# ZKTLabs/zkt-plonk

Hardware: AMD Instinct MI355X
Metric: proofs/sec (withdraw, n=2^20) (higher is better)
Workload: dtype u32 limbs (256-bit Montgomery); 1 GPU; full prove, WithdrawCircuit INPUTS=8 HEIGHT=64 Poseidon x5 (1019498 gates, 538 Poseidon gadgets), bn254, n=2^20, TABLE_SIZE=1024, 12 public inputs; parallelism=proofs sharded across 1 GPU(s), chained=True, distinct_witnesses=2, witness_on_device=True, table_cached=True, proof_bytes=802

## Files before the change

### include/zkt_plonk.h

```cpp
#ifndef ZKT_PLONK_H
#define ZKT_PLONK_H

#include <stddef.h>
#include <stdint.h>

#ifdef __cplusplus
extern "C" {
#endif

typedef struct zkt_ctx zkt_ctx;

enum {
    ZKT_CURVE_BN254 = 0,
    ZKT_CURVE_BLS12_381 = 1
};

enum {
    ZKT_OK = 0,
    ZKT_ERR_INVALID_ARGUMENT = 1,
    ZKT_ERR_INVALID_DOMAIN_SIZE = 2,
    ZKT_ERR_HIP = 3,
    ZKT_ERR_NO_DEVICE = 4,
    ZKT_ERR_TOO_MANY_COEFFICIENTS = 5,
    ZKT_ERR_ZERO_DENOMINATOR = 6,
    ZKT_ERR_EQUAL_CHALLENGES = 7,
    ZKT_ERR_NOT_IN_TABLE = 8,
    ZKT_ERR_QUOTIENT_TOO_SHORT = 9,
    ZKT_ERR_NOT_LOADED = 10,
    ZKT_ERR_COMM = 11
};

int zkt_ctx_create(int curve_id, int device_id, zkt_ctx** out);
void zkt_ctx_destroy(zkt_ctx* ctx);
int zkt_ctx_fork(zkt_ctx* ctx, zkt_ctx** out);
const char* zkt_last_error(const zkt_ctx* ctx);
int zkt_ctx_set_stream(zkt_ctx* ctx, void* hip_stream);
int zkt_ctx_synchronize(zkt_ctx* ctx);
int zkt_profile_enable(zkt_ctx* ctx, int on);
int zkt_profile_get(zkt_ctx* ctx, const char* name, uint64_t* calls, double* total_ms);
const char* zkt_version(void);

typedef struct {
    void* user;
    int rank;
    int world;
    int device_buffers;
    int (*all_gather)(void* user, const void* send, void* recv, size_t bytes, int on_device, void* hip_stream);
    int (*all_gather_async)(void* user, const void* d_send, void* d_recv, size_t bytes, void* hip_stream);
} zkt_comm_vtable;
#define ZKT_QUOTIENT_CHUNKS 4
int zkt_ctx_set_comm(zkt_ctx* ctx, const zkt_comm_vtable* comm);
int zkt_shard_range(size_t total, int rank, int world, size_t* lo, size_t* hi);
int zkt_comm_stats(zkt_ctx* ctx, uint64_t* calls, uint64_t* bytes_sent);
int zkt_comm_selftest(const zkt_comm_vtable* comm, const void* send, void* recv, size_t bytes);

int zkt_dev_alloc(zkt_ctx* ctx, size_t bytes, void** dptr);
int zkt_dev_free(zkt_ctx* ctx, void* dptr);
int zkt_dev_upload(zkt_ctx* ctx, void* dptr, const void* host, size_t bytes);
int zkt_dev_download(zkt_ctx* ctx, void* host, const void* dptr, size_t bytes);

int zkt_ntt(zkt_ctx* ctx, int log_n, int inverse, int coset, const uint64_t* in, size_t in_len, uint64_t* out);
int zkt_ntt_dev(zkt_ctx* ctx, int log_n, int inverse, int coset, const void* d_in, size_t in_len, void* d_out);
int zkt_ntt_class(zkt_ctx* ctx, int log_n, int log_big, int cls, const uint64_t* in, size_t in_len, uint64_t* out);
int zkt_domain_group_gen(zkt_ctx* ctx, int log_n, uint64_t* out4);

int zkt_srs_load(zkt_ctx* ctx, const uint64_t* g1_xy_mont, size_t count);
int zkt_srs_load_dev(zkt_ctx* ctx, const void* d_g1_xy_mont, size_t count);
int zkt_srs_generate(zkt_ctx* ctx, const uint64_t* tau_canonical4, size_t count);
int zkt_srs_download(zkt_ctx* ctx, size_t offset, size_t count, uint64_t* out_xy_mont);
int zkt_srs_generate_g2(int curve_id, const uint64_t* tau_canonical4, uint64_t* out_h, uint64_t* out_beta_h);
int zkt_srs_load_slice(zkt_ctx* ctx, const uint64_t* g1_xy_mont_slice, size_t offset, size_t count, size_t total);
int zkt_srs_generate_slice(zkt_ctx* ctx, const uint64_t* tau_canonical4, size_t offset, size_t count, size_t total);
int zkt_msm_g1(zkt_ctx* ctx, const uint64_t* scalars, size_t len, size_t base_offset, int scalars_montgomery,
               uint64_t* out_xy_mont, int* out_is_infinity);
int zkt_msm_g1_dev(zkt_ctx* ctx, const void* d_scalars, size_t len, size_t base_offset, int scalars_montgomery,
                   void* out_xy_mont_host);
int zkt_msm_enqueue_dev(zkt_ctx* ctx, const void* d_scalars, size_t len, size_t base_offset, int scalars_montgomery);
int zkt_msm_info(zkt_ctx* ctx, int* window_bits, int* windows, size_t* srs_count);

#define ZKT_MSM_BASES_MAX ((size_t)1 << 22)
int zkt_msm_g1_bases(zkt_ctx* ctx, const uint64_t* bases_xy_mont, const uint64_t* scalars, size_t n,
                     int scalars_montgomery, uint64_t* out_xy_mont, int* out_is_infinity);
int zkt_msm_g1_bases_dev(zkt_ctx* ctx, const void* d_bases_xy_mont, const void* d_scalars, size_t n,
                         int scalars_montgomery, uint64_t* out_xy_mont_host, int* out_is_infinity);
int zkt_msm_bases_info(zkt_ctx* ctx, size_t n, int scalars_montgomery, int* window_bits, int* windows);

#define ZKT_KZG_BATCH_MAX 32
int zkt_kzg_commit_batch(zkt_ctx* ctx, const uint64_t* const* coeffs, const size_t* lens, int k,
                         int scalars_montgomery, uint64_t* out_xy_mont, int* out_is_infinity);
int zkt_kzg_commit_batch_dev(zkt_ctx* ctx, const void* const* d_coeffs, const size_t* lens, int k,
                             int scalars_montgomery, uint64_t* out_xy_mont, int* out_is_infinity);
int zkt_kzg_open(zkt_ctx* ctx, const uint64_t* const* coeffs, const size_t* lens, int k,
                 const uint64_t* challenges_mont, const uint64_t* point_mont,
                 uint64_t* out_w_xy_mont, int* out_w_is_infinity, uint64_t* out_evals_mont);
int zkt_kzg_open_dev(zkt_ctx* ctx, const void* const* d_coeffs, const size_t* lens, int k,
                     const uint64_t* challenges_mont, const uint64_t* point_mont,
                     uint64_t* out_w_xy_mont, int* out_w_is_infinity, uint64_t* out_evals_mont);

int zkt_ctx_set_lagrange(zkt_ctx* ctx, int on);
int zkt_ctx_set_wire_elimination(zkt_ctx* ctx, int mode);
int zkt_ctx_set_quotient_route(zkt_ctx* ctx, int mode);
int zkt_ctx_set_fused_passes(zkt_ctx* ctx, int mode);
int zkt_lagrange_info(zkt_ctx* ctx, int* log_n, size_t* bases);
int zkt_commit_evals_dev(zkt_ctx* ctx, const void* d_evals, const uint64_t* blinders, int k, int path, uint64_t* out_xy_mont,
                         int* out_is_infinity);

enum {
    ZKT_TRANSCRIPT_MERLIN = 0,
    ZKT_TRANSCRIPT_ETHEREUM = 1
};
typedef struct zkt_transcript zkt_transcript;
zkt_transcript* zkt_transcript_new(int kind, const char* label);
void zkt_transcript_free(zkt_transcript* t);
void zkt_transcript_append_u64(zkt_transcript* t, const char* label, uint64_t v);
void zkt_transcript_append_scalars(zkt_transcript* t, const char* label, const uint8_t* le32, size_t count, int single);
void zkt_transcript_append_commitment(zkt_transcript* t, const char* label, const uint8_t* x_le, const uint8_t* y_le,
                                      size_t fq_bytes, int is_infinity);
void zkt_transcript_challenge_scalar(zkt_transcript* t, const char* label, int fr_bits, uint8_t out_le32[32]);
void zkt_transcript_seed(zkt_transcript* t, uint64_t circuit_size, const uint8_t* xy_le, const uint8_t* is_infinity,
                         size_t fq_bytes);
int zkt_transcript_append_message(zkt_transcript* t, const char* label, const uint8_t* msg, size_t len);
int zkt_transcript_challenge_bytes(zkt_transcript* t, const char* label, uint8_t* out, size_t len);

typedef struct {
    void* user;
    void (*append_u64)(void* user, const char* label, uint64_t v);
    void (*append_scalars)(void* user, const char* label, const uint64_t* fr_mont, size_t count, int single);
    void (*append_commitment)(void* user, const char* label, const uint64_t* g1_xy_mont, int is_infinity);
    void (*challenge_scalar)(void* user, const char* label, uint64_t* fr_mont_out4);
} zkt_transcript_vtable;

int zkt_circuit_load(zkt_ctx* ctx, int log_n, const uint64_t* const* pk_polys, const size_t* pk_lens);

int zkt_circuit_setup(zkt_ctx* ctx, int log_n, const uint64_t* const* evals, const size_t* eval_lens, int evals_on_device,
                      uint64_t* out_commitments, int* out_is_infinity);

int zkt_circuit_sigma_dev(zkt_ctx* ctx, int log_n, const uint32_t* d_w_l, const uint32_t* d_w_r, const uint32_t* d_w_o,
                          size_t n_rows, size_t n_vars, void* const* d_sigma);
int zkt_circuit_setup_wiring(zkt_ctx* ctx, int log_n, const uint64_t* const* evals, const size_t* eval_lens,
                             int evals_on_device, const uint32_t* w_l, const uint32_t* w_r, const uint32_t* w_o,
                             size_t n_rows, size_t n_vars, int wiring_on_device,
                             uint64_t* out_commitments, int* out_is_infinity);

typedef struct {
    const uint64_t* a_evals;
    const uint64_t* b_evals;
    const uint64_t* c_evals;
    size_t n_rows;
    const uint64_t* table;
    size_t table_len;
    const size_t* pi_pos;
    const uint64_t* pi_vals;
    size_t n_pi;
    const uint64_t* blinders;
    int wires_on_device;
    const uint64_t* variables;
    size_t n_vars;
    const uint32_t* w_l;
    const uint32_t* w_r;
    const uint32_t* w_o;
} zkt_prove_inputs;
#define ZKT_VARIABLE_ZERO 0xFFFFFFFFu

int zkt_prove(zkt_ctx* ctx, const zkt_prove_inputs* in, zkt_transcript* transcript, uint8_t* proof_out,
              size_t proof_cap, size_t* proof_len);
int zkt_prove_set_next(zkt_ctx* ctx, const zkt_prove_inputs* next);
int zkt_prove_with(zkt_ctx* ctx, const zkt_prove_inputs* in, const zkt_transcript_vtable* transcript,
                   uint8_t* proof_out, size_t proof_cap, size_t* proof_len);

enum {
    ZKT_CHECK_WIRING = 1
};
#define ZKT_CHECK_NONE ((uint64_t)-1)
typedef struct {
    int satisfied;
    int checked;
    uint64_t n_arithmetic;
    uint64_t first_arithmetic;
    uint64_t residual[4];
    uint64_t n_lookup;
    uint64_t first_lookup;
    uint64_t n_wiring;
    uint64_t first_wiring_row;
    int first_wiring_column;
} zkt_witness_report;
int zkt_circuit_check_witness(zkt_ctx* ctx, const zkt_prove_inputs* in, int flags, zkt_witness_report* out);

typedef struct {
// ... 207 lines not shown
```

### shim/src/ffi.rs

```rust
use std::os::raw::{c_char, c_int, c_void};

#[repr(C)]
pub struct ZktCtx {
    _private: [u8; 0],
}

#[repr(C)]
pub struct ZktTranscriptVtable {
    pub user: *mut c_void,
    pub append_u64: extern "C" fn(*mut c_void, *const c_char, u64),
    pub append_scalars: extern "C" fn(*mut c_void, *const c_char, *const u64, usize, c_int),
    pub append_commitment: extern "C" fn(*mut c_void, *const c_char, *const u64, c_int),
    pub challenge_scalar: extern "C" fn(*mut c_void, *const c_char, *mut u64),
}

#[repr(C)]
pub struct ZktCommVtable {
    pub user: *mut c_void,
    pub rank: c_int,
    pub world: c_int,
    pub device_buffers: c_int,
    pub all_gather: extern "C" fn(*mut c_void, *const c_void, *mut c_void, usize, c_int, *mut c_void) -> c_int,
    pub all_gather_async: Option<extern "C" fn(*mut c_void, *const c_void, *mut c_void, usize, *mut c_void) -> c_int>,
}
// ... 4 lines not shown
    pub b_evals: *const u64,
    pub c_evals: *const u64,
    pub n_rows: usize,
    pub table: *const u64,
    pub table_len: usize,
    pub pi_pos: *const usize,
    pub pi_vals: *const u64,
    pub n_pi: usize,
    pub blinders: *const u64,
    pub wires_on_device: c_int,
    pub variables: *const u64,
    pub n_vars: usize,
    pub w_l: *const u32,
    pub w_r: *const u32,
    pub w_o: *const u32,
}

#[repr(C)]
pub struct ZktWitnessReport {
    pub satisfied: c_int,
    pub checked: c_int,
    pub n_arithmetic: u64,
    pub first_arithmetic: u64,
    pub residual: [u64; 4],
    pub n_lookup: u64,
    pub first_lookup: u64,
    pub n_wiring: u64,
    pub first_wiring_row: u64,
    pub first_wiring_column: c_int,
}

#[repr(C)]
pub struct ZktSrsReport {
    pub count: u64,
    pub n_bad: u64,
    pub first_bad: u64,
    pub by_status: [u64; 6],
    pub first_bad_status: c_int,
    pub points_ok: c_int,
    pub structure_checked: c_int,
    pub structure_ok: c_int,
    pub ok: c_int,
    pub sum_xy_mont: [u64; 12],
    pub sum_is_infinity: c_int,
}

pub const ZKT_CHECK_WIRING: c_int = 1;
pub const ZKT_CHECK_NONE: u64 = u64::MAX;
pub const ZKT_VARIABLE_ZERO: u32 = 0xFFFF_FFFF;
pub const ZKT_CURVE_BN254: c_int = 0;
pub const ZKT_CURVE_BLS12_381: c_int = 1;
pub const ZKT_KZG_BATCH_MAX: usize = 32;

extern "C" {
    pub fn zkt_ctx_create(curve_id: c_int, device_id: c_int, out: *mut *mut ZktCtx) -> c_int;
    pub fn zkt_ctx_destroy(ctx: *mut ZktCtx);
    pub fn zkt_last_error(ctx: *const ZktCtx) -> *const c_char;
    pub fn zkt_ctx_set_comm(ctx: *mut ZktCtx, comm: *const ZktCommVtable) -> c_int;
    pub fn zkt_shard_range(total: usize, rank: c_int, world: c_int, lo: *mut usize, hi: *mut usize) -> c_int;
    pub fn zkt_ntt(ctx: *mut ZktCtx, log_n: c_int, inverse: c_int, coset: c_int, input: *const u64, in_len: usize,
                   out: *mut u64) -> c_int;
    pub fn zkt_srs_load(ctx: *mut ZktCtx, g1_xy_mont: *const u64, count: usize) -> c_int;
    pub fn zkt_srs_load_slice(ctx: *mut ZktCtx, g1_xy_mont: *const u64, offset: usize, count: usize, total: usize) -> c_int;
    pub fn zkt_srs_load_file(ctx: *mut ZktCtx, ck_path: *const c_char, max_powers: usize) -> c_int;
    pub fn zkt_msm_g1(ctx: *mut ZktCtx, scalars: *const u64, len: usize, base_offset: usize, scalars_montgomery: c_int,
                      out_xy_mont: *mut u64, out_is_infinity: *mut c_int) -> c_int;
    pub fn zkt_ctx_fork(ctx: *mut ZktCtx, out: *mut *mut ZktCtx) -> c_int;
    pub fn zkt_kzg_commit_batch(ctx: *mut ZktCtx, coeffs: *const *const u64, lens: *const usize, k: c_int,
                                scalars_montgomery: c_int, out_xy_mont: *mut u64, out_is_infinity: *mut c_int) -> c_int;
    pub fn zkt_kzg_commit_batch_dev(ctx: *mut ZktCtx, d_coeffs: *const *const c_void, lens: *const usize, k: c_int,
                                    scalars_montgomery: c_int, out_xy_mont: *mut u64, out_is_infinity: *mut c_int) -> c_int;
    pub fn zkt_kzg_open(ctx: *mut ZktCtx, coeffs: *const *const u64, lens: *const usize, k: c_int, challenges_mont: *const u64,
                        point_mont: *const u64, out_w_xy_mont: *mut u64, out_w_is_infinity: *mut c_int,
                        out_evals_mont: *mut u64) -> c_int;
    pub fn zkt_kzg_open_dev(ctx: *mut ZktCtx, d_coeffs: *const *const c_void, lens: *const usize, k: c_int,
                            challenges_mont: *const u64, point_mont: *const u64, out_w_xy_mont: *mut u64,
                            out_w_is_infinity: *mut c_int, out_evals_mont: *mut u64) -> c_int;
    pub fn zkt_commit_evals_dev(ctx: *mut ZktCtx, d_evals: *const c_void, blinders: *const u64, k: c_int, path: c_int,
                                out_xy_mont: *mut u64, out_is_infinity: *mut c_int) -> c_int;
    pub fn zkt_ctx_set_lagrange(ctx: *mut ZktCtx, on: c_int) -> c_int;
    pub fn zkt_ctx_set_wire_elimination(ctx: *mut ZktCtx, mode: c_int) -> c_int;
    pub fn zkt_ctx_set_quotient_route(ctx: *mut ZktCtx, mode: c_int) -> c_int;
    pub fn zkt_ctx_set_fused_passes(ctx: *mut ZktCtx, mode: c_int) -> c_int;
    pub fn zkt_lagrange_info(ctx: *mut ZktCtx, log_n: *mut c_int, bases: *mut usize) -> c_int;
    pub fn zkt_circuit_load(ctx: *mut ZktCtx, log_n: c_int, pk_polys: *const *const u64, pk_lens: *const usize) -> c_int;
    pub fn zkt_circuit_load_file(ctx: *mut ZktCtx, pk_path: *const c_char, log_n: c_int) -> c_int;
    pub fn zkt_keyfile_extended_prover_key(path: *const c_char, curve_id: c_int, which: c_int, out_mont: *mut u64, cap: usize,
                                           lens17: *mut usize) -> c_int;
    pub fn zkt_circuit_check_epk_file(ctx: *mut ZktCtx, epk_path: *const c_char, first_mismatch_vector: *mut c_int,
                                      mismatch_at: *mut usize) -> c_int;
    pub fn zkt_circuit_setup(ctx: *mut ZktCtx, log_n: c_int, evals: *const *const u64, eval_lens: *const usize,
                             evals_on_device: c_int, out_commitments: *mut u64, out_is_infinity: *mut c_int) -> c_int;
    pub fn zkt_circuit_sigma_dev(ctx: *mut ZktCtx, log_n: c_int, d_w_l: *const u32, d_w_r: *const u32, d_w_o: *const u32,
                                 n_rows: usize, n_vars: usize, d_sigma: *const *mut c_void) -> c_int;
    pub fn zkt_circuit_setup_wiring(ctx: *mut ZktCtx, log_n: c_int, evals: *const *const u64, eval_lens: *const usize,
                                    evals_on_device: c_int, w_l: *const u32, w_r: *const u32, w_o: *const u32, n_rows: usize,
                                    n_vars: usize, wiring_on_device: c_int, out_commitments: *mut u64,
                                    out_is_infinity: *mut c_int) -> c_int;
    pub fn zkt_prove_with(ctx: *mut ZktCtx, inputs: *const ZktProveInputs, transcript: *const ZktTranscriptVtable,
                          proof_out: *mut u8, proof_cap: usize, proof_len: *mut usize) -> c_int;
    pub fn zkt_prove_set_next(ctx: *mut ZktCtx, next: *const ZktProveInputs) -> c_int;
    pub fn zkt_circuit_check_witness(ctx: *mut ZktCtx, inputs: *const ZktProveInputs, flags: c_int,
                                     out: *mut ZktWitnessReport) -> c_int;
    pub fn zkt_g1_msm_host(curve_id: c_int, points_xy_mont: *const u64, scalars: *const u64, n: usize, scalars_montgomery: c_int,
                           out_xy_mont: *mut u64, out_is_infinity: *mut c_int) -> c_int;
    pub fn zkt_msm_g1_bases(ctx: *mut ZktCtx, bases_xy_mont: *const u64, scalars: *const u64, n: usize,
                            scalars_montgomery: c_int, out_xy_mont: *mut u64, out_is_infinity: *mut c_int) -> c_int;
    pub fn zkt_msm_g1_bases_dev(ctx: *mut ZktCtx, d_bases_xy_mont: *const c_void, d_scalars: *const c_void, n: usize,
                                scalars_montgomery: c_int, out_xy_mont_host: *mut u64, out_is_infinity: *mut c_int) -> c_int;
    pub fn zkt_verify(curve_id: c_int, inputs: *const ZktVerifyInputs, transcript: *mut c_void, h_g2_mont: *const u64,
                      beta_h_g2_mont: *const u64, accepted: *mut c_int) -> c_int;
    pub fn zkt_verify_batch(curve_id: c_int, inputs: *const ZktVerifyInputs, transcripts: *const *mut c_void, count: usize,
                            h_g2_mont: *const u64, beta_h_g2_mont: *const u64, accepted: *mut c_int) -> c_int;
    pub fn zkt_verify_batch_prepare_dev(ctx: *mut ZktCtx, inputs: *const ZktVerifyInputs, transcripts: *const *mut c_void, count: usize,
                                        h_g2_mont: *const u64, beta_h_g2_mont: *const u64, out_ab: *mut u64,
                                        out_ab_is_infinity: *mut c_int, out_rho: *mut u64) -> c_int;
    pub fn zkt_verify_batch_dev(ctx: *mut ZktCtx, inputs: *const ZktVerifyInputs, transcripts: *const *mut c_void, count: usize,
                                h_g2_mont: *const u64, beta_h_g2_mont: *const u64, accepted: *mut c_int) -> c_int;
    pub fn zkt_verify_batch_locate(ctx: *mut ZktCtx, inputs: *const ZktVerifyInputs, transcripts: *const *mut c_void, count: usize,
                                   h_g2_mont: *const u64, beta_h_g2_mont: *const u64, accepted: *mut c_int, out_bad: *mut u8,
                                   n_bad: *mut usize, n_checks: *mut usize) -> c_int;
    pub fn zkt_g1_decompress(ctx: *mut ZktCtx, compressed: *const u8, n: usize, out_xy_mont: *mut u64, out_status: *mut u8) -> c_int;
    pub fn zkt_g1_decompress_dev(ctx: *mut ZktCtx, d_compressed: *const c_void, n: usize, d_out_xy_mont: *mut c_void,
                                 d_out_status: *mut c_void) -> c_int;
    pub fn zkt_g1_check(ctx: *mut ZktCtx, points_xy_mont: *const c_void, n: usize, points_on_device: c_int, out_status: *mut u8) -> c_int;
    pub fn zkt_srs_check(ctx: *mut ZktCtx, g1_xy_mont: *const c_void, count: usize, points_on_device: c_int, h_g2_mont: *const u64,
                         beta_h_g2_mont: *const u64, seed32: *const u8, out_status: *mut u8, report: *mut ZktSrsReport) -> c_int;
    pub fn zkt_poseidon_load(ctx: *mut ZktCtx, params: *const ZktPoseidonParams, out: *mut *mut c_void) -> c_int;
    pub fn zkt_poseidon_free(ctx: *mut ZktCtx, params: *mut c_void);
    pub fn zkt_poseidon_hash_batch_dev(ctx: *mut ZktCtx, params: *const c_void, d_inputs: *const c_void, batch: usize,
                                       arity: c_int, d_out_hashes: *mut c_void, d_out_states: *mut c_void) -> c_int;
    pub fn zkt_poseidon_gadget_vars_per_hash(params: *const c_void) -> usize;
    pub fn zkt_poseidon_gadget_witness_dev(ctx: *mut ZktCtx, params: *const c_void, args: *const ZktPoseidonGadgetArgs) -> c_int;
    pub fn zkt_poseidon_gadget_check(ctx: *mut ZktCtx, params: *const c_void) -> c_int;
    pub fn zkt_merkle_path_vars_per_level(params: *const c_void) -> usize;
    pub fn zkt_poseidon_merkle_path_witness_dev(ctx: *mut ZktCtx, params: *const c_void, args: *const ZktMerklePathArgs) -> c_int;
    pub fn zkt_poseidon_merkle_path_validate(ctx: *mut ZktCtx, params: *const c_void, args: *const ZktMerklePathArgs) -> c_int;
    pub fn zkt_merkle_tree_create(ctx: *mut ZktCtx, params: *const c_void, height: c_int, capacity: usize, out: *mut *mut c_void) -> c_int;
    pub fn zkt_merkle_tree_free(ctx: *mut ZktCtx, tree: *mut c_void);
    pub fn zkt_merkle_tree_append_dev(ctx: *mut ZktCtx, tree: *mut c_void, d_leaves: *const c_void, m: usize, first_index: *mut u64) -> c_int;
    pub fn zkt_merkle_tree_append(ctx: *mut ZktCtx, tree: *mut c_void, leaves: *const u64, m: usize, first_index: *mut u64) -> c_int;
    pub fn zkt_merkle_tree_root(ctx: *mut ZktCtx, tree: *mut c_void, out4: *mut u64) -> c_int;
    pub fn zkt_merkle_tree_info(tree: *const c_void, height: *mut c_int, count: *mut u64, capacity: *mut u64) -> c_int;
    pub fn zkt_merkle_tree_layer(ctx: *mut ZktCtx, tree: *mut c_void, layer: c_int, first: u64, n: usize, out: *mut u64) -> c_int;
    pub fn zkt_merkle_tree_paths(ctx: *mut ZktCtx, tree: *mut c_void, indices: *const u64, k: usize, out_siblings: *mut u64) -> c_int;
    pub fn zkt_merkle_tree_paths_to_variables_dev(ctx: *mut ZktCtx, tree: *mut c_void, indices: *const u64, k: usize,
                                                  d_variables: *mut c_void, n_vars: usize, bit_var0: *const u32,
                                                  sibling_var0: *const u32) -> c_int;
    pub fn zkt_debug_merkle_tree_split(tree: *mut c_void, wide_min_parents: c_int) -> c_int;
    pub fn zkt_debug_live_allocations(count: *mut u64, bytes: *mut u64) -> c_int;
    pub fn zkt_dev_alloc(ctx: *mut ZktCtx, bytes: usize, dptr: *mut *mut c_void) -> c_int;
    pub fn zkt_dev_free(ctx: *mut ZktCtx, dptr: *mut c_void) -> c_int;
    pub fn zkt_dev_upload(ctx: *mut ZktCtx, dptr: *mut c_void, host: *const c_void, bytes: usize) -> c_int;
}

#[cfg(feature = "rccl")]
#[link(name = "zkt_comm_rccl")]
extern "C" {
    pub fn zkt_comm_rccl_unique_id(out: *mut u8) -> c_int;
    pub fn zkt_comm_rccl_create(id: *const u8, rank: c_int, world: c_int, device: c_int, out: *mut *mut c_void) -> c_int;
    pub fn zkt_comm_rccl_vtable(comm: *mut c_void, out: *mut ZktCommVtable) -> c_int;
    pub fn zkt_comm_rccl_destroy(comm: *mut c_void);
    pub fn zkt_comm_rccl_last_error(comm: *const c_void) -> *const c_char;
}

#[repr(C)]
// ... 50 lines not shown
```

### zkt-plonk_amd/_lib.py

```python
from __future__ import annotations

import ctypes
import os
import re
from typing import Optional

import numpy as np

_HERE = os.path.dirname(os.path.abspath(__file__))
_LIB = os.environ.get("ZKT_LIB_PATH") or os.path.join(_HERE, "libzkt_plonk_hip.so")
_HEADER = os.path.join(_HERE, "..", "include", "zkt_plonk.h")

MSM_BASES_MAX = 1 << 22
G1_DECOMPRESS_MAX = 1 << 22
VERIFY_BATCH_DEV_MAX = MSM_BASES_MAX // 24
KZG_BATCH_MAX = 32
CURVE_BN254 = 0
CURVE_BLS12_381 = 1
_CURVES = {"bn254": 0, "bls12_381": 1, "bls12-381": 1, 0: 0, 1: 1}

_lib = None


class ZktError(RuntimeError):
# ... 1433 lines not shown
    def debug_combine_split(self, table, f, fresh: bool = True):
        t = np.ascontiguousarray(table, dtype=np.uint64).reshape(-1, 4)
        ff = np.ascontiguousarray(f, dtype=np.uint64).reshape(-1, 4)
        if self.circuit_log_n is None or ff.shape[0] != 1 << self.circuit_log_n:
            raise ValueError("f must hold the n elements of a circuit loaded through this Context")
        n = ff.shape[0]
        h1, h2 = np.empty((n, 4), dtype=np.uint64), np.empty((n, 4), dtype=np.uint64)
        P64 = ctypes.POINTER(ctypes.c_uint64)
        self._L.zkt_debug_combine_split.argtypes = [ctypes.c_void_p, P64, ctypes.c_size_t, P64, ctypes.c_int, P64, P64]
        self.check(self._L.zkt_debug_combine_split(self._h, u64p(t) if t.shape[0] else None, t.shape[0], u64p(ff),
                                                   1 if fresh else 0, u64p(h1), u64p(h2)))
        return h1, h2

    def debug_commit_wires_dev(self, d_variables: int, n_vars: int, d_w_l: int, d_w_r: int, d_w_o: int, n_rows: int, blinders,
                               route: int = 1, pi_pos=None):
        bl = np.ascontiguousarray(blinders, dtype=np.uint64).reshape(6, 4)
        out = np.zeros((3, 2 * self.fq_limbs), dtype=np.uint64)
        inf = (ctypes.c_int * 3)()
        took = (ctypes.c_int * 3)()
        if route == 2 or pi_pos is not None:
            pos = [int(x) for x in (pi_pos or ())]
            pi = (ctypes.c_size_t * max(len(pos), 1))(*pos)
            self._L.zkt_debug_commit_wires_pi_dev.argtypes = [ctypes.c_void_p, ctypes.c_void_p, ctypes.c_size_t, ctypes.c_void_p,
                                                              ctypes.c_void_p, ctypes.c_void_p, ctypes.c_size_t,
                                                              ctypes.POINTER(ctypes.c_uint64), ctypes.c_int,
                                                              ctypes.POINTER(ctypes.c_size_t), ctypes.c_size_t,
                                                              ctypes.POINTER(ctypes.c_uint64), ctypes.POINTER(ctypes.c_int),
                                                              ctypes.POINTER(ctypes.c_int)]
            self.check(self._L.zkt_debug_commit_wires_pi_dev(self._h, ctypes.c_void_p(d_variables), n_vars, ctypes.c_void_p(d_w_l),
                                                             ctypes.c_void_p(d_w_r), ctypes.c_void_p(d_w_o), n_rows, u64p(bl),
                                                             int(route), pi, len(pos), u64p(out), inf, took))
            return out, [bool(x) for x in inf], [int(x) for x in took]
        self._L.zkt_debug_commit_wires_dev.argtypes = [ctypes.c_void_p, ctypes.c_void_p, ctypes.c_size_t, ctypes.c_void_p,
                                                       ctypes.c_void_p, ctypes.c_void_p, ctypes.c_size_t,
                                                       ctypes.POINTER(ctypes.c_uint64), ctypes.c_int,
                                                       ctypes.POINTER(ctypes.c_uint64), ctypes.POINTER(ctypes.c_int),
                                                       ctypes.POINTER(ctypes.c_int)]
        self.check(self._L.zkt_debug_commit_wires_dev(self._h, ctypes.c_void_p(d_variables), n_vars, ctypes.c_void_p(d_w_l),
                                                      ctypes.c_void_p(d_w_r), ctypes.c_void_p(d_w_o), n_rows, u64p(bl), int(route),
                                                      u64p(out), inf, took))
        return out, [bool(x) for x in inf], [int(x) for x in took]

    def check_epk_file(self, path: str):
        self._L.zkt_circuit_check_epk_file.argtypes = [ctypes.c_void_p, ctypes.c_char_p, ctypes.POINTER(ctypes.c_int),
                                                       ctypes.POINTER(ctypes.c_size_t)]
        vec, at = ctypes.c_int(0), ctypes.c_size_t(0)
        self.check(self._L.zkt_circuit_check_epk_file(self._h, path.encode(), ctypes.byref(vec), ctypes.byref(at)))
        if vec.value < 0:
            return None
        return vec.value, (-1 if at.value == ctypes.c_size_t(-1).value else at.value)

    def debug_eval_lincomb(self, polys, points, scalars, out_len: int):
        keep = [np.ascontiguousarray(p_, dtype=np.uint64).reshape(-1, 4) for p_ in polys]
        k = len(keep)
        P64 = ctypes.POINTER(ctypes.c_uint64)
        ptrs = (P64 * k)(*[u64p(a) for a in keep])
        lens = (ctypes.c_size_t * k)(*[a.shape[0] for a in keep])
        pts = np.ascontiguousarray(points, dtype=np.uint64).reshape(k, 4)
        scs = np.ascontiguousarray(scalars, dtype=np.uint64).reshape(k, 4)
        ev = np.empty((k, 4), dtype=np.uint64)
        lc = np.empty((out_len, 4), dtype=np.uint64)
        self._L.zkt_debug_eval_lincomb.argtypes = [ctypes.c_void_p, ctypes.POINTER(P64), ctypes.POINTER(ctypes.c_size_t), ctypes.c_int,
                                                   P64, P64, P64, P64, ctypes.c_size_t]
        self.check(self._L.zkt_debug_eval_lincomb(self._h, ptrs, lens, k, u64p(pts), u64p(scs), u64p(ev), u64p(lc), out_len))
        return ev, lc

    def debug_open_witness(self, coeffs, z) -> np.ndarray:
        p_ = np.ascontiguousarray(coeffs, dtype=np.uint64).reshape(-1, 4)
        zz = np.ascontiguousarray(z, dtype=np.uint64).reshape(4)
        out = np.empty((p_.shape[0] - 1, 4), dtype=np.uint64)
        self._L.zkt_debug_open_witness.argtypes = [ctypes.c_void_p, ctypes.POINTER(ctypes.c_uint64), ctypes.c_size_t,
                                                   ctypes.POINTER(ctypes.c_uint64), ctypes.POINTER(ctypes.c_uint64)]
        self.check(self._L.zkt_debug_open_witness(self._h, u64p(p_), p_.shape[0], u64p(zz), u64p(out)))
        return out

    def set_quotient_route(self, mode: int = 0):
        self._L.zkt_ctx_set_quotient_route.argtypes = [ctypes.c_void_p, ctypes.c_int]
        self.check(self._L.zkt_ctx_set_quotient_route(self._h, int(mode)))

    def set_fused_passes(self, mode: int = 0):
        self._L.zkt_ctx_set_fused_passes.argtypes = [ctypes.c_void_p, ctypes.c_int]
        self.check(self._L.zkt_ctx_set_fused_passes(self._h, int(mode)))

    def debug_quotient_top(self):
        u = np.zeros((6, 4), dtype=np.uint64)
        on = ctypes.c_int(0)
        self._L.zkt_debug_quotient_top.argtypes = [ctypes.c_void_p, ctypes.POINTER(ctypes.c_uint64), ctypes.POINTER(ctypes.c_int)]
        self.check(self._L.zkt_debug_quotient_top(self._h, u64p(u), ctypes.byref(on)))
        return u, bool(on.value)

    def debug_quotient_coeffs(self, count: int) -> np.ndarray:
        out = np.zeros((count, 4), dtype=np.uint64)
        self._L.zkt_debug_quotient_coeffs.argtypes = [ctypes.c_void_p, ctypes.POINTER(ctypes.c_uint64), ctypes.c_size_t]
        self.check(self._L.zkt_debug_quotient_coeffs(self._h, u64p(out), int(count)))
        return out

    def debug_quotient(self, n: int, challenges, wit, pi_pos=(), pi_vals=None) -> np.ndarray:
        ch = np.ascontiguousarray(challenges, dtype=np.uint64).reshape(5, 4)
        keep = [None if w is None else np.ascontiguousarray(w, dtype=np.uint64).reshape(4 * n, 4) for w in wit]
        assert len(keep) == 9
        ptrs = (ctypes.c_void_p * 9)(*[None if w is None else w.ctypes.data for w in keep])
        pos = np.ascontiguousarray(list(pi_pos), dtype=np.uint64)
        vals = np.ascontiguousarray(pi_vals if len(pos) else np.zeros((0, 4)), dtype=np.uint64).reshape(-1, 4)
        out = np.empty((4 * n, 4), dtype=np.uint64)
        self.check(self._L.zkt_debug_quotient(self._h, u64p(ch), ptrs, u64p(pos) if len(pos) else None,
                                              u64p(vals) if len(pos) else None, len(pos), u64p(out)))
        return out
```

### zkt-plonk_amd/csrc/capi.hip

```cpp
#include "ctx.hpp"

#include <cstdlib>
#include "hostinv.hpp"
#include "ec.hpp"
#include "hostec.hpp"
#include "fx_test.hpp"
#include "msm.hpp"

#include <atomic>
#include <cstring>

namespace zkt {

const char* exp_env(const char* name) {
#ifdef ZKT_EXPERIMENTS
    return getenv(name);
#else
    (void)name;
    return nullptr;
#endif
}

int set_err(zkt_ctx* c, int code, const std::string& msg) {
    if (c) c->err = msg;
// ... 128 lines not shown
    (void)hipEventCreate(&e);
    return e;
}
ProfScope::ProfScope(zkt_ctx* ctx, const char* name, hipStream_t on_stream, uint64_t units) : c(ctx), count(units) {
    if (!c->prof_on) return;
    if (c->prof_on == 2 && strcmp(name, "msm_accumulate") != 0 && strcmp(name, "host_wait") != 0) return;
    stream = on_stream ? on_stream : c->stream;
    slot = &c->prof[name];
    e0 = prof_event(c);
    e1 = prof_event(c);
    (void)hipEventRecord(e0, stream);
}
ProfScope::~ProfScope() {
    if (!slot) return;
    (void)hipEventRecord(e1, stream);
    slot->pending.emplace_back(e0, e1);
    slot->calls += count;
    ++slot->launches;
}
static void prof_resolve(zkt_ctx* c) {
    (void)hipStreamSynchronize(c->stream);
    (void)hipDeviceSynchronize();
    for (auto& kv : c->prof) {
        for (auto& pr : kv.second.pending) {
            float ms = 0.f;
            if (hipEventElapsedTime(&ms, pr.first, pr.second) == hipSuccess) kv.second.total_ms += ms;
            c->event_pool.push_back(pr.first);
            c->event_pool.push_back(pr.second);
        }
        kv.second.pending.clear();
    }
}

template <class P>
__global__ void k_fr_mul(const Fe<P>* a, const Fe<P>* b, Fe<P>* o, size_t n) {
    size_t i = (size_t)blockIdx.x * blockDim.x + threadIdx.x;
    if (i < n) fe_store<P>(o + i, fe_mul<P>(fe_load<P>(a + i), fe_load<P>(b + i)));
}

template <class P>
__global__ void k_fx_test(int op, const uint32_t* in, size_t n, uint32_t* out) {
    constexpr int W = 4 * FxP<P>::L;
    size_t i = (size_t)blockIdx.x * blockDim.x + threadIdx.x;
    if (i < n) fx_test_op<P>(op, in + i * W, out + i * W);
}
template <class Q>
__global__ void k_xyzz_test(int op, const uint32_t* in, size_t n, uint32_t* out) {
    constexpr int W = 4 * FxP<Q>::L + 1;
    size_t i = (size_t)blockIdx.x * blockDim.x + threadIdx.x;
    if (i < n) xyzz_test_op<Q>(op, in + i * 2 * W, out + i * W);
}

template <class P>
static int dump_params(uint32_t* out, size_t words) {
    const int N = P::N;
    if (words < (size_t)(3 * N + 1)) return -1;
    for (int i = 0; i < N; ++i) out[i] = P::mod(i);
    out[N] = P::INV;
    for (int i = 0; i < N; ++i) out[N + 1 + i] = P::one(i);
    for (int i = 0; i < N; ++i) out[2 * N + 1 + i] = P::r2(i);
    return N;
}

}

using namespace zkt;

extern "C" {

const char* zkt_version(void) { return "zkt-plonk_amd 0.1 (gfx950)"; }

int zkt_ctx_create(int curve_id, int device_id, zkt_ctx** out) {
    if (!out) return ZKT_ERR_INVALID_ARGUMENT;
    *out = nullptr;
    if (curve_id != ZKT_CURVE_BN254 && curve_id != ZKT_CURVE_BLS12_381) return ZKT_ERR_INVALID_ARGUMENT;
    int count = 0;
    if (hipGetDeviceCount(&count) != hipSuccess || count <= 0 || device_id < 0 || device_id >= count)
        return ZKT_ERR_NO_DEVICE;
    if (hipSetDevice(device_id) != hipSuccess) return ZKT_ERR_NO_DEVICE;
    zkt_ctx* c = new zkt_ctx();
    c->batch_off = exp_env("ZKT_MSM_NO_BATCH") != nullptr;
    c->aux_off = exp_env("ZKT_NO_AUX") != nullptr;
    if (const char* parts = exp_env("ZKT_FUSED_PARTS")) c->fused_parts = atoi(parts) & 63;
    c->curve = curve_id;
    c->device = device_id;
    if (hipStreamCreateWithFlags(&c->stream, hipStreamNonBlocking) != hipSuccess) {
        delete c;
        return ZKT_ERR_HIP;
    }
    c->own_stream = true;
    *out = c;
    return ZKT_OK;
}

int zkt_ctx_fork(zkt_ctx* parent, zkt_ctx** out) {
    if (!parent || !out) return ZKT_ERR_INVALID_ARGUMENT;
    *out = nullptr;
    if (parent->sharded()) return set_err(parent, ZKT_ERR_INVALID_ARGUMENT, "zkt_ctx_fork: not for a context with a communicator");
    zkt_ctx* c = nullptr;
    int rc = zkt_ctx_create(parent->curve, parent->device, &c);
    if (rc) return rc;
    (void)hipStreamSynchronize(parent->stream);
    c->is_fork = true;
    c->lagrange_off = parent->lagrange_off;
    c->wire_elim_mode = parent->wire_elim_mode;
    c->quotient_route = parent->quotient_route;
    c->fused_passes = parent->fused_passes;
    c->fused_parts = parent->fused_parts;
    c->batch_off = parent->batch_off;
    c->aux_off = parent->aux_off;
    c->ntt_plans = parent->ntt_plans;
    if ((rc = msm_fork(c, parent)) || (rc = circuit_fork(c, parent))) {
        parent->err = c->err;
        zkt_ctx_destroy(c);
        return rc;
    }
    *out = c;
    return ZKT_OK;
}

void zkt_ctx_destroy(zkt_ctx* c) {
    if (!c) return;
    (void)hipSetDevice(c->device);
    (void)hipStreamSynchronize(c->stream);
    circuit_release(c);
    msm_release(c);
    prof_resolve(c);
    for (hipEvent_t e : c->event_pool) (void)hipEventDestroy(e);
    c->event_pool.clear();
    c->ntt_plans.clear();
    c->msmb.reset();
    c->kzg.reset();
    if (c->comm.pinned) (void)hipHostFree(c->comm.pinned);
    for (const auto& a : c->owned) counted_free(a);
    c->owned.clear();
    if (c->own_stream && c->stream) (void)hipStreamDestroy(c->stream);
    delete c;
}

int zkt_ctx_set_comm(zkt_ctx* c, const zkt_comm_vtable* comm) {
    if (!c) return ZKT_ERR_INVALID_ARGUMENT;
    if (int rf = refuse_if_forked(c, "zkt_ctx_set_comm")) return rf;
    if (c->is_fork && comm && comm->world > 1) return set_err(c, ZKT_ERR_INVALID_ARGUMENT, "a forked context cannot take a communicator");
    if (comm && comm->world > 1) {
        const int w = comm->world;
        if ((w != 2 && w != 4 && w != 8) || comm->rank < 0 || comm->rank >= w || !comm->all_gather)
            return set_err(c, ZKT_ERR_INVALID_ARGUMENT, "communicator: world must be 1, 2, 4 or 8 with a valid rank and callback");
    }
    (void)hipSetDevice(c->device);
    (void)hipStreamSynchronize(c->stream);
    circuit_release(c);
    msm_release(c);
    c->comm.vt = zkt_comm_vtable{};
    c->comm.vt.world = 1;
    if (comm && comm->world > 1) c->comm.vt = *comm;
    c->comm.calls = 0;
    c->comm.bytes = 0;
    return ZKT_OK;
}
int zkt_shard_range(size_t total, int rank, int world, size_t* lo, size_t* hi) {
    if (world < 1 || rank < 0 || rank >= world || !lo || !hi) return ZKT_ERR_INVALID_ARGUMENT;
    const size_t base = total / (size_t)world, rem = total % (size_t)world;
    *lo = (size_t)rank * base + ((size_t)rank < rem ? (size_t)rank : rem);
    *hi = *lo + base + ((size_t)rank < rem ? 1 : 0);
    return ZKT_OK;
}
int zkt_comm_stats(zkt_ctx* c, uint64_t* calls, uint64_t* bytes_sent) {
    if (!c || !calls || !bytes_sent) return ZKT_ERR_INVALID_ARGUMENT;
    *calls = c->comm.calls;
    *bytes_sent = c->comm.bytes;
    return ZKT_OK;
}
int zkt_comm_selftest(const zkt_comm_vtable* comm, const void* send, void* recv, size_t bytes) {
    if (!comm || !comm->all_gather || !send || !recv) return ZKT_ERR_INVALID_ARGUMENT;
    return comm->all_gather(comm->user, send, recv, bytes, 0, nullptr) ? ZKT_ERR_COMM : ZKT_OK;
}

const char* zkt_last_error(const zkt_ctx* c) { return c ? c->err.c_str() : "null context"; }

int zkt_ctx_set_stream(zkt_ctx* c, void* hip_stream) {
    if (!c) return ZKT_ERR_INVALID_ARGUMENT;
    ZKT_HIP(c, hipStreamSynchronize(c->stream));
    if (c->own_stream && c->stream) (void)hipStreamDestroy(c->stream);
    c->stream = (hipStream_t)hip_stream;
    c->own_stream = false;
    return ZKT_OK;
}

int zkt_profile_enable(zkt_ctx* c, int on) {
    if (!c) return ZKT_ERR_INVALID_ARGUMENT;
    prof_resolve(c);
// ... 336 lines not shown
```

### zkt-plonk_amd/csrc/ctx.hpp

```cpp
#pragma once
#include <hip/hip_runtime.h>
#include <stdint.h>
#include <stddef.h>
#include <map>
#include <string>
#include <tuple>
#include <vector>
#include <memory>

#include "../../include/zkt_plonk.h"
#include "fp.hpp"
#include "fx.hpp"
#include "ntt.hpp"

namespace zkt {

struct MsmState;
struct MsmBasesState;
struct KzgState;
struct CircuitState;

}

struct zkt_ctx {
    int curve = 0;
    int device = 0;
    hipStream_t stream = nullptr;
    bool own_stream = false;
    std::string err;

    std::map<std::tuple<int, int, int, int>, std::shared_ptr<void>> ntt_plans;
    int ntt_split_npass = 0;
    int ntt_split_log_r[3] = {0, 0, 0};
    void* ntt_scratch = nullptr;
    size_t ntt_scratch_bytes = 0;
    void* io_a = nullptr;
    size_t io_a_bytes = 0;
    void* io_b = nullptr;
    size_t io_b_bytes = 0;
    void* check_scratch = nullptr;
    size_t check_scratch_bytes = 0;
    void* verify_scratch = nullptr;
    size_t verify_scratch_bytes = 0;

    int prof_on = 0;
    struct ProfSlot {
        std::vector<std::pair<hipEvent_t, hipEvent_t>> pending;
        double total_ms = 0.0;
        uint64_t calls = 0;
        uint64_t launches = 0;
    };
    std::map<std::string, ProfSlot> prof;
    std::vector<hipEvent_t> event_pool;

    struct Comm {
        zkt_comm_vtable vt{};
        void* pinned = nullptr;
        size_t pinned_bytes = 0;
        uint64_t calls = 0, bytes = 0;
    } comm;
    bool sharded() const { return comm.vt.world > 1; }

    std::shared_ptr<zkt::MsmState> msm;
    std::shared_ptr<zkt::MsmBasesState> msmb;
    std::shared_ptr<zkt::KzgState> kzg;
    size_t srs_check_chunk = 0;
    uint64_t msm_epoch = 0;
    uint64_t srs_generation = 0;
    bool is_fork = false;
    bool aux_off = false;
    bool batch_off = false;
    bool lagrange_off = false;
    int wire_elim_mode = 1;
    int quotient_route = 0;
    int fused_passes = 0;
    int fused_parts = 63;
    bool fused(int part) const { return fused_passes != 2 && (fused_parts & part); }
    std::shared_ptr<zkt::CircuitState> circuit;
    std::vector<std::pair<void*, size_t>> owned;
};

namespace zkt {

const char* exp_env(const char* name);

int set_err(zkt_ctx* c, int code, const std::string& msg);
int refuse_if_forked(zkt_ctx* c, const char* what);
int hip_fail(zkt_ctx* c, hipError_t e, const char* what);

#define ZKT_HIP(c, call)                                        \
    do {                                                        \
        hipError_t _e = (call);                                 \
        if (_e != hipSuccess) return zkt::hip_fail((c), _e, #call); \
    } while (0)

struct ProfScope {
    zkt_ctx* c;
    zkt_ctx::ProfSlot* slot = nullptr;
    hipEvent_t e0 = nullptr, e1 = nullptr;
    hipStream_t stream = nullptr;
    uint64_t count = 1;
    ProfScope(zkt_ctx* ctx, const char* name, hipStream_t on_stream = nullptr, uint64_t units = 1);
    ~ProfScope();
};

int comm_all_gather_host(zkt_ctx* c, const void* send, void* recv, size_t bytes);
int comm_all_gather_dev(zkt_ctx* c, const void* d_send, void* d_recv, size_t bytes);
bool comm_async_available(const zkt_ctx* c);
int comm_all_gather_async(zkt_ctx* c, const void* d_send, void* d_recv, size_t bytes, hipStream_t st);

int ensure_buffer(zkt_ctx* c, void** p, size_t* cur, size_t bytes);
struct DevBuf {
    void* p = nullptr;
    size_t bytes = 0;
};
inline int grow(zkt_ctx* c, DevBuf& b, size_t bytes) { return ensure_buffer(c, &b.p, &b.bytes, bytes); }
int dev_alloc(zkt_ctx* c, void** p, size_t bytes);
void dev_free(zkt_ctx* c, void* p);

struct DevShared {
    const int device;
    std::vector<std::pair<void*, size_t>> mem;
    std::shared_ptr<DevShared> from;
    explicit DevShared(int dev) : device(dev) {}
    DevShared(const DevShared&) = delete;
    DevShared& operator=(const DevShared&) = delete;
    ~DevShared();
    int alloc(zkt_ctx* c, void** p, size_t bytes);
    void release(void* p);
};
inline std::shared_ptr<DevShared> dev_shared_reader(const std::shared_ptr<DevShared>& of) {
    if (!of) return nullptr;
    auto r = std::make_shared<DevShared>(of->device);
    r->from = of;
    return r;
}
inline bool dev_shared_has_readers(const std::shared_ptr<DevShared>& m) { return m && m.use_count() > 1; }

template <class P>
Fe<P> root_of_unity(int log_n);
int ntt_run(zkt_ctx* c, int log_n, int inverse, int coset, const void* d_in, size_t in_len, void* d_out);
int ntt_run_batch(zkt_ctx* c, int log_n, int inverse, int coset, int nb, const void* const* d_in, const size_t* in_len,
                  void* const* d_out, const void* d_head = nullptr);
int ntt_fold_heads(zkt_ctx* c, int nb, const void* const* d_in, size_t n, const uint32_t* gammas, void* d_out);
int ntt_run_classes(zkt_ctx* c, int log_n, int inverse, const int codes[3], int nb, const void* const* d_in, const size_t* in_len,
                    void* const* d_out, size_t in_stride, size_t out_stride, const void* d_head = nullptr);
int ntt_class_code(int log_big, int cls);
int ntt_force_split(zkt_ctx* c, int npass, const int* log_r);
int ntt_run_class(zkt_ctx* c, int log_n, int log_big, int cls, const void* d_in, size_t in_len, void* d_out, void* d_fold);

void circuit_release(zkt_ctx* c);
int circuit_fork(zkt_ctx* child, const zkt_ctx* parent);
bool circuit_tables_have_readers(const zkt_ctx* c);

}
```

### zkt-plonk_amd/csrc/msm.hip

```cpp
#include "ctx.hpp"
#include "ec.hpp"
#include "ecx.hpp"
#include "hostec.hpp"
#include "msm.hpp"

#include <algorithm>
#include <functional>
#include <type_traits>
#include <cstdlib>
#include <cstring>

namespace zkt {

template <class C>
__global__ void k_srs_generate(Affine<typename C::Fq>* out, size_t count, Fe<typename C::Fr> tau_mont,
                               Affine<typename C::Fq> g, size_t first) {
    using Q = typename C::Fq;
    using R = typename C::Fr;
    size_t i = (size_t)blockIdx.x * blockDim.x + threadIdx.x;
    if (i >= count) return;
    Fe<R> s = fe_from_mont<R>(fe_from_mont<R>(fe_pow_u64<R>(tau_mont, (uint64_t)(first + i))));
    Xyzz<Q> acc = xyzz_identity<Q>();
    bool started = false;
#pragma unroll 1
// ... 487 lines not shown
        const uint32_t key = (b << lb) + col;
        if (owns) offsets[key] = first[k];
        if (owns && key >= 1 && key <= B && run[k]) {
            const uint32_t tb = (first[k] + chunk - 1) / chunk;
            const uint32_t te = (uint32_t)(((uint64_t)first[k] + run[k] + chunk - 1) / chunk);
            uint32_t at = 256;
            if (te - tb > 8) at = atomicAdd(&nbig, 1u);
            if (at < 256) {
                big[at][0] = key; big[at][1] = tb; big[at][2] = te;
            } else {
                for (uint32_t t = tb; t < te; ++t) chunk_bucket[t] = key;
            }
        }
    }
    __syncthreads();
    const uint32_t nb = nbig < 256u ? nbig : 256u;
    for (uint32_t e = 0; e < nb; ++e)
        for (uint32_t t = big[e][1] + threadIdx.x; t < big[e][2]; t += 256) chunk_bucket[t] = big[e][0];
    for (uint32_t t = t0; t < t1; ++t) {
#pragma unroll
        for (uint32_t k = 0; k < K; ++k) pos2[(size_t)t * COLS + threadIdx.x * K + k] += first[k];
    }
}

constexpr int MSM_L2S_THREADS = 1024;
constexpr int MSM_L2S_PER = MSM_L2_TILE / MSM_L2S_THREADS;
template <class PF, int LC>
__global__ __launch_bounds__(MSM_L2S_THREADS) void k_msm_l2_scatter(const typename PF::type* pairs, uint32_t nb1, uint32_t lb,
                                                                    const uint32_t* tile_start, const uint2* tile_desc,
                                                                    const uint32_t* cnt2, const uint32_t* pos2,
                                                                    uint32_t* vals, MsmBatch bt) {
    constexpr uint32_t COLS = 1u << LC;
    {
        const uint32_t y = blockIdx.y;
        pairs = reinterpret_cast<const typename PF::type*>(reinterpret_cast<const char*>(pairs) + y * bt.s_pairs_bytes);
        tile_start += y * bt.s_bin;
        tile_desc += y * bt.s_tile_desc;
        cnt2 += y * bt.s_cnt;
        pos2 += y * bt.s_cnt;
        vals += y * bt.s_vals;
    }
    typedef typename std::conditional<(LC <= 8), uint8_t, uint16_t>::type key_t;
    __shared__ uint32_t cursor[COLS], delta[COLS], wsum[16];
    __shared__ uint32_t sval[MSM_L2_TILE];
    __shared__ key_t skey[MSM_L2_TILE];
    const L2Item it = msm_l2_item(blockIdx.x, nb1, tile_start, tile_desc);
    if (!it.valid) return;
    const uint32_t cnt = it.e - it.s;
    typename PF::type v[MSM_L2S_PER];
#pragma unroll
    for (int k = 0; k < MSM_L2S_PER; ++k) {
        const uint32_t j = (uint32_t)MSM_L2S_THREADS * k + threadIdx.x;
        if (j < cnt) v[k] = pairs[it.s + j];
    }
    uint32_t mine = 0, p2 = 0;
    if (threadIdx.x < COLS) {
        mine = cnt2[(size_t)blockIdx.x * COLS + threadIdx.x];
        p2 = pos2[(size_t)blockIdx.x * COLS + threadIdx.x];
    }
    uint32_t ex;
    if constexpr (LC <= 8) ex = block_excl_scan_256(mine, wsum);
    else ex = block_excl_scan_1024(mine, wsum, nullptr);
    if (threadIdx.x < COLS) {
        cursor[threadIdx.x] = ex;
        delta[threadIdx.x] = p2 - ex;
    }
    __syncthreads();
    uint32_t a[MSM_L2S_PER];
#pragma unroll
    for (int k = 0; k < MSM_L2S_PER; ++k) {
        const uint32_t j = (uint32_t)MSM_L2S_THREADS * k + threadIdx.x;
        if (j < cnt) a[k] = atomicAdd(&cursor[PF::low(v[k], lb)], 1u);
    }
#pragma unroll
    for (int k = 0; k < MSM_L2S_PER; ++k) {
        const uint32_t j = (uint32_t)MSM_L2S_THREADS * k + threadIdx.x;
        if (j < cnt) {
            sval[a[k]] = PF::val(v[k], lb);
            skey[a[k]] = (key_t)PF::low(v[k], lb);
        }
    }
    __syncthreads();
    for (uint32_t j = threadIdx.x; j < cnt; j += MSM_L2S_THREADS) vals[delta[skey[j]] + j] = sval[j];
}

template <class C>
__global__ __launch_bounds__(256) void k_msm_accumulate(const uint32_t* vals, uint32_t B, const uint32_t* chunk_bucket,
                                                        MsmBatch bt) {
    using Q = typename C::Fq;
    const uint32_t y = blockIdx.y;
    const Affine<Q>* table = (const Affine<Q>*)bt.table[y];
    vals += y * bt.s_vals;
    chunk_bucket += y * bt.s_chunk;
    const uint32_t* offsets = bt.offsets[y];
    XyzzRaw<Q>* pieces = (XyzzRaw<Q>*)bt.pieces[y];
    const uint32_t chunk = bt.params[y][0];
    const uint32_t base = offsets[1], m = offsets[B + 1];
    const uint32_t t = blockIdx.x * blockDim.x + threadIdx.x;
    const uint64_t p0 = (uint64_t)base + (uint64_t)t * chunk;
    if (p0 >= m) return;
    const uint32_t p1 = (uint32_t)((p0 + chunk < m) ? p0 + chunk : m);
    uint32_t cur = chunk_bucket[t];
    uint32_t end = offsets[cur + 1];
    uint32_t end2 = offsets[(cur + 2 <= B + 1) ? cur + 2 : B + 1];
    XyzzX<Q> acc = xx_identity<Q>();
    uint32_t v = vals[p0];
    uint32_t v1 = (p0 + 1 < p1) ? vals[p0 + 1] : 0u;
    Fe<Q> nx = fe_load<Q>(&table[v & 0x7fffffffu].x), ny = fe_load<Q>(&table[v & 0x7fffffffu].y);
    for (uint32_t p = (uint32_t)p0; p < p1; ++p) {
        const uint32_t vcur = v;
        const Fe<Q> cx = nx, cy = ny;
        v = v1;
        if (p + 1 < p1) {
            nx = fe_load<Q>(&table[v & 0x7fffffffu].x);
            ny = fe_load<Q>(&table[v & 0x7fffffffu].y);
        }
        if (p + 2 < p1) v1 = vals[p + 2];
        if (p == end) {
            xx_store_raw<Q>(pieces + (size_t)t + cur, acc);
            acc = xx_identity<Q>();
            do {
                ++cur;
                end = end2;
                end2 = offsets[(cur + 2 <= B + 1) ? cur + 2 : B + 1];
            } while (end <= p);
        }
        if (!(fe_is_zero<Q>(cx) && fe_is_zero<Q>(cy))) {
            AffineX<Q> q;
            q.x = fx_unpack<Q>(cx);
            q.y = fx_unpack<Q>(cy);
            if (vcur >> 31) q.y = fx_sub<Q, 1>(fx_zero<Q>(), q.y);
            acc = xx_add_mixed<Q, true>(acc, q);
        }
    }
    xx_store_raw<Q>(pieces + (size_t)t + cur, acc);
}


template <class C, bool MSM_TAIL_INL>
__global__ __launch_bounds__(256) void k_msm_bucket_sum(uint32_t B, MsmTailBatch tb) {
    using Q = typename C::Fq;
    const uint32_t* offsets = tb.offsets[blockIdx.y];
    const XyzzRaw<Q>* pieces = (const XyzzRaw<Q>*)tb.pieces[blockIdx.y];
    Xyzz<Q>* buckets = (Xyzz<Q>*)tb.buckets[blockIdx.y];
    uint32_t* heavy = tb.heavy[blockIdx.y];
    const uint32_t chunk = tb.params[blockIdx.y][0];
    const uint32_t b = blockIdx.x * blockDim.x + threadIdx.x;
    if (b > B) return;
    XyzzX<Q> acc = xx_identity<Q>();
    if (b >= 1) {
        const uint32_t base = offsets[1];
        const uint32_t s = offsets[b], e = offsets[b + 1];
        if (e > s) {
            const uint32_t t0 = (s - base) / chunk, t1 = (e - 1 - base) / chunk;
            if (t1 - t0 >= MSM_HEAVY) {
                heavy[1 + atomicAdd(heavy, 1u)] = b;
                return;
            }
            acc = xx_load_raw<Q>(pieces + (size_t)t0 + b);
            for (uint32_t t = t0 + 1; t <= t1; ++t) acc = xx_add<Q, MSM_TAIL_INL>(acc, xx_load_raw<Q>(pieces + (size_t)t + b));
        }
    }
    xx_store<Q>(buckets + b, acc);
}

template <class Q>
// ... 331 lines not shown
    st->strides.s_tile_desc = up(P.l2_items);
    st->strides.s_cnt = up((size_t)P.l2_items << P.lcols);
    if ((rc = dev_alloc(c, (void**)&st->bin_offs, NB * st->strides.s_bin_offs * 4))) return rc;
    if ((rc = dev_alloc(c, (void**)&st->bin_aux, NB * st->strides.s_bin_aux * 4))) return rc;
    if ((rc = dev_alloc(c, (void**)&st->bin_start, NB * st->strides.s_bin * 4))) return rc;
    if ((rc = dev_alloc(c, (void**)&st->tile_start, NB * st->strides.s_bin * 4))) return rc;
    if ((rc = dev_alloc(c, &st->tile_desc, NB * st->strides.s_tile_desc * 8))) return rc;
    if ((rc = dev_alloc(c, (void**)&st->cnt2, NB * st->strides.s_cnt * 4))) return rc;
    if ((rc = dev_alloc(c, (void**)&st->pos2, NB * st->strides.s_cnt * 4))) return rc;
    if ((rc = msm_scatter_lds_cap<C, false>(c, P.packed, P.dig))) return rc;
    static_assert(MsmState::SLOTS == 11, "per-slot arrays are sized for 11 slots");
    for (int i = 0; i < MsmState::SLOTS; ++i) {
        if ((rc = dev_alloc(c, (void**)&st->offsets[i], (((size_t)P.nb1 << P.lb) + 2) * 4))) return rc;
        if ((rc = dev_alloc(c, (void**)&st->heavy[i], ((size_t)P.keys + 2) * 4))) return rc;
        if ((rc = dev_alloc(c, (void**)&st->params[i], 16))) return rc;
    }
    if ((rc = msm_acc_setup<C>(c, &st->acc_threads, &st->acc_lds))) return rc;
    size_t max_chunks = std::min(m, st->acc_threads) + 1;
    for (int i = 0; i < MsmState::SLOTS; ++i)
        if ((rc = dev_alloc(c, &st->pieces[i], (max_chunks + P.keys + 2) * sizeof(XyzzRaw<Q>)))) return rc;
    st->strides.s_chunk = up(max_chunks + 2);
    if ((rc = dev_alloc(c, (void**)&st->chunk_bucket, NB * st->strides.s_chunk * 4))) return rc;
    ZKT_HIP(c, hipStreamCreateWithFlags(&st->side, hipStreamNonBlocking));
    for (int i = 0; i < MsmState::SLOTS; ++i) {
        if ((rc = dev_alloc(c, &st->buckets[i], ((size_t)P.keys + 1) * sizeof(Xyzz<Q>)))) return rc;
        {
            const int q = P.c - 1, q2 = q / 2, q1 = q - q2;
            if ((rc = dev_alloc(c, &st->rowcol[i], (((size_t)1 << q1) + ((size_t)1 << q2)) * sizeof(Xyzz<Q>)))) return rc;
        }
        ZKT_HIP(c, hipHostMalloc(&st->host_result[i], (size_t)(MSM_MAX_Y + 1) * MSM_R2_BLOCKS * sizeof(Xyzz<Q>), hipHostMallocMapped));
        ZKT_HIP(c, hipHostGetDevicePointer(&st->host_result_dev[i], st->host_result[i], 0));
        ZKT_HIP(c, hipEventCreateWithFlags(&st->ev_main[i], hipEventDisableTiming));
        ZKT_HIP(c, hipEventCreateWithFlags(&st->ev_done[i], hipEventDisableTiming));
    }
    st->defer_tails = count <= MSM_DEFER_MAX;
    if (const char* e = exp_env("ZKT_MSM_DEFER")) st->defer_tails = atoi(e) != 0;
    c->msm = st;
    ++c->msm_epoch;
    ++c->srs_generation;
    return ZKT_OK;
}

template <class C>
static int table_finish(zkt_ctx* c, void* table, size_t count) {
    using Q = typename C::Fq;
    MsmState& st = *c->msm;
    unsigned blocks = (unsigned)((count + 127) / 128);
    hipLaunchKernelGGL(k_srs_windows<C>, dim3(blocks), dim3(128), 0, c->stream, (Affine<Q>*)table, count, st.plan.win);
    ZKT_HIP(c, hipGetLastError());
    const size_t total = (size_t)st.plan.W * count;
    hipLaunchKernelGGL(k_srs_to_fx<C>, dim3((unsigned)((total + 255) / 256)), dim3(256), 0, c->stream,
                       (Affine<Q>*)table, total);
    ZKT_HIP(c, hipGetLastError());
    ZKT_HIP(c, hipStreamSynchronize(c->stream));
    return ZKT_OK;
}
template <class C>
static int srs_finish(zkt_ctx* c) {
    return table_finish<C>(c, c->msm->table, c->msm->count);
}
int msm_fork(zkt_ctx* child, const zkt_ctx* parent) {
    msm_release(child);
    if (!parent->msm) return ZKT_OK;
    int rc = parent->curve == ZKT_CURVE_BN254 ? msm_setup<Bn254Curve>(child, parent->msm->count, parent->msm.get())
                                               : msm_setup<Bls381Curve>(child, parent->msm->count, parent->msm.get());
    if (rc) return rc;
    child->srs_generation = parent->srs_generation;
    return ZKT_OK;
}
int msm_table_finish(zkt_ctx* c, void* table, size_t count) {
    if (c->curve == ZKT_CURVE_BN254) return table_finish<Bn254Curve>(c, table, count);
    return table_finish<Bls381Curve>(c, table, count);
}

void msm_release(zkt_ctx* c) {
    if (!c->msm) return;
    MsmState& st = *c->msm;
    (void)hipStreamSynchronize(c->stream);
    if (st.side) (void)hipStreamSynchronize(st.side);
    wire_bases_drop(c);
    for (DevBuf& b : st.wb_scalars) dev_free(c, b.p);
    dev_free(c, st.wb_dig);
    void* ptrs[] = {st.vals2, st.pairs, st.bin_offs, st.bin_aux, st.bin_start, st.tile_start, st.cnt2, st.pos2, st.chunk_bucket,
                    st.tile_desc};
    for (void* p : ptrs) dev_free(c, p);
    for (int i = 0; i < MsmState::SLOTS; ++i) {
        dev_free(c, st.heavy[i]); dev_free(c, st.offsets[i]); dev_free(c, st.pieces[i]); dev_free(c, st.params[i]);
        dev_free(c, st.buckets[i]); dev_free(c, st.rowcol[i]);
    }
    c->msm.reset();
}
bool msm_tables_have_readers(const zkt_ctx* c) {
    return c->msm && (dev_shared_has_readers(c->msm->table_mem) || dev_shared_has_readers(c->msm->lag_mem) ||
                      dev_shared_has_readers(c->msm->wb.mem));
}

template <class C>
static int srs_load_t(zkt_ctx* c, const void* src, size_t count, bool src_on_device, size_t slice_off = 0, size_t total = 0) {
    using Q = typename C::Fq;
    if (count == 0) return set_err(c, ZKT_ERR_INVALID_ARGUMENT, "empty SRS");
    if (int rf = refuse_if_forked(c, "loading a key")) return rf;
    msm_release(c);
    int rc = msm_setup<C>(c, count);
    if (rc) return rc;
    c->msm->slice_off = slice_off;
    c->msm->total = total ? total : count;
    ZKT_HIP(c, hipMemcpyAsync(c->msm->table, src, count * sizeof(Affine<Q>),
                              src_on_device ? hipMemcpyDeviceToDevice : hipMemcpyHostToDevice, c->stream));
    {
        using R = typename C::Fr;
        Fe<R> raw_one = fe_zero<R>();
        raw_one.v[0] = 1u;
        const Fe<R> rinv = fe_from_mont<R>(raw_one);
        hipLaunchKernelGGL((k_srs_scale<C, false>), dim3((unsigned)((count + 127) / 128)), dim3(128), 0, c->stream,
                           (const Affine<Q>*)c->msm->table, (Affine<Q>*)c->msm->table, count, rinv);
        ZKT_HIP(c, hipGetLastError());
    }
    return srs_finish<C>(c);
}

template <class C>
static Affine<typename C::Fq> generator_mont();
template <>
Affine<Bn254Fq> generator_mont<Bn254Curve>() {
    Affine<Bn254Fq> g;
    g.x = fe_from_u32<Bn254Fq>(1);
    g.y = fe_from_u32<Bn254Fq>(2);
    return g;
}
template <>
Affine<Bls381Fq> generator_mont<Bls381Curve>() {
    static const uint32_t gx[12] = {0xdb22c6bbu, 0xfb3af00au, 0xf97a1aefu, 0x6c55e83fu, 0x171bac58u, 0xa14e3a3fu,
                                    0x9774b905u, 0xc3688c4fu, 0x4fa9ac0fu, 0x2695638cu, 0x3197d794u, 0x17f1d3a7u};
    static const uint32_t gy[12] = {0x46c5e7e1u, 0x0caa2329u, 0xa2888ae4u, 0xd03cc744u, 0x2c04b3edu, 0x00db18cbu,
                                    0xd5d00af6u, 0xfcf5e095u, 0x741d8ae4u, 0xa09e30edu, 0xe3aaa0f1u, 0x08b3f481u};
    Affine<Bls381Fq> g;
    for (int i = 0; i < 12; ++i) {
        g.x.v[i] = gx[i];
        g.y.v[i] = gy[i];
    }
    g.x = fe_to_mont<Bls381Fq>(g.x);
    g.y = fe_to_mont<Bls381Fq>(g.y);
    return g;
}

template <class C>
static int srs_generate_t(zkt_ctx* c, const uint64_t* tau4, size_t count, size_t slice_off = 0, size_t total = 0) {
    using Q = typename C::Fq;
    using R = typename C::Fr;
    if (count == 0) return set_err(c, ZKT_ERR_INVALID_ARGUMENT, "empty SRS");
    if (int rf = refuse_if_forked(c, "loading a key")) return rf;
    msm_release(c);
    int rc = msm_setup<C>(c, count);
    if (rc) return rc;
    c->msm->slice_off = slice_off;
    c->msm->total = total ? total : count;
    Fe<R> tau;
    memcpy(tau.v, tau4, 32);
    tau = fe_to_mont<R>(tau);
    unsigned blocks = (unsigned)((count + 127) / 128);
    hipLaunchKernelGGL(k_srs_generate<C>, dim3(blocks), dim3(128), 0, c->stream, (Affine<Q>*)c->msm->table, count, tau,
                       generator_mont<C>(), slice_off);
    ZKT_HIP(c, hipGetLastError());
    return srs_finish<C>(c);
}

template <class C, bool TI>
// ... 37 lines not shown
    ZKT_HIP(c, hipGetLastError());
    }
    for (int j = 0; j < k; ++j) ZKT_HIP(c, hipEventRecord(st.ev_done[st.tail_wait[j]], st.side));
    return ZKT_OK;
}

template <class C>
static int msm_launch_tails(zkt_ctx* c) {
    bool inl = c->msm->defer_tails || c->msm->count <= MSM_TAIL_INL_MAX;
    if (const char* e = exp_env("ZKT_MSM_TAIL_INL")) inl = atoi(e) != 0;
    return inl ? msm_launch_tails_t<C, true>(c) : msm_launch_tails_t<C, false>(c);
}

struct MsmWork {
    uint32_t *bin_offs, *bin_aux, *bin_start, *tile_start;
    void* tile_desc;
    uint32_t *cnt2, *pos2;
    void* pairs;
    uint32_t *vals, *chunk_bucket;
};

template <class C, bool VB>
static int msm_launch_grouping(zkt_ctx* c, const MsmPlan& P, const MsmWork& wk, const MsmBatch& bt, int mont, size_t n, unsigned ky,
                               size_t acc_threads, bool defer_tails) {
    const uint32_t S = P.l1_scalars;
    const unsigned nblk = (unsigned)((n + S - 1) / S);
    const uint32_t total = P.nb1 * nblk, ntiles = (total + MSM_SCAN_TILE - 1) / MSM_SCAN_TILE;
    const uint2* tile_desc = (const uint2*)wk.tile_desc;
    {
        auto kc = msm_pick_bin_count<C, VB>(P.dig);
        hipLaunchKernelGGL(kc, dim3(nblk, ky), dim3(1024), (size_t)P.nb1 * 4, c->stream, bt, mont, P.win, S, P.nb1, P.lb, wk.bin_offs);
    }
    hipLaunchKernelGGL(k_msm_scan_tiles, dim3(ntiles, ky), dim3(1024), 0, c->stream, wk.bin_offs, total, wk.bin_aux, bt);
    hipLaunchKernelGGL(k_msm_scan_aux, dim3(1, ky), dim3(1024), 0, c->stream, wk.bin_offs, wk.bin_aux, ntiles, nblk, P.nb1,
                       wk.bin_start, wk.tile_start, (uint2*)wk.tile_desc, (uint32_t)acc_threads, P.keys, defer_tails ? 1u : 0u, bt);
    ZKT_HIP(c, hipGetLastError());
    const size_t lds_scatter = (size_t)((3 * P.nb1 + 3) & ~3u) * 4 + (size_t)MSM_L1_CAP * (P.packed ? 4 : 8);
    const uint32_t items = (uint32_t)((size_t)P.W * n / MSM_L2_TILE + P.nb1);
    if (P.packed) {
        auto ks = msm_pick_bin_scatter<C, PairPacked, VB>(P.dig);
        hipLaunchKernelGGL(ks, dim3(nblk, ky), dim3(1024), lds_scatter, c->stream, bt, mont, P.win, S, P.nb1, P.lb, wk.bin_offs,
                           wk.bin_aux, (uint32_t*)wk.pairs);
        ZKT_HIP(c, hipGetLastError());
        hipLaunchKernelGGL((k_msm_l2_count<PairPacked, 8>), dim3(items, ky), dim3(256), 0, c->stream, (const uint32_t*)wk.pairs,
                           P.nb1, P.lb, wk.tile_start, tile_desc, wk.cnt2, bt);
    } else {
        auto ks = msm_pick_bin_scatter<C, PairWide, VB>(P.dig);
        hipLaunchKernelGGL(ks, dim3(nblk, ky), dim3(1024), lds_scatter, c->stream, bt, mont, P.win, S, P.nb1, P.lb, wk.bin_offs,
                           wk.bin_aux, (uint2*)wk.pairs);
        ZKT_HIP(c, hipGetLastError());
        auto kc2 = P.lcols == 8 ? k_msm_l2_count<PairWide, 8> : k_msm_l2_count<PairWide, 10>;
        hipLaunchKernelGGL(kc2, dim3(items, ky), dim3(256), 0, c->stream, (const uint2*)wk.pairs, P.nb1, P.lb, wk.tile_start,
                           tile_desc, wk.cnt2, bt);
    }
    {
        auto ksc = P.lcols == 8 ? k_msm_l2_scan<8> : k_msm_l2_scan<10>;
        hipLaunchKernelGGL(ksc, dim3(P.nb1, ky), dim3(256), 0, c->stream, wk.cnt2, wk.pos2, wk.bin_start, wk.tile_start, P.keys,
                           P.lb, wk.chunk_bucket, bt);
    }
    if (P.packed) {
        hipLaunchKernelGGL((k_msm_l2_scatter<PairPacked, 8>), dim3(items, ky), dim3(MSM_L2S_THREADS), 0, c->stream,
                           (const uint32_t*)wk.pairs, P.nb1, P.lb, wk.tile_start, tile_desc, wk.cnt2, wk.pos2, wk.vals, bt);
    } else {
        auto kss = P.lcols == 8 ? k_msm_l2_scatter<PairWide, 8> : k_msm_l2_scatter<PairWide, 10>;
        hipLaunchKernelGGL(kss, dim3(items, ky), dim3(MSM_L2S_THREADS), 0, c->stream, (const uint2*)wk.pairs, P.nb1, P.lb,
                           wk.tile_start, tile_desc, wk.cnt2, wk.pos2, wk.vals, bt);
    }
    ZKT_HIP(c, hipGetLastError());
    return ZKT_OK;
}

template <class C>
static int msm_launch_accumulate(zkt_ctx* c, const MsmPlan& P, const uint32_t* vals, const uint32_t* chunk_bucket, const MsmBatch& bt,
                                 size_t n, size_t acc_threads, size_t acc_lds) {
    const uint32_t max_chunks = (uint32_t)std::min((size_t)P.W * n, acc_threads);
    hipLaunchKernelGGL(k_msm_accumulate<C>, dim3((max_chunks + 255) / 256, 1), dim3(256), acc_lds, c->stream, vals, P.keys,
                       chunk_bucket, bt);
    ZKT_HIP(c, hipGetLastError());
    return ZKT_OK;
}

template <class C>
static int msm_enqueue_batch(zkt_ctx* c, int k, const void* const* d_scalars, const size_t* ns, const size_t* base_offs, int mont,
                             const int* slots, const int* tbls) {
    MsmState& st = *c->msm;
    if (k < 1 || k > MSM_BATCH) return set_err(c, ZKT_ERR_INVALID_ARGUMENT, "msm batch size");
    ++c->msm_epoch;
    for (int j = 0; j < k; ++j)
        for (int w = 0; w < st.n_tail_wait; ++w)
            if (st.tail_wait[w] == slots[j])
                if (int rc0 = msm_launch_tails<C>(c)) return rc0;
    if (st.n_tail_wait + k > MSM_TAIL_BATCH)
        if (int rc0 = msm_launch_tails<C>(c)) return rc0;
    MsmBatch bt = st.strides;
    bool all_lag = true;
    for (int j = 0; j < k; ++j) all_lag = all_lag && tbls[j] != 0;
    size_t n_max = 0;
    for (int j = 0; j < MSM_BATCH; ++j) {
        const int jj = j < k ? j : 0;
        const int slot = slots[jj];
        if (j < k && st.pending[slot]) ZKT_HIP(c, hipStreamWaitEvent(c->stream, st.ev_done[slot], 0));
        bt.scalars[j] = d_scalars[jj];
        bt.n[j] = ns[jj];
        bt.base_off[j] = base_offs[jj];
        bt.table[j] = st.tbl_table(tbls[jj]);
        bt.tcount[j] = st.tbl_count(tbls[jj]);
        bt.heavy[j] = st.heavy[slot];
        bt.params[j] = st.params[slot];
        bt.offsets[j] = st.offsets[slot];
        bt.pieces[j] = st.pieces[slot];
        if (j < k) n_max = std::max(n_max, ns[jj]);
    }
    {
    ProfScope prof_all(c, all_lag ? "msm_lag_main" : "msm_main", nullptr, (uint64_t)k);
    const MsmWork wk{st.bin_offs, st.bin_aux, st.bin_start, st.tile_start, st.tile_desc, st.cnt2, st.pos2, st.pairs, st.vals2,
                     st.chunk_bucket};
    if (int rc = msm_launch_grouping<C, false>(c, st.plan, wk, bt, mont, n_max, (unsigned)k, st.acc_threads, st.defer_tails))
        return rc;
    for (int j = 0; j < k; ++j) {
        MsmBatch one = bt;
        one.offsets[0] = bt.offsets[j];
        one.pieces[0] = bt.pieces[j];
        one.params[0] = bt.params[j];
        one.table[0] = bt.table[j];
        {
            ProfScope prof_acc(c, tbls[j] ? "msm_lag_accumulate" : "msm_accumulate");
            if (int rc = msm_launch_accumulate<C>(c, st.plan, st.vals2 + (size_t)j * st.strides.s_vals,
                                                  st.chunk_bucket + (size_t)j * st.strides.s_chunk, one, ns[j], st.acc_threads, st.acc_lds))
                return rc;
        }
        ZKT_HIP(c, hipEventRecord(st.ev_main[slots[j]], c->stream));
        st.tail_wait[st.n_tail_wait++] = slots[j];
        st.pending[slots[j]] = true;
        if (st.defer_tails && st.n_tail_wait < MSM_TAIL_BATCH) continue;
        if (int rc = msm_launch_tails<C>(c)) return rc;
    }
    }
    return ZKT_OK;
}

template <class C>
static int msm_enqueue(zkt_ctx* c, const void* d_scalars, size_t n, size_t base_off, int mont, int slot = 0, int tbl = 0) {
    return msm_enqueue_batch<C>(c, 1, &d_scalars, &n, &base_off, mont, &slot, &tbl);
}

template <class Q>
static Xyzz<Q> msm_host_finish(const MsmState& st, int slot) {
    const int ny = msm_rows(st.plan.c);
    int exps[MSM_MAX_Y + 1];
    for (int y = 0; y <= ny; ++y) exps[y] = y;
    return hostec::weighted_row_sum<Q>((const Xyzz<Q>*)st.host_result[slot], ny + 1, MSM_R2_BLOCKS, exps);
}

template <class C>
static int msm_collect(zkt_ctx* c, int slot, Affine<typename C::Fq>* out) {
    using Q = typename C::Fq;
    MsmState& st = *c->msm;
    if (int rc0 = msm_launch_tails<C>(c)) return rc0;
    ZKT_HIP(c, hipEventSynchronize(st.ev_done[slot]));
    st.pending[slot] = false;
    *out = xyzz_to_affine_host<Q>(msm_host_finish<Q>(st, slot));
    return ZKT_OK;
}

template <class C>
static int msm_collect_sharded(zkt_ctx* c, const int* slots, const bool* have, int k, Affine<typename C::Fq>* out) {
    using Q = typename C::Fq;
    MsmState& st = *c->msm;
    const int world = c->comm.vt.world;
    std::vector<Xyzz<Q>> send(k), recv((size_t)k * world);
    if (int rc0 = msm_launch_tails<C>(c)) return rc0;
    for (int j = 0; j < k; ++j) {
        if (have[j]) {
            ZKT_HIP(c, hipEventSynchronize(st.ev_done[slots[j]]));
            st.pending[slots[j]] = false;
            send[j] = msm_host_finish<Q>(st, slots[j]);
        } else {
            send[j] = xyzz_identity<Q>();
        }
    }
    int rc = comm_all_gather_host(c, send.data(), recv.data(), (size_t)k * sizeof(Xyzz<Q>));
    if (rc) return rc;
    for (int j = 0; j < k; ++j) {
        Xyzz<Q> acc = xyzz_identity<Q>();
        for (int r = 0; r < world; ++r) acc = xyzz_add<Q>(acc, recv[(size_t)r * k + j]);
        out[j] = xyzz_to_affine_host<Q>(acc);
    }
    return ZKT_OK;
}

template <class C>
static int msm_run_t(zkt_ctx* c, const void* d_scalars, size_t n, size_t base_off, int mont, uint64_t* out_xy,
                     int* out_inf) {
    using Q = typename C::Fq;
    if (!c->msm) return set_err(c, ZKT_ERR_NOT_LOADED, "no SRS loaded (zkt_srs_load)");
    MsmState& st = *c->msm;
    if (base_off > st.count || n > st.count - base_off)
        return set_err(c, ZKT_ERR_TOO_MANY_COEFFICIENTS, "TooManyCoefficients: polynomial longer than the committer key");
    Affine<Q> res;
    if (n == 0) {
        res.x = fe_zero<Q>();
        res.y = fe_zero<Q>();
    } else {
        int rc = msm_enqueue<C>(c, d_scalars, n, base_off, mont, 0);
        if (rc) return rc;
        if ((rc = msm_collect<C>(c, 0, &res))) return rc;
    }
    memcpy(out_xy, res.x.v, Q::N * 4);
    memcpy(out_xy + Q::N / 2, res.y.v, Q::N * 4);
    if (out_inf) *out_inf = aff_is_inf<Q>(res) ? 1 : 0;
    return ZKT_OK;
}

int msm_begin(zkt_ctx* c, const void* d_scalars, size_t n, size_t base_off, int mont, int slot, int tbl) {
    if (!c->msm) return set_err(c, ZKT_ERR_NOT_LOADED, "no SRS loaded (zkt_srs_load)");
    if (slot < 0 || slot >= MsmState::SLOTS) return set_err(c, ZKT_ERR_INVALID_ARGUMENT, "bad MSM slot");
    if (tbl < 0 || tbl > MSM_TBL_WIRE + 2) return set_err(c, ZKT_ERR_INVALID_ARGUMENT, "bad MSM base table");
    if (tbl && !c->msm->tbl_table(tbl)) return set_err(c, ZKT_ERR_NOT_LOADED, "no Lagrange-basis table built");
    const size_t cnt = c->msm->tbl_count(tbl);
    if (n == 0 || base_off > cnt || n > cnt - base_off)
        return set_err(c, ZKT_ERR_TOO_MANY_COEFFICIENTS, "TooManyCoefficients: polynomial longer than the committer key");
    if (c->curve == ZKT_CURVE_BN254) return msm_enqueue<Bn254Curve>(c, d_scalars, n, base_off, mont, slot, tbl);
    return msm_enqueue<Bls381Curve>(c, d_scalars, n, base_off, mont, slot, tbl);
}
int msm_begin_batch(zkt_ctx* c, int k, const void* const* d_scalars, const size_t* ns, int mont, const int* slots, const int* tbls) {
    if (!c->msm) return set_err(c, ZKT_ERR_NOT_LOADED, "no SRS loaded (zkt_srs_load)");
    if (k < 1 || k > MSM_BATCH) return set_err(c, ZKT_ERR_INVALID_ARGUMENT, "msm batch size");
    size_t offs[MSM_BATCH] = {};
    for (int j = 0; j < k; ++j) {
        if (slots[j] < 0 || slots[j] >= MsmState::SLOTS) return set_err(c, ZKT_ERR_INVALID_ARGUMENT, "bad MSM slot");
        for (int i = 0; i < j; ++i)
            if (slots[i] == slots[j]) return set_err(c, ZKT_ERR_INVALID_ARGUMENT, "msm batch: slots must differ");
        if (tbls[j] < 0 || tbls[j] > MSM_TBL_WIRE + 2) return set_err(c, ZKT_ERR_INVALID_ARGUMENT, "bad MSM base table");
        if (tbls[j] && !c->msm->tbl_table(tbls[j])) return set_err(c, ZKT_ERR_NOT_LOADED, "no Lagrange-basis table built");
        if (ns[j] == 0 || ns[j] > c->msm->tbl_count(tbls[j]))
            return set_err(c, ZKT_ERR_TOO_MANY_COEFFICIENTS, "TooManyCoefficients: polynomial longer than the committer key");
    }
    if (c->curve == ZKT_CURVE_BN254) return msm_enqueue_batch<Bn254Curve>(c, k, d_scalars, ns, offs, mont, slots, tbls);
    return msm_enqueue_batch<Bls381Curve>(c, k, d_scalars, ns, offs, mont, slots, tbls);
}
bool msm_defers_tails(const zkt_ctx* c) { return c->msm && c->msm->defer_tails; }
bool msm_batches_grouping(const zkt_ctx* c) {
    if (!c->msm) return false;
    const size_t n = c->msm->count;
    if (const char* e = exp_env("ZKT_MSM_BATCH_MAX_LOG")) return n <= ((size_t)1 << atoi(e)) + 64;
    return n <= MSM_DEFER_MAX || (n > ((size_t)1 << 17) + 64 && n <= ((size_t)1 << 18) + 64);
}
int msm_flush_tails(zkt_ctx* c) {
    if (!c->msm) return ZKT_OK;
    if (c->curve == ZKT_CURVE_BN254) return msm_launch_tails<Bn254Curve>(c);
    return msm_launch_tails<Bls381Curve>(c);
}
int msm_begin_many(zkt_ctx* c, int k, const void* const* d_scalars, const size_t* ns, int mont, const int* slots, const int* tbls,
                   bool grouped, const std::function<int(int)>& ready) {
    for (int at = 0; at < k;) {
        const int kk = grouped ? std::min(MSM_BATCH, k - at) : 1;
        for (int j = at; j < at + kk && ready; ++j)
            if (int rc = ready(j)) return rc;
        const int rc = grouped ? msm_begin_batch(c, kk, d_scalars + at, ns + at, mont, slots + at, tbls + at)
                               : msm_begin(c, d_scalars[at], ns[at], 0, mont, slots[at], tbls[at]);
        if (rc) return rc;
        at += kk;
    }
    return msm_flush_tails(c);
}
int msm_end(zkt_ctx* c, int slot, uint64_t* out_xy) {
    if (c->curve == ZKT_CURVE_BN254) {
        Affine<Bn254Fq> a;
        int rc = msm_collect<Bn254Curve>(c, slot, &a);
        if (rc) return rc;
        memcpy(out_xy, a.x.v, 32);
        memcpy(out_xy + 4, a.y.v, 32);
        return ZKT_OK;
    }
    Affine<Bls381Fq> a;
    int rc = msm_collect<Bls381Curve>(c, slot, &a);
    if (rc) return rc;
    memcpy(out_xy, a.x.v, 48);
    memcpy(out_xy + 6, a.y.v, 48);
    return ZKT_OK;
}

int msm_end_sharded(zkt_ctx* c, const int* slots, const bool* have, int k, uint64_t* out_xy ) {
    if (c->curve == ZKT_CURVE_BN254) {
        std::vector<Affine<Bn254Fq>> a(k);
        int rc = msm_collect_sharded<Bn254Curve>(c, slots, have, k, a.data());
        if (rc) return rc;
        for (int j = 0; j < k; ++j) {
            memcpy(out_xy + 12 * j, a[j].x.v, 32);
            memcpy(out_xy + 12 * j + 4, a[j].y.v, 32);
        }
        return ZKT_OK;
    }
    std::vector<Affine<Bls381Fq>> a(k);
    int rc = msm_collect_sharded<Bls381Curve>(c, slots, have, k, a.data());
    if (rc) return rc;
    for (int j = 0; j < k; ++j) {
        memcpy(out_xy + 12 * j, a[j].x.v, 48);
        memcpy(out_xy + 12 * j + 6, a[j].y.v, 48);
    }
    return ZKT_OK;
}
void msm_slice(zkt_ctx* c, size_t* off, size_t* count, size_t* total) {
    *off = c->msm ? c->msm->slice_off : 0;
    *count = c->msm ? c->msm->count : 0;
    *total = c->msm ? c->msm->total : 0;
}
// ... 304 lines not shown
```

### zkt-plonk_amd/csrc/msm.hpp

```cpp
#pragma once
#include "ctx.hpp"

#include <functional>

namespace zkt {

constexpr int MSM_CHUNK_MIN = 16;
constexpr int MSM_R2_BLOCKS = 1;
constexpr int MSM_MAX_Y = 24;

struct MsmWindows {
    int W;
    uint8_t width[40];
    uint16_t start[40];
};

struct MsmPlan {
    MsmWindows win{};
    int W = 0, c = 0;
    int dig = 0;
    uint32_t Bw = 0;
    uint32_t keys = 0;
    uint32_t lb = 8;
    int lcols = 8;
// ... 20 lines not shown

constexpr int MSM_TAIL_BATCH = 6;
struct MsmTailBatch {
    const uint32_t* offsets[MSM_TAIL_BATCH];
    const uint32_t* params[MSM_TAIL_BATCH];
    const void* pieces[MSM_TAIL_BATCH];
    void* buckets[MSM_TAIL_BATCH];
    uint32_t* heavy[MSM_TAIL_BATCH];
    void* rowcol[MSM_TAIL_BATCH];
    void* partials[MSM_TAIL_BATCH];
};

constexpr int MSM_HEAVY = 32;
constexpr int MSM_HEAVY_BLOCKS = 64;

struct WireBases {
    std::shared_ptr<DevShared> mem;
    void* table[3] = {};
    uint32_t* u[3] = {};
    size_t cnt[3] = {};
    bool use[3] = {};
    bool elim[3] = {};
    bool has_c[3] = {};
    bool elim_wanted = false;
    std::vector<size_t> pi_pos;
    bool built = false;
    bool stale = false;
    const void* w[3] = {};
    size_t n_rows = 0, n_vars = 0;
    int log_n = -1;
    uint64_t srs_generation = 0;
    uint64_t digest[2] = {};
};
constexpr int MSM_TBL_WIRE = 2;

struct LagrangeTable {
    std::shared_ptr<DevShared> lag_mem;
    void* table2 = nullptr;
    size_t count2 = 0;
    int lag_log_n = -1;
    bool lag_failed = false;
};

struct MsmState : LagrangeTable {
    size_t count = 0;
    size_t slice_off = 0, total = 0;
    MsmPlan plan;
    uint32_t* heavy[11] = {};
    std::shared_ptr<DevShared> table_mem;
    void* table = nullptr;
    WireBases wb;
    DevBuf wb_scalars[3];
    uint64_t* wb_dig = nullptr;
    uint64_t* wb_pin = nullptr;
    const void* tbl_table(int tbl) const { return tbl >= MSM_TBL_WIRE ? wb.table[tbl - MSM_TBL_WIRE] : tbl ? table2 : table; }
    size_t tbl_count(int tbl) const {
        return tbl >= MSM_TBL_WIRE ? wb.cnt[tbl - MSM_TBL_WIRE] + (wb.has_c[tbl - MSM_TBL_WIRE] ? 1 : 0) + 2 : tbl ? count2 : count;
    }
    uint32_t* params[11] = {};
    uint32_t* vals2 = nullptr;
    void* pairs = nullptr;
    uint32_t* bin_offs = nullptr;
    uint32_t* bin_aux = nullptr;
    uint32_t *bin_start = nullptr, *tile_start = nullptr;
    void* tile_desc = nullptr;
    uint32_t *cnt2 = nullptr, *pos2 = nullptr;
    uint32_t* chunk_bucket = nullptr;
    MsmBatch strides{};
    uint32_t* offsets[11] = {};
    void* pieces[11] = {};
    static constexpr int SLOTS = 11;
    void* buckets[SLOTS] = {};
    void* rowcol[SLOTS] = {};
    void* host_result[SLOTS] = {};
    void* host_result_dev[SLOTS] = {};
    size_t acc_lds = 0;
    size_t acc_threads = 196608;
    hipStream_t side = nullptr;
    hipEvent_t ev_main[SLOTS] = {}, ev_done[SLOTS] = {};
    bool pending[SLOTS] = {};
    bool defer_tails = false;
    int tail_wait[SLOTS] = {};
    int n_tail_wait = 0;
    ~MsmState() {
        for (int i = 0; i < SLOTS; ++i) {
            if (host_result[i]) (void)hipHostFree(host_result[i]);
            if (ev_main[i]) (void)hipEventDestroy(ev_main[i]);
            if (ev_done[i]) (void)hipEventDestroy(ev_done[i]);
        }
        if (side) (void)hipStreamDestroy(side);
        if (wb_pin) (void)hipHostFree(wb_pin);
    }
};

struct MsmBasesState {
    DevBuf bases;
    DevBuf scalars;
    DevBuf vals, pairs, bin_offs, bin_aux, bin_start, tile_start, tile_desc, cnt2, pos2, chunk_bucket;
    DevBuf offsets, heavy, params, pieces, buckets, rowcol;
    DevBuf check_points, check_status;
    void* partials = nullptr;
    void* partials_dev = nullptr;
    size_t acc_lds = 0, acc_threads = 0;
    ~MsmBasesState() {
        if (partials) (void)hipHostFree(partials);
    }
};

constexpr size_t MSM_DEFER_MAX = ((size_t)1 << 16) + 64;
constexpr size_t MSM_TAIL_INL_MAX = ((size_t)1 << 18) + 64;

int srs_load(zkt_ctx* c, const void* src, size_t count, bool on_device, size_t slice_off = 0, size_t total = 0);
int srs_generate(zkt_ctx* c, const uint64_t* tau4, size_t count, size_t slice_off = 0, size_t total = 0);
void msm_release(zkt_ctx* c);
bool msm_tables_have_readers(const zkt_ctx* c);
int msm_table_finish(zkt_ctx* c, void* table, size_t count);
int msm_fork(zkt_ctx* child, const zkt_ctx* parent);
void msm_slice(zkt_ctx* c, size_t* off, size_t* count, size_t* total);
int msm_g1_dev(zkt_ctx* c, const void* d_scalars, size_t n, size_t base_off, int mont, uint64_t* out_xy, int* out_inf);
int msm_bases(zkt_ctx* c, const void* bases, bool bases_on_device, const void* scalars, bool scalars_on_device, size_t n, int mont,
              uint64_t* out_xy, int* out_inf);
int msm_bases_scratch(zkt_ctx* c, MsmBasesState** out);
int msm_begin(zkt_ctx* c, const void* d_scalars, size_t n, size_t base_off, int mont, int slot, int tbl = 0);
int msm_begin_batch(zkt_ctx* c, int k, const void* const* d_scalars, const size_t* ns, int mont, const int* slots, const int* tbls);
int msm_begin_many(zkt_ctx* c, int k, const void* const* d_scalars, const size_t* ns, int mont, const int* slots, const int* tbls,
                   bool grouped, const std::function<int(int)>& ready = {});
int msm_end(zkt_ctx* c, int slot, uint64_t* out_xy);
int msm_end_sharded(zkt_ctx* c, const int* slots, const bool* have, int k, uint64_t* out_xy );
int msm_flush_tails(zkt_ctx* c);
bool msm_defers_tails(const zkt_ctx* c);
bool msm_batches_grouping(const zkt_ctx* c);

int lagrange_ensure(zkt_ctx* c, int log_n);
bool lagrange_ready(const zkt_ctx* c, int log_n);
size_t lagrange_bases(const zkt_ctx* c);
struct WireElimKeys {
    const void* pk[5];
    const size_t* pi_pos;
    size_t n_pi;
};
int wire_bases_prepare(zkt_ctx* c, int log_n, const uint32_t* const* d_idx, size_t n_rows, size_t n_vars, const WireElimKeys* elim = nullptr);
bool wire_bases_use(const zkt_ctx* c, int k);
int wire_bases_route(const zkt_ctx* c, int k);
int wire_bases_digest(zkt_ctx* c, const uint32_t* const* d_idx, size_t n_rows);
int wire_bases_lens(zkt_ctx* c, const uint32_t* d_lens);
int wire_bases_scalars(zkt_ctx* c, int k, const void* d_vars, const void* d_blinders, size_t n, const void** out, size_t* len);
bool wire_bases_check(zkt_ctx* c, int k, size_t n);
void wire_bases_drop(zkt_ctx* c);

}
```

### zkt-plonk_amd/csrc/poly.hip

```cpp
#include "poly.hpp"
#include "hostinv.hpp"

namespace zkt {

template <class P>
ZKT_D Fe<P> arg_fe(const uint32_t* w) {
    Fe<P> r;
#pragma unroll
    for (int i = 0; i < 8; ++i) r.v[i] = w[i];
    return r;
}

template <class P>
__global__ void k_mul_vec(const Fe<P>* a, const Fe<P>* b, Fe<P>* o, size_t n) {
    size_t i = (size_t)blockIdx.x * blockDim.x + threadIdx.x;
    if (i < n) fe_store<P>(o + i, fe_mul<P>(fe_load<P>(a + i), fe_load<P>(b + i)));
}

template <class P>
__global__ void k_trim_len(const Fe<P>* p, size_t lo, size_t n, uint32_t* len, int skip_if_set, Fe<P>* zero_at,
                           int zero_count) {
    if (zero_at && blockIdx.x == 0 && (int)threadIdx.x < zero_count) fe_store<P>(zero_at + threadIdx.x, fe_zero<P>());
    if (skip_if_set && *len != 0) return;
    size_t i = lo + (size_t)blockIdx.x * blockDim.x + threadIdx.x;
// ... 345 lines not shown
}

constexpr int TB_THREADS = 1024;
template <class P>
ZKT_D uint32_t wg_trim_len(const Fe<P>* p, size_t n, uint32_t* best) {
    const int t = threadIdx.x;
    __syncthreads();
    if (t == 0) *best = 0;
    __syncthreads();
    for (size_t hi = n; hi > 0;) {
        const size_t lo = hi > (size_t)TB_THREADS ? hi - TB_THREADS : 0;
        const size_t i = lo + t;
        uint32_t v = 0;
        if (i < hi && !fe_is_zero<P>(fe_load<P>(p + i))) v = (uint32_t)(i + 1);
#pragma unroll
        for (int d = 32; d >= 1; d >>= 1) {
            uint32_t o = __shfl_down(v, d);
            v = o > v ? o : v;
        }
        if ((t & 63) == 0 && v) atomicMax(best, v);
        __syncthreads();
        const uint32_t found = *best;
        __syncthreads();
        if (found) return found;
        hi = lo;
    }
    return 0;
}
struct TrimBlindJob {
    void* poly;
    const void* bl;
    uint32_t* len;
    int k;
};
struct TrimBlindArgs {
    TrimBlindJob job[NTT_MAX_BATCH];
};
template <class P>
__global__ __launch_bounds__(TB_THREADS) void k_trim_blind(TrimBlindArgs a, size_t n, int zero_count) {
    __shared__ uint32_t best;
    const TrimBlindJob j = a.job[blockIdx.x];
    Fe<P>* p = (Fe<P>*)j.poly;
    const int t = threadIdx.x;
    if (t < zero_count) fe_store<P>(p + n + t, fe_zero<P>());
    if (j.k < 0) return;
    const uint32_t L = wg_trim_len<P>(p, n, &best);
    if (t == 0) *j.len = L;
    Fe<P> b = fe_zero<P>();
    if (t < j.k) {
        b = fe_load<P>((const Fe<P>*)j.bl + t);
        fe_store<P>(p + L + t, b);
    }
    __syncthreads();
    if (t < j.k) fe_store<P>(p + t, fe_sub<P>(fe_load<P>(p + t), b));
}

template <class P>
__global__ void k_lagrange_scalars(const Fe<P>* ev, size_t n, const uint32_t* len, const Fe<P>* bl, int k, const Fe<P>* roots,
                                   Fe<P> ninv, Fe<P>* D) {
    const size_t i = (size_t)blockIdx.x * blockDim.x + threadIdx.x;
    if (i >= n + (size_t)k) return;
    const size_t L = k ? (size_t)*len : n;
    if (i >= n) {
        const size_t t = i - n;
        Fe<P> acc = fe_zero<P>();
        for (int j = 0; j < k; ++j)
            if (L + j == n + t) acc = fe_add<P>(acc, fe_load<P>(bl + j));
        fe_store<P>(D + i, acc);
        return;
    }
    Fe<P> e0 = fe_load<P>(ev + i), e1 = (i + 1 < n) ? fe_load<P>(ev + i + 1) : fe_zero<P>();
    if (L != n) {
        for (int j = 0; j < k; ++j) {
            const size_t q = (L + j) & (n - 1);
            if (q == (size_t)j) continue;
            const Fe<P> b = fe_load<P>(bl + j);
            e0 = fe_add<P>(e0, fe_mul<P>(b, fe_sub<P>(fe_load<P>(roots + ((i * q) & (n - 1))), fe_load<P>(roots + ((i * j) & (n - 1))))));
            if (i + 1 < n)
                e1 = fe_add<P>(e1, fe_mul<P>(b, fe_sub<P>(fe_load<P>(roots + (((i + 1) * q) & (n - 1))),
                                                           fe_load<P>(roots + (((i + 1) * j) & (n - 1))))));
        }
    }
    fe_store<P>(D + i, fe_mul<P>(fe_sub<P>(e0, e1), ninv));
}

struct FxArg {
    uint32_t l[9];
};
struct QuotientDev {
    const void *a, *b, *c, *pi, *z1, *z2, *t, *h1, *h2;
    const void *q_m, *q_l, *q_r, *q_o, *q_c, *q_lookup, *q_table, *sigma1, *sigma2, *sigma3, *x, *l1;
    void* out;
    FxArg beta, delta, alpha_k3, alpha2, alpha3_opd_k2, alpha3_k2, alpha4, alpha5;
    FxArg gamma, epsilon, eopd;
    FxArg zh_inv[4];
    uint64_t n4;
    uint64_t first, count;
    const uint32_t* pi_tab;
    uint32_t n_pi_direct;
    uint32_t G, cls, next_off;
    const void *z1_next, *z2_next, *t_next, *h1_next;
    uint64_t cls_stride;
};
template <class P>
ZKT_D Fx<P> arg_fx(const FxArg& w) {
    Fx<P> r;
#pragma unroll
    for (int i = 0; i < FxP<P>::L; ++i) r.l[i] = w.l[i];
    return r;
}

template <class P>
__global__ __launch_bounds__(256) void k_quotient(QuotientDev q) {
    static_assert(FxP<P>::L == 9, "scalar field limbs");
    typedef Fx<P> X;
    const uint64_t i = q.first + (uint64_t)blockIdx.x * blockDim.x + threadIdx.x;
    if (i >= q.first + q.count) return;
    const uint64_t j = (i + q.next_off < q.n4) ? i + q.next_off : i + q.next_off - q.n4;
    const uint64_t coff = (uint64_t)blockIdx.y * q.cls_stride;
    const uint32_t cls = q.cls + blockIdx.y;
#define LD(ptr, idx) fx_unpack<P>(fe_load<P>((const Fe<P>*)(ptr) + coff + (idx)))
    const X beta = arg_fx<P>(q.beta), delta = arg_fx<P>(q.delta), gamma = arg_fx<P>(q.gamma);
    const X a = LD(q.a, i), b = LD(q.b, i), c = LD(q.c, i);
    X acc = fx_mul2_inl<P>(fx_mul<P>(a, b), LD(q.q_m, i), c, LD(q.q_o, i));
    acc = fx_add<P>(acc, fx_mul2_inl<P>(a, LD(q.q_l, i), b, LD(q.q_r, i)));
    const X l1 = LD(q.l1, i);
    if (q.pi_tab) {
        X pi = fx_zero<P>();
#pragma unroll 1
        for (uint32_t e = 0; e < q.n_pi_direct; e += 2) {
            X v[2], l[2];
#pragma unroll
            for (int h = 0; h < 2; ++h) {
                const uint32_t* ent = q.pi_tab + (size_t)(e + h) * 10;
                const bool live = e + h < q.n_pi_direct;
                const uint64_t rot = live ? ent[0] : 0;
                const uint64_t at = (i >= rot) ? i - rot : i + q.n4 - rot;
                l[h] = LD(q.l1, at);
#pragma unroll
                for (int w = 0; w < 9; ++w) v[h].l[w] = live ? ent[1 + w] : 0u;
            }
            pi = fx_add<P>(pi, fx_mul2_inl<P>(v[0], l[0], v[1], l[1]));
        }
        acc = fx_add<P>(acc, fx_add<P>(LD(q.q_c, i), pi));
    } else {
        acc = fx_add<P>(acc, fx_add<P>(LD(q.q_c, i), LD(q.pi, i)));
    }
    const X z1 = LD(q.z1, i), z1n = LD(q.z1_next, j);
    const X ag = fx_add<P>(a, gamma), bg = fx_add<P>(b, gamma), cg = fx_add<P>(c, gamma);
    const X one = fx_const_to_ark<P>();
    {
        const X bx = fx_mul<P>(LD(q.x, i), beta);
        const X d2 = fx_dbl<P>(bx), d4 = fx_dbl<P>(d2), d8 = fx_dbl<P>(d4);
        const X ak3 = arg_fx<P>(q.alpha_k3);
        X p1 = fx_mul<P>(z1, ak3);
        p1 = fx_mul<P>(p1, fx_add<P>(bx, ag));
        p1 = fx_mul<P>(p1, fx_add<P>(fx_sub<P, 2>(d8, bx), bg));
        X p2 = fx_mul<P>(z1n, ak3);
        p2 = fx_mul<P>(p2, fx_add<P>(fx_mul<P>(LD(q.sigma1, i), beta), ag));
        p2 = fx_mul<P>(p2, fx_add<P>(fx_mul<P>(LD(q.sigma2, i), beta), bg));
        const X p12 = fx_mul2_inl<P>(p1, fx_add<P>(fx_add<P>(fx_add<P>(d8, d4), bx), cg), fx_sub_lazy<P, 3>(fx_zero<P>(), p2),
                                     fx_add<P>(fx_mul<P>(LD(q.sigma3, i), beta), cg));
        acc = fx_add<P>(acc, p12);
    }
    {
        const X eps = arg_fx<P>(q.epsilon), eopd = arg_fx<P>(q.eopd);
// ... 462 lines not shown
int scan_add(zkt_ctx* c, const void* in, void* out, size_t n, bool reverse, void* d_tmp) { ZKT_DISPATCH(c, scan_add_t, in, out, n, reverse, d_tmp); }

template <class P> static int z_combine_t(zkt_ctx* c, const void* pn, const void* sd, const uint32_t* inv, void* out, size_t n) {
    hipLaunchKernelGGL(k_z_combine<P>, dim3(nblocks(n)), dim3(256), 0, c->stream, (const Fe<P>*)pn, (const Fe<P>*)sd, host_fe<P>(inv), (Fe<P>*)out, n);
    ZKT_HIP(c, hipGetLastError());
    return ZKT_OK;
}
int z_combine(zkt_ctx* c, const void* pn, const void* sd, const uint32_t inv_total[8], void* out, size_t n) { ZKT_DISPATCH(c, z_combine_t, pn, sd, inv_total, out, n); }

static size_t scan_tmp_elems(size_t n) {
    size_t nb = (n + SC_BLK - 1) / SC_BLK, need = 1;
    while (nb > 1) {
        need += 2 * nb;
        nb = (nb + SC_BLK - 1) / SC_BLK;
    }
    return need;
}
size_t grand_product_tmp_elems(size_t n) { return 2 * scan_tmp_elems(n); }
template <class P> static int grand_product_scan_t(zkt_ctx* c, const ZTermsArgs& a, int which, void* pn, void* sd, void* tmp,
                                                   const void** d_total_den, bool totals_later) {
    const size_t n = a.n;
    if (n == 0 || (n & (n - 1))) return set_err(c, ZKT_ERR_INVALID_ARGUMENT, "grand product: n must be a power of two");
    const size_t nb = (n + SC_BLK - 1) / SC_BLK;
    Fe<P>* tn = (Fe<P>*)tmp;
    Fe<P>* td = tn + scan_tmp_elems(n);
    if (which == 1)
        hipLaunchKernelGGL((k_z_terms_scan<P, 1>), dim3((unsigned)nb, 2), dim3(256), 0, c->stream, a, (Fe<P>*)pn, (Fe<P>*)sd, tn, td);
    else
        hipLaunchKernelGGL((k_z_terms_scan<P, 2>), dim3((unsigned)nb, 2), dim3(256), 0, c->stream, a, (Fe<P>*)pn, (Fe<P>*)sd, tn, td);
    ZKT_HIP(c, hipGetLastError());
    if (nb > 1 && !totals_later) {
        int rc;
        if ((rc = scan_t<P, OpMul>(c, tn, tn + nb, nb, false, tn + 2 * nb))) return rc;
        if ((rc = scan_t<P, OpMul>(c, td, td + nb, nb, false, td + 2 * nb))) return rc;
    }
    *d_total_den = nb > 1 ? td + nb + (nb - 1) : td;
    return ZKT_OK;
}
int grand_product_scan(zkt_ctx* c, const ZTermsArgs& a, int which, void* pn_local, void* sd_local, void* d_tmp, const void** d_total_den,
                       bool totals_later) {
    ZKT_DISPATCH(c, grand_product_scan_t, a, which, pn_local, sd_local, d_tmp, d_total_den, totals_later);
}
bool grand_product_totals_fit(size_t n) { return (n + SC_BLK - 1) / SC_BLK <= (size_t)SC_BLK; }
template <class P> static int grand_product_totals2_t(zkt_ctx* c, size_t n, void* tmp1, void* tmp2) {
    const size_t nb = (n + SC_BLK - 1) / SC_BLK;
    if (nb <= 1) return ZKT_OK;
    if (nb > (size_t)SC_BLK) return set_err(c, ZKT_ERR_INVALID_ARGUMENT, "grand product: the block totals need more than one block");
    Fe<P>*tn1 = (Fe<P>*)tmp1, *tn2 = (Fe<P>*)tmp2;
    hipLaunchKernelGGL((k_scan_rows4<P, OpMul>), dim3(1, 4), dim3(256), 0, c->stream, tn1, tn1 + scan_tmp_elems(n), tn2,
                       tn2 + scan_tmp_elems(n), nb);
    ZKT_HIP(c, hipGetLastError());
    return ZKT_OK;
}
int grand_product_totals2(zkt_ctx* c, size_t n, void* d_tmp1, void* d_tmp2) { ZKT_DISPATCH(c, grand_product_totals2_t, n, d_tmp1, d_tmp2); }
template <class P> static int grand_product_combine_t(zkt_ctx* c, const void* pn, const void* sd, const void* tmp, const uint32_t* inv,
                                                      void* out, size_t n) {
    const size_t nb = (n + SC_BLK - 1) / SC_BLK;
    const Fe<P>* tn = (const Fe<P>*)tmp;
    const Fe<P>* td = tn + scan_tmp_elems(n);
    hipLaunchKernelGGL(k_z_apply_combine<P>, dim3((unsigned)nb), dim3(256), 0, c->stream, (const Fe<P>*)pn, (const Fe<P>*)sd, tn + nb, td + nb,
                       host_fe<P>(inv), (Fe<P>*)out, n);
    ZKT_HIP(c, hipGetLastError());
    return ZKT_OK;
}
int grand_product_combine(zkt_ctx* c, const void* pn_local, const void* sd_local, const void* d_tmp, const uint32_t inv_total[8], void* out,
                          size_t n) {
    ZKT_DISPATCH(c, grand_product_combine_t, pn_local, sd_local, d_tmp, inv_total, out, n);
}

template <class P> static int lagrange_scalars_t(zkt_ctx* c, const void* ev, size_t n, const uint32_t* d_len, const void* d_bl, int k,
                                                 const void* roots, void* out) {
    Fe<P> nn = fe_zero<P>();
    nn.v[0] = (uint32_t)(n & 0xffffffffu);
    nn.v[1] = (uint32_t)((uint64_t)n >> 32);
    const Fe<P> ninv = fe_inv_host<P>(fe_to_mont<P>(nn));
    hipLaunchKernelGGL(k_lagrange_scalars<P>, dim3(nblocks(n + (size_t)k)), dim3(256), 0, c->stream, (const Fe<P>*)ev, n, d_len,
                       (const Fe<P>*)d_bl, k, (const Fe<P>*)roots, ninv, (Fe<P>*)out);
    ZKT_HIP(c, hipGetLastError());
    return ZKT_OK;
}
int lagrange_scalars(zkt_ctx* c, const void* ev, size_t n, const uint32_t* d_len, const void* d_blinders, int k, const void* d_roots,
                     void* out) {
    ZKT_DISPATCH(c, lagrange_scalars_t, ev, n, d_len, d_blinders, k, d_roots, out);
}

template <class P> static FxArg hat_arg(const Fe<P>& s) {
    const Fx<P> h = fx_cond_sub_p<P>(fx_from_ark<P>(s));
    FxArg r;
    for (int i = 0; i < 9; ++i) r.l[i] = h.l[i];
    return r;
}
template <class P> static FxArg ark_arg(const Fe<P>& s) {
    const Fx<P> h = fx_unpack<P>(s);
    FxArg r;
    for (int i = 0; i < 9; ++i) r.l[i] = h.l[i];
    return r;
}
template <class P> static int quotient_t(zkt_ctx* c, const QuotientArgs& a) {
    ProfScope prof(c, "quotient");
    auto get = [](const uint32_t* w) { Fe<P> r; for (int i = 0; i < 8; ++i) r.v[i] = w[i]; return r; };
    const Fe<P> alpha = get(a.alpha), beta = get(a.beta), gamma = get(a.gamma), delta = get(a.delta), eps = get(a.epsilon);
    const Fe<P> k2 = fe_from_u32<P>(1u << 10), k3 = fe_from_u32<P>(1u << 15);
    const Fe<P> a2 = fe_sqr<P>(alpha), a3 = fe_mul<P>(a2, alpha), a4 = fe_mul<P>(a3, alpha), a5 = fe_mul<P>(a4, alpha);
    const Fe<P> opd = fe_add<P>(delta, fe_one<P>());
    QuotientDev q{};
    q.a = a.a; q.b = a.b; q.c = a.c; q.pi = a.pi; q.z1 = a.z1; q.z2 = a.z2; q.t = a.t; q.h1 = a.h1; q.h2 = a.h2;
    q.q_m = a.q_m; q.q_l = a.q_l; q.q_r = a.q_r; q.q_o = a.q_o; q.q_c = a.q_c; q.q_lookup = a.q_lookup; q.q_table = a.q_table;
    q.sigma1 = a.sigma1; q.sigma2 = a.sigma2; q.sigma3 = a.sigma3; q.x = a.x; q.l1 = a.l1; q.out = a.out;
    q.beta = hat_arg<P>(beta);
    q.delta = hat_arg<P>(delta);
    q.alpha_k3 = hat_arg<P>(fe_mul<P>(alpha, k3));
    q.alpha2 = hat_arg<P>(a2);
    q.alpha3_opd_k2 = hat_arg<P>(fe_mul<P>(fe_mul<P>(a3, opd), k2));
    q.alpha3_k2 = hat_arg<P>(fe_mul<P>(a3, k2));
    q.alpha4 = hat_arg<P>(a4);
    q.alpha5 = hat_arg<P>(a5);
    q.gamma = ark_arg<P>(gamma);
    q.epsilon = ark_arg<P>(eps);
    q.eopd = ark_arg<P>(fe_mul<P>(eps, opd));
    for (int k = 0; k < 4; ++k) q.zh_inv[k] = hat_arg<P>(get(a.zh_inv[k]));
    q.n4 = a.n4;
    q.pi_tab = a.pi_tab;
    q.n_pi_direct = a.n_pi_direct;
    if (a.G <= 1) {
        q.G = 1; q.cls = 0; q.next_off = 4;
        q.z1_next = a.z1; q.z2_next = a.z2; q.t_next = a.t; q.h1_next = a.h1;
    } else {
        q.G = a.G; q.cls = a.cls; q.next_off = a.next_off;
        q.z1_next = a.z1_next; q.z2_next = a.z2_next; q.t_next = a.t_next; q.h1_next = a.h1_next;
    }
    if (a.pi_tab && a.n_pi_direct > (uint32_t)QUOTIENT_PI_DIRECT_MAX)
        return set_err(c, ZKT_ERR_INVALID_ARGUMENT, "too many direct public inputs");
    q.first = a.first;
    q.count = a.count ? a.count : a.n4 - a.first;
    if (q.first + q.count > a.n4) return set_err(c, ZKT_ERR_INVALID_ARGUMENT, "quotient range outside the vectors");
    const unsigned ncls = a.ncls > 1 ? a.ncls : 1;
    if (ncls > 1 && (a.G <= 1 || a.cls + ncls > a.G)) return set_err(c, ZKT_ERR_INVALID_ARGUMENT, "quotient classes outside the coset");
    q.cls_stride = ncls > 1 ? a.cls_stride : 0;
    hipLaunchKernelGGL(k_quotient<P>, dim3(nblocks(q.count), ncls), dim3(256), 0, c->stream, q);
    ZKT_HIP(c, hipGetLastError());
    return ZKT_OK;
}
template <class P> static int to_hat_t(zkt_ctx* c, void* v, size_t n, int k32) {
    if (k32 == 0) hipLaunchKernelGGL((k_to_hat<P, 0>), dim3(nblocks(n)), dim3(256), 0, c->stream, (Fe<P>*)v, n);
    else hipLaunchKernelGGL((k_to_hat<P, 1>), dim3(nblocks(n)), dim3(256), 0, c->stream, (Fe<P>*)v, n);
    ZKT_HIP(c, hipGetLastError());
    return ZKT_OK;
}
int to_hat_form(zkt_ctx* c, void* v, size_t n, int k32) { ZKT_DISPATCH(c, to_hat_t, v, n, k32); }
int quotient_pointwise(zkt_ctx* c, const QuotientArgs& a) { ZKT_DISPATCH(c, quotient_t, a); }

template <class P>
__global__ void k_interleave(const Fe<P>* in, Fe<P>* out, uint64_t n4, uint32_t log_g, uint64_t piece) {
    const uint64_t t = (uint64_t)blockIdx.x * blockDim.x + threadIdx.x;
    if (t >= n4) return;
    const uint64_t cls = t & ((1u << log_g) - 1), i = t >> log_g;
    const uint64_t j = i / piece, o = i - j * piece;
    fe_store<P>(out + t, fe_load<P>(in + ((j << log_g) + cls) * piece + o));
}
template <class P> static int interleave_t(zkt_ctx* c, const void* in, void* out, size_t n4, uint32_t G, uint32_t chunks) {
    uint32_t lg = 0;
    while ((1u << lg) < G) ++lg;
    const uint64_t m = n4 >> lg;
    if (chunks == 0 || m % chunks) return set_err(c, ZKT_ERR_INVALID_ARGUMENT, "interleave: pieces must divide the class");
    hipLaunchKernelGGL(k_interleave<P>, dim3(nblocks(n4)), dim3(256), 0, c->stream, (const Fe<P>*)in, (Fe<P>*)out, (uint64_t)n4, lg,
                       m / chunks);
// ... 299 lines not shown
```

### zkt-plonk_amd/csrc/poly.hpp

```cpp
#pragma once
#include "ctx.hpp"

namespace zkt {

constexpr int LC_MAX_TERMS = 24;
struct LinCombArgs {
    const void* poly[LC_MAX_TERMS];
    uint64_t len[LC_MAX_TERMS];
    uint32_t scalar[LC_MAX_TERMS][8];
    int nterms;
};

constexpr int EVAL_MAX = 16;
struct EvalArgs {
    const void* poly[EVAL_MAX];
    uint64_t len[EVAL_MAX];
    uint32_t point[EVAL_MAX][8];
    int count;
    uint8_t table[EVAL_MAX];
};

struct QuotientArgs {
    const void *a, *b, *c, *pi, *z1, *z2, *t, *h1, *h2;
    const void *q_m, *q_l, *q_r, *q_o, *q_c, *q_lookup, *q_table, *sigma1, *sigma2, *sigma3, *x, *l1;
    void* out;
    uint32_t alpha[8], beta[8], gamma[8], delta[8], epsilon[8];
    uint32_t zh_inv[4][8];
    uint64_t n4;
    const uint32_t* pi_tab;
    uint32_t n_pi_direct;
    uint32_t G, cls, next_off;
    const void *z1_next, *z2_next, *t_next, *h1_next;
    uint64_t first, count;
    uint32_t ncls;
    uint64_t cls_stride;
};
constexpr int QUOTIENT_PI_DIRECT_MAX = 16;

struct ZTermsArgs {
    const void *a, *b, *c, *s1, *s2, *s3, *roots;
    const void *f, *t, *h1, *h2;
    void *num, *den;
    uint32_t beta[8], gamma[8], delta[8], epsilon[8];
    uint64_t n;
};

int poly_mul_vec(zkt_ctx* c, const void* a, const void* b, void* out, size_t n);
int poly_set_zero(zkt_ctx* c, void* p, size_t n_elems);
int poly_trim_len(zkt_ctx* c, const void* p, size_t n, uint32_t* d_len, void* zero_at = nullptr, int zero_count = 0);
int poly_copy_pad(zkt_ctx* c, const void* d_in, size_t len, void* out, size_t n);
int poly_gather_pad(zkt_ctx* c, const void* d_values, size_t n_vars, const uint32_t* d_idx, size_t rows, void* out, size_t n,
                    uint32_t* d_status);
int poly_add_blinders(zkt_ctx* c, void* p, const uint32_t* d_len, const void* d_blinders, int k, size_t cap);
int poly_lincomb(zkt_ctx* c, const LinCombArgs& a, void* out, size_t n);
struct TrimBlindSpec {
    void* poly;
    const void* d_blinders;
    uint32_t* d_len;
    int k;
};
int poly_trim_blind(zkt_ctx* c, const TrimBlindSpec* jobs, int nb, size_t n, int zero_count);
int lagrange_scalars(zkt_ctx* c, const void* ev, size_t n, const uint32_t* d_len, const void* d_blinders, int k, const void* d_roots,
                     void* out);
int poly_eval_many(zkt_ctx* c, const EvalArgs& a, void* d_partials, void* d_results, void* d_powers);
int poly_eval_open_tables(zkt_ctx* c, const EvalArgs& a, const uint32_t z0[8], const uint32_t z0_inv[8], const uint32_t z1[8],
                          const uint32_t z1_inv[8], size_t len, void* d_partials, void* d_results, void* d_powers);
int z1_terms(zkt_ctx* c, const ZTermsArgs& a);
int z2_terms(zkt_ctx* c, const ZTermsArgs& a);
int scan_mul(zkt_ctx* c, const void* in, void* out, size_t n, bool reverse, void* d_tmp );
int scan_add(zkt_ctx* c, const void* in, void* out, size_t n, bool reverse, void* d_tmp);
int z_combine(zkt_ctx* c, const void* pn, const void* sd, const uint32_t inv_total[8], void* out, size_t n);
size_t grand_product_tmp_elems(size_t n);
int grand_product_scan(zkt_ctx* c, const ZTermsArgs& a, int which, void* pn_local, void* sd_local, void* d_tmp, const void** d_total_den,
                       bool totals_later = false);
bool grand_product_totals_fit(size_t n);
int grand_product_totals2(zkt_ctx* c, size_t n, void* d_tmp1, void* d_tmp2);
int grand_product_combine(zkt_ctx* c, const void* pn_local, const void* sd_local, const void* d_tmp, const uint32_t inv_total[8], void* out,
                          size_t n);
int quotient_pointwise(zkt_ctx* c, const QuotientArgs& a);
int to_hat_form(zkt_ctx* c, void* v, size_t n, int k32);
int quotient_interleave(zkt_ctx* c, const void* in, void* out, size_t n4, uint32_t G, uint32_t chunks = 1);
int quotient_split_blind(zkt_ctx* c, const void* q, size_t n, const void* d_b0b1, void* q_lo, void* q_mid, void* q_hi,
                         uint32_t* d_status, bool fused = false, bool closed = false);
constexpr int QC_WIN = 14, QC_WIN_POLYS = 6;
int quotient_classes_of_coset(zkt_ctx* c, const void* in, void* out, size_t n);
int quotient_gather_windows(zkt_ctx* c, const void* const* polys, size_t first, void* out);
int quotient_classes_combine(zkt_ctx* c, void* q, size_t n, const uint32_t* vinv, const uint32_t* u, const uint32_t* g3);
int quotient_classes_close(zkt_ctx* c, void* q, size_t n, const uint32_t* vinv, const uint32_t* u, const uint32_t* g3, void* q_lo,
                           void* q_mid, void* q_hi);
int open_witness(zkt_ctx* c, const void* p, size_t len, const uint32_t z[8], const uint32_t z_inv[8], void* d_tmp_a, void* d_tmp_b,
                 void* d_scan_tmp, void* out, void* d_powers );
size_t open_witness_powers(size_t maxlen);
constexpr int OPEN_PW_ROW = 257;
int open_elems(size_t len);
size_t open_blocks(size_t len);
int open_pow_tables(zkt_ctx* c, const uint32_t z[8], const uint32_t z_inv[8], void* d_powers, size_t len);
int open_divide(zkt_ctx* c, const void* t, size_t len, void* d_tmp, void* d_scan_tmp, void* out, const void* d_powers,
                void* d_total = nullptr);
int open_combine(zkt_ctx* c, const LinCombArgs& a, void* out, size_t len, const void* d_powers);
int poly_sum_rows(zkt_ctx* c, const void* d_partials, int nblk, int rows, void* d_out);
int sigma_build(zkt_ctx* c, int log_n, const uint32_t* d_w_l, const uint32_t* d_w_r, const uint32_t* d_w_o, size_t n_rows, size_t n_vars,
                void* const* d_sigma);
size_t sigma_scratch_bytes(int log_n, size_t n_rows);
int sigma_enqueue(zkt_ctx* c, int log_n, const uint32_t* d_w_l, const uint32_t* d_w_r, const uint32_t* d_w_o, size_t n_rows, size_t n_vars,
                  void* const* d_sigma, void* d_scratch, uint32_t* d_flag);
struct WitnessCheckKeys {
    int log_n;
    const void* pk[5];
    const void* q_lookup_ev;
    const void* sigma_ev[3];
};
int selector_evals_enqueue(zkt_ctx* c, int log_n, const void* const* pk, void* const* outs);
int witness_check(zkt_ctx* c, const WitnessCheckKeys& keys, const zkt_prove_inputs& in, int flags, zkt_witness_report* out);
int gen_powers(zkt_ctx* c, void* out, size_t n, const uint32_t base[8], const uint32_t scale[8]);
int lookup_count(zkt_ctx* c, const void* f, size_t n, const void* d_sorted_keys, const uint32_t* d_perm, uint32_t nkeys,
                 uint32_t* d_counts, uint32_t* d_status);
int lookup_starts(zkt_ctx* c, const uint32_t* d_base_counts, uint32_t* d_hits, uint32_t nkeys, size_t n, uint32_t* d_even,
                  uint32_t* d_odd, uint32_t* d_status);
int lookup_expand(zkt_ctx* c, const void* d_keys_insertion, const uint32_t* d_starts, uint32_t nkeys, void* out, size_t n);

}
```

### zkt-plonk_amd/csrc/prover.hip

```cpp
#include "ctx.hpp"
#include "hostinv.hpp"
#include <chrono>
#include <cstdio>
#include <cstdlib>
#include "ec.hpp"
#include "keyfile.hpp"
#include "linearisation.hpp"
#include "msm.hpp"
#include "poly.hpp"
#include "quotient_classes.hpp"
#include "transcript.hpp"

#include <algorithm>
#include <functional>
#include <cstring>
#include <memory>
#include <optional>
#include <vector>

namespace zkt {

enum { PK_QM = 0, PK_QL, PK_QR, PK_QO, PK_QC, PK_S1, PK_S2, PK_S3, PK_QLOOKUP, PK_QTABLE, PK_COUNT };
enum { CS_QM = 0, CS_QL, CS_QR, CS_QO, CS_QC, CS_QLOOKUP, CS_QTABLE, CS_S1, CS_S2, CS_S3, CS_X, CS_L1, CS_COUNT };
enum { W_A = 0, W_B, W_C, W_PI, W_Z1, W_Z2, W_T, W_H1, W_H2, W_COUNT };

struct CircuitKeys {
    std::shared_ptr<DevShared> keys_mem;
    void* pk[PK_COUNT] = {};
    size_t pk_len[PK_COUNT] = {};
    void* coset[CS_COUNT] = {};
    void* sigma_ev[3] = {};
    void* q_lookup_ev = nullptr;
    void* roots = nullptr;
    uint32_t zh_inv[4][8] = {};
};
struct ClassTables {
    std::shared_ptr<DevShared> class_mem;
    void* ccoset[CS_COUNT] = {};
    bool ccoset_ready = false;
    uint32_t key_win[4][QCW][8] = {};
    uint32_t qc_gamma[4][8] = {}, qc_vinv[9][8] = {}, qc_g3[3][8] = {};
};

struct CircuitState : CircuitKeys, ClassTables {
    int log_n = 0;
    size_t n = 0;
    int G = 1, cls = 0, log_m = 0;
    size_t m = 0;
    void* wnext[4] = {};
    void* fold = nullptr;
    void* qgather = nullptr;
    bool have[16] = {};
    void* ev[8] = {};
    void* sc[4] = {};
    void* scan_tmp = nullptr;
    void* poly[13] = {};
    void* wcos[W_COUNT] = {};
    void* qev = nullptr;
    void* lag_scalars = nullptr;
    void* lag_scalars_q[3] = {};
    void* small = nullptr;
    uint32_t* status = nullptr;
    uint32_t* lk_u32 = nullptr;
    uint32_t lk_nkeys = 0;
    std::vector<uint32_t> lk_host_keys, lk_host_sorted, lk_host_counts, lk_host_order;
    bool has_next = false, prefetch_same_table = false;
    int prefetch_stage = 0;
    uint64_t prefetch_epoch = 0;
    zkt_prove_inputs next_in{}, prefetch_in{};
    void* poly_alt[3] = {};
    uint32_t* status_alt = nullptr;
    void* lk_keys = nullptr;
    size_t lk_cap = 0;
    void* pinned = nullptr;
    hipStream_t comm_stream = nullptr;
    hipEvent_t ev_piece[ZKT_QUOTIENT_CHUNKS] = {}, ev_gathered = nullptr;
    hipStream_t aux_stream = nullptr;
    hipEvent_t ev_aux_go = nullptr, ev_aux_done = nullptr;
    void* aux_scan_tmp = nullptr;
    void* aux_pw = nullptr;
    hipStream_t copy_stream = nullptr;
    hipEvent_t ev_copy[4] = {};
    void* pinned_pi = nullptr;
    uint32_t* pi_tab = nullptr;
    void* eval_pw = nullptr;
    std::vector<uint64_t> cached_table;
    bool t_cached = false, t_coset_valid = false;
    uint64_t t_srs_generation = 0;
    uint64_t t_commit_xy[12] = {};
    bool wire_route[3] = {};
    bool wire_dense_only = false;
    int wire_elim_force = -1;
    bool use_classes = false;
    void* heads = nullptr;
    void* d_win = nullptr;
    void* pinned_win = nullptr;
    hipEvent_t ev_win = nullptr;
    uint32_t last_u[6][8] = {};
    bool last_u_valid = false;
};

template <class P>
struct HostF {
    using F = Fe<P>;
    static F from_words(const uint64_t* w) {
        F r;
        memcpy(r.v, w, 32);
        return r;
    }
    static void to_le_bytes(const F& mont, uint8_t out[32]) {
        F c = fe_from_mont<P>(mont);
        memcpy(out, c.v, 32);
    }
    static F from_le_bytes(const uint8_t in[32]) {
        F c;
        memcpy(c.v, in, 32);
        return fe_to_mont<P>(c);
    }
};

template <class Q>
static void fq_to_le(const Fe<Q>& mont, uint8_t* out) {
    Fe<Q> c = fe_from_mont<Q>(mont);
    memcpy(out, c.v, Q::N * 4);
}

template <class Q>
static void serialize_point(const Affine<Q>& p, std::vector<uint8_t>& out) {
    const size_t nb = Q::N * 4;
    std::vector<uint8_t> b(nb, 0);
    if (aff_is_inf<Q>(p)) {
        b[nb - 1] |= 0x40;
    } else {
        fq_to_le<Q>(p.x, b.data());
        Fe<Q> y = fe_from_mont<Q>(p.y);
        Fe<Q> ny = fe_from_mont<Q>(fe_neg<Q>(p.y));
        bool greater = false;
        for (int i = Q::N - 1; i >= 0; --i) {
            if (y.v[i] != ny.v[i]) {
                greater = y.v[i] > ny.v[i];
                break;
            }
        }
        if (greater) b[nb - 1] |= 0x80;
    }
    out.insert(out.end(), b.begin(), b.end());
}

template <class R>
static void pi_rows(const uint64_t* pi_pos, const uint64_t* pi_vals, size_t n_pi, size_t G, uint32_t* tab) {
    for (size_t i = 0; i < n_pi; ++i) {
        tab[10 * i] = (uint32_t)(4 * pi_pos[i] / G);
        const Fx<R> v = fx_unpack<R>(HostF<R>::from_words(pi_vals + 4 * i));
        for (int w = 0; w < 9; ++w) tab[10 * i + 1 + w] = v.l[w];
    }
}

static void quotient_vectors(QuotientArgs& q, void* const cs[CS_COUNT], void* const w[W_COUNT], size_t off) {
    auto at = [&](void* const* v, int k) { return (const void*)((const char*)v[k] + off); };
    q.q_m = at(cs, CS_QM); q.q_l = at(cs, CS_QL); q.q_r = at(cs, CS_QR); q.q_o = at(cs, CS_QO); q.q_c = at(cs, CS_QC);
    q.q_lookup = at(cs, CS_QLOOKUP); q.q_table = at(cs, CS_QTABLE); q.x = at(cs, CS_X); q.l1 = at(cs, CS_L1);
    q.sigma1 = at(cs, CS_S1); q.sigma2 = at(cs, CS_S2); q.sigma3 = at(cs, CS_S3);
    q.a = at(w, W_A); q.b = at(w, W_B); q.c = at(w, W_C); q.pi = at(w, W_PI);
    q.z1 = at(w, W_Z1); q.z2 = at(w, W_Z2); q.t = at(w, W_T); q.h1 = at(w, W_H1); q.h2 = at(w, W_H2);
}
static QuotientArgs quotient_args(const CircuitState& S, void* const w[W_COUNT], const void* alpha, const void* beta,
                                  const void* gamma, const void* delta, const void* epsilon) {
    QuotientArgs q{};
    quotient_vectors(q, S.coset, w, 0);
    memcpy(q.alpha, alpha, 32); memcpy(q.beta, beta, 32); memcpy(q.gamma, gamma, 32);
    memcpy(q.delta, delta, 32); memcpy(q.epsilon, epsilon, 32);
    memcpy(q.zh_inv, S.zh_inv, sizeof(q.zh_inv));
    return q;
}

constexpr int WIRE_ELIM_MIN_LOG_N = 17;
constexpr int QUOTIENT_CLASSES_MIN_LOG_N = 18;

template <class C>
struct Prover {
    using R = typename C::Fr;
    using Q = typename C::Fq;
    using F = Fe<R>;
    using H = HostF<R>;

    zkt_ctx* c;
    CircuitState& S;
    HostTranscript& tr;
    const size_t cap;
    void *const d_partials, *const d_results;
    Prover(zkt_ctx* ctx, CircuitState& st, HostTranscript& t)
        : c(ctx), S(st), tr(t), cap(st.n + 8), d_partials((char*)st.small + 64 * 32), d_results((char*)st.small + 32 * 32) {
        trace_on = exp_env("ZKT_HOST_TRACE") != nullptr;
    }
    bool copy_fenced = false;
    bool trace_on = false;
    std::vector<std::pair<const char*, std::chrono::steady_clock::time_point>> marks;
    void mark(const char* what) {
        if (trace_on) marks.emplace_back(what, std::chrono::steady_clock::now());
    }
    void dump_marks() {
        if (!trace_on || marks.empty()) return;
        for (size_t i = 1; i < marks.size(); ++i)
            fprintf(stderr, "[zkt host] %-28s %8.1f us\n", marks[i].first,
                    std::chrono::duration<double, std::micro>(marks[i].second - marks[i - 1].second).count());
        marks.clear();
    }

    void tr_commit(const char* label, const Affine<Q>& p) {
        uint8_t x[64], y[64];
        bool inf = aff_is_inf<Q>(p);
        if (!inf) {
            fq_to_le<Q>(p.x, x);
            fq_to_le<Q>(p.y, y);
        }
        tr.append_commitment(label, x, y, Q::N * 4, inf);
    }
    void tr_scalar(const char* label, const F& v) {
        uint8_t b[32];
        H::to_le_bytes(v, b);
        tr.append_scalars(label, b, 1, 32, true);
    }
    F tr_challenge(const char* label) {
        uint8_t b[32];
        tr.challenge_scalar(label, R::BITS, b);
        return H::from_le_bytes(b);
    }
    static void put(uint32_t dst[8], const F& v) { memcpy(dst, v.v, 32); }

    std::optional<ProfScope> idle;
    void wait_begin() {
        if (c->prof_on && !idle) idle.emplace(c, "host_wait");
    }
    void wait_end() { idle.reset(); }

    int commit_begin(const void* d_poly, size_t len, int slot) {
        if (!c->sharded()) return msm_begin(c, d_poly, len, 0, 1, slot);
        size_t off, cnt, total;
        msm_slice(c, &off, &cnt, &total);
        if (len > total)
            return set_err(c, ZKT_ERR_TOO_MANY_COEFFICIENTS, "TooManyCoefficients: polynomial longer than the committer key");
        S.have[slot] = len > off;
        if (!S.have[slot]) return ZKT_OK;
        const size_t l = std::min(len, off + cnt) - off;
        return msm_begin(c, (const char*)d_poly + off * 32, l, 0, 1, slot);
    }
    struct Pending {
        const void* scalars;
        size_t len;
        int slot, tbl;
    };
    Pending queue[6];
    int n_queue = 0, n_lag_queued = 0;
    bool queueing() const { return !c->sharded() && !c->batch_off && msm_batches_grouping(c); }
    int commit_flush() {
        const int k = n_queue;
        const void* sc[6];
        size_t lens[6];
        int slots[6], tbls[6];
        for (int j = 0; j < k; ++j) {
            sc[j] = queue[j].scalars; lens[j] = queue[j].len; slots[j] = queue[j].slot; tbls[j] = queue[j].tbl;
        }
        n_queue = 0;
        n_lag_queued = 0;
        return msm_begin_many(c, k, sc, lens, 1, slots, tbls, true);
    }
    int commit_push(const void* scalars, size_t len, int slot, int tbl) {
        if (n_queue == 6)
            if (int rc = commit_flush()) return rc;
        queue[n_queue++] = Pending{scalars, len, slot, tbl};
        return ZKT_OK;
    }
    int commit_begin_many(void* const* d_polys, const size_t* lens, const int* slots, int k) {
        for (int j = 0; j < k; ++j) {
            const int rc = queueing() ? commit_push(d_polys[j], lens[j], slots[j], 0) : commit_begin(d_polys[j], lens[j], slots[j]);
            if (rc) return rc;
        }
        return ZKT_OK;
    }
    int commit_evals_begin(const void* ev, const void* d_poly, int blinder_off, int k, int len_slot, int slot) {
        const bool q = queueing();
        if (!lagrange_ready(c, S.log_n) || c->lagrange_off)
            return q ? commit_push(d_poly, S.n + (size_t)k, slot, 0) : commit_begin(d_poly, S.n + (size_t)k, slot);
        if (q && n_lag_queued == 3)
            if (int rc0 = commit_flush()) return rc0;
        void* d = q ? S.lag_scalars_q[n_lag_queued] : S.lag_scalars;
        int rc = lagrange_scalars(c, ev, S.n, S.status + 8 + len_slot, (const char*)S.small + (size_t)blinder_off * 32, k, S.roots, d);
        if (rc) return rc;
        if (!q) return msm_begin(c, d, S.n + (size_t)k, 0, 1, slot, 1);
        ++n_lag_queued;
        return commit_push(d, S.n + (size_t)k, slot, 1);
    }
    int commit_collect(const int* slots, const bool* skip, int k, Affine<Q>* out) {
        wait_begin();
        if (!c->sharded()) {
            for (int j = 0; j < k; ++j) {
                if (skip && skip[j]) continue;
                uint64_t xy[12];
                int rc = msm_end(c, slots[j], xy);
                if (rc) return rc;
                memcpy(out[j].x.v, xy, Q::N * 4);
                memcpy(out[j].y.v, xy + Q::N / 2, Q::N * 4);
            }
            return ZKT_OK;
        }
        bool have[16];
        uint64_t xy[16 * 12];
        for (int j = 0; j < k; ++j) have[j] = !(skip && skip[j]) && S.have[slots[j]];
        int rc = msm_end_sharded(c, slots, have, k, xy);
        if (rc) return rc;
        for (int j = 0; j < k; ++j) {
            if (skip && skip[j]) continue;
            memcpy(out[j].x.v, xy + 12 * j, Q::N * 4);
            memcpy(out[j].y.v, xy + 12 * j + Q::N / 2, Q::N * 4);
        }
        return ZKT_OK;
    }

    int collect_wires(Affine<Q>* cm, int* took = nullptr) {
        for (int k = 0; k < 3; ++k) {
            const bool routed = S.wire_route[k];
            S.wire_route[k] = false;
            if (took) took[k] = 0;
            if (!routed) continue;
            if (wire_bases_check(c, k, S.n)) {
                if (took) took[k] = wire_bases_route(c, k);
                continue;
            }
            static const int slot[1] = {0};
            int rc = msm_begin(c, S.poly[k], S.n + 2, 0, 1, 0);
            if (rc || (rc = commit_collect(slot, nullptr, 1, cm + k))) return rc;
        }
        return ZKT_OK;
    }

    struct PolyJob {
        const void* ev;
        void* poly;
        int blinder_off, k, len_slot;
    };
    int evals_to_blinded_polys(const PolyJob* jobs, int nb) {
        const size_t n = S.n;
        int rc;
        const void* ins[NTT_MAX_BATCH];
        void* outs[NTT_MAX_BATCH];
        size_t lens[NTT_MAX_BATCH];
        for (int y = 0; y < nb; ++y) {
            ins[y] = jobs[y].ev;
            outs[y] = jobs[y].poly;
            lens[y] = n;
        }
        if ((rc = ntt_run_batch(c, S.log_n, 1, 0, nb, ins, lens, outs))) return rc;
        if (c->fused(4)) {
            TrimBlindSpec tb[NTT_MAX_BATCH];
            for (int y = 0; y < nb; ++y)
                tb[y] = TrimBlindSpec{jobs[y].poly, (const char*)S.small + (size_t)jobs[y].blinder_off * 32, S.status + 8 + jobs[y].len_slot,
                                      jobs[y].k > 0 ? jobs[y].k : -1};
            return poly_trim_blind(c, tb, nb, n, 8);
        }
        for (int y = 0; y < nb; ++y) {
            void* poly = jobs[y].poly;
            if (jobs[y].k > 0) {
                if ((rc = poly_trim_len(c, poly, n, S.status + 8 + jobs[y].len_slot, (char*)poly + n * 32, 8))) return rc;
                if ((rc = poly_add_blinders(c, poly, S.status + 8 + jobs[y].len_slot,
                                            (const char*)S.small + (size_t)jobs[y].blinder_off * 32, jobs[y].k, n + 8)))
                    return rc;
            } else {
                ZKT_HIP(c, hipMemsetAsync((char*)poly + n * 32, 0, 8 * 32, c->stream));
            }
        }
        return ZKT_OK;
    }
    int evals_to_blinded_poly(const void* ev, void* poly, int blinder_off, int k, int len_slot) {
        const PolyJob j{ev, poly, blinder_off, k, len_slot};
        return evals_to_blinded_polys(&j, 1);
    }

    int check_status() {
        uint32_t st = 0;
        ZKT_HIP(c, hipMemcpyAsync(&st, S.status, 4, hipMemcpyDeviceToHost, c->stream));
        wait_begin();
        ZKT_HIP(c, hipStreamSynchronize(c->stream));
        if (st & 16u) return set_err(c, ZKT_ERR_INVALID_ARGUMENT, "wire index outside the variable map");
        if (st & 4u) return set_err(c, ZKT_ERR_NOT_IN_TABLE, "ElementNotIndexedInTable: a looked-up value is not in the table");
        if (st & 8u) return set_err(c, ZKT_ERR_INVALID_ARGUMENT, "combine_split: h1/h2 length differs from n");
        if (st & 2u) return set_err(c, ZKT_ERR_QUOTIENT_TOO_SHORT, "quotient degree exceeds 3n+5: the circuit is not satisfied");
        if (st & 1u) return set_err(c, ZKT_ERR_QUOTIENT_TOO_SHORT, "quotient polynomial too short to split (prove.rs:287-300)");
        return ZKT_OK;
    }

    int combine_split(const uint64_t* table, size_t table_len, bool fresh) {
        const size_t n = S.n;
        F* d_keys = (F*)S.lk_keys;
        F* d_sorted = d_keys + S.lk_cap;
        uint32_t* d_perm = S.lk_u32;
        uint32_t* d_base = S.lk_u32 + S.lk_cap;
        uint32_t* d_even = S.lk_u32 + 2 * S.lk_cap;
// ... 245 lines not shown
                if (wire_tables && wire_bases_use(c, k)) {
                    if ((rc = wire_bases_scalars(c, k, d_vars, (const char*)S.small + (size_t)(2 * k) * 32, n, &sc, &len))) return rc;
                    tbl = MSM_TBL_WIRE + k;
                    S.wire_route[k] = true;
                }
                rc = queueing() ? commit_push(sc, len, k, tbl) : tbl ? msm_begin(c, sc, len, 0, 1, k, tbl) : commit_begin(sc, len, k);
                if (rc) return rc;
            }
        }
        if ((rc = commit_flush())) return rc;
        return to_coset_many({W_A, W_B, W_C});
    }

    bool table_is_cached(const zkt_prove_inputs& in) const {
        return S.t_cached && S.t_srs_generation == c->srs_generation && S.cached_table.size() == 4 * in.table_len &&
               (in.table_len == 0 || memcmp(S.cached_table.data(), in.table, in.table_len * 32) == 0);
    }
    int enqueue_table(const zkt_prove_inputs& in, bool with_coset) {
        const size_t n = S.n;
        int rc;
        if (in.table_len >= n) return set_err(c, ZKT_ERR_INVALID_ARGUMENT, "max table size is equal or larger than n");
        S.t_cached = false;
        S.t_coset_valid = false;
        ZKT_HIP(c, hipMemsetAsync(S.ev[3], 0, n * 32, c->stream));
        if (in.table_len) ZKT_HIP(c, hipMemcpyAsync(S.ev[3], in.table, in.table_len * 32, hipMemcpyHostToDevice, c->stream));
        if ((rc = evals_to_blinded_poly(S.ev[3], S.poly[3], 0, 0, 3))) return rc;
        if ((rc = commit_evals_begin(S.ev[3], S.poly[3], 0, 0, 3, 3))) return rc;
        if (with_coset && (rc = to_coset(W_T))) return rc;
        return ZKT_OK;
    }

    int enqueue_round_2(const zkt_prove_inputs& in, bool* same_table_out, bool table_done = false) {
        const size_t n = S.n;
        int rc;
        ProfScope prof_round(c, "round2");
        const bool same_table = !table_done && table_is_cached(in);
        *same_table_out = same_table;
        if (!same_table && !table_done && (rc = enqueue_table(in, false))) return rc;
        if ((rc = poly_mul_vec(c, S.q_lookup_ev, S.ev[2], S.ev[4], n))) return rc;
        if ((rc = combine_split(in.table, in.table_len, !same_table))) return rc;
        {
            const PolyJob jobs[2] = {{S.ev[5], S.poly[4], 6, 3, 4}, {S.ev[6], S.poly[5], 9, 2, 5}};
            if ((rc = evals_to_blinded_polys(jobs, 2))) return rc;
        }
        if ((rc = commit_evals_begin(S.ev[5], S.poly[4], 6, 3, 4, 4))) return rc;
        if ((rc = commit_evals_begin(S.ev[6], S.poly[5], 9, 2, 5, 5))) return rc;
        if ((rc = commit_flush())) return rc;
        if (!S.t_coset_valid && !table_done) return to_coset_many({W_T, W_H1, W_H2});
        return to_coset_many({W_H1, W_H2});
    }

    Challenges<R> ch;
    XiPoint<R> at;
    F ev[EV_COUNT];
    Affine<Q> cm[11], wit[2];
    F w, shifted;
    bool same_table = false, classes = false, pi_direct = false, fused3 = false, fused5 = false;

    int rounds_1_2(const zkt_prove_inputs& in) {
        int rc;
        if (S.prefetch_stage == 2 && S.prefetch_epoch == c->msm_epoch && same_inputs(S.prefetch_in, in)) {
            same_table = S.prefetch_same_table;
            swap_work_sets();
            S.prefetch_stage = 0;
            return ZKT_OK;
        }
        S.prefetch_stage = 0;
        const bool table_first = !table_is_cached(in);
        if (table_first && in.a_evals && !in.wires_on_device) {
            ZKT_HIP(c, hipEventRecord(S.ev_copy[3], c->stream));
            ZKT_HIP(c, hipStreamWaitEvent(S.copy_stream, S.ev_copy[3], 0));
            copy_fenced = true;
        }
        if (table_first && (rc = enqueue_table(in, true))) return rc;
        if ((rc = enqueue_round_1(in))) return rc;
        return enqueue_round_2(in, &same_table, table_first);
    }

    int collect_rounds_1_2(const zkt_prove_inputs& in) {
        static const int slots[6] = {0, 1, 2, 3, 4, 5};
        const bool skip[6] = {false, false, false, same_table, false, false};
        int rc;
        if ((rc = commit_collect(slots, skip, 6, cm))) return rc;
        if ((rc = collect_wires(cm))) return rc;
        mark("wait commits of rounds 1+2");
        if (!same_table) {
            memcpy(S.t_commit_xy, cm[3].x.v, Q::N * 4);
            memcpy(S.t_commit_xy + Q::N / 2, cm[3].y.v, Q::N * 4);
            S.cached_table.assign(in.table, in.table + 4 * in.table_len);
            S.t_cached = true;
            S.t_srs_generation = c->srs_generation;
        } else {
            memcpy(cm[3].x.v, S.t_commit_xy, Q::N * 4);
            memcpy(cm[3].y.v, S.t_commit_xy + Q::N / 2, Q::N * 4);
        }
        return ZKT_OK;
    }

    void* pn2() const { return S.wcos[W_Z1]; }
    void* sd2() const { return (char*)S.wcos[W_Z1] + S.n * 32; }
    int grand_products_begin() {
        const size_t n = S.n;
        int rc;
        ZTermsArgs za{};
        za.a = S.ev[0]; za.b = S.ev[1]; za.c = S.ev[2];
        za.s1 = S.sigma_ev[0]; za.s2 = S.sigma_ev[1]; za.s3 = S.sigma_ev[2]; za.roots = S.roots;
        za.f = S.ev[4]; za.t = S.ev[3]; za.h1 = S.ev[5]; za.h2 = S.ev[6];
        za.num = S.sc[0]; za.den = S.sc[1]; za.n = n;
        put(za.beta, ch.beta); put(za.gamma, ch.gamma); put(za.delta, ch.delta); put(za.epsilon, ch.epsilon);
        F* pin = (F*)S.pinned;
        fused3 = c->fused(2) && grand_product_tmp_elems(n) <= n + 8;
        const void *tot1 = S.sc[3], *tot2 = sd2();
        if (fused3) {
            const bool later = c->fused(32) && grand_product_totals_fit(n);
            if ((rc = grand_product_scan(c, za, 1, S.sc[2], S.sc[3], S.sc[0], &tot1, later))) return rc;
            if ((rc = grand_product_scan(c, za, 2, pn2(), sd2(), S.sc[1], &tot2, later))) return rc;
            if (later && (rc = grand_product_totals2(c, n, S.sc[0], S.sc[1]))) return rc;
        } else {
            if ((rc = z1_terms(c, za))) return rc;
            if ((rc = scan_mul(c, S.sc[0], S.sc[2], n, false, S.scan_tmp))) return rc;
            if ((rc = scan_mul(c, S.sc[1], S.sc[3], n, true, S.scan_tmp))) return rc;
            if ((rc = z2_terms(c, za))) return rc;
            if ((rc = scan_mul(c, S.sc[0], pn2(), n, false, S.scan_tmp))) return rc;
            if ((rc = scan_mul(c, S.sc[1], sd2(), n, true, S.scan_tmp))) return rc;
        }
        ZKT_HIP(c, hipMemcpyAsync(pin, tot1, 32, hipMemcpyDeviceToHost, c->stream));
        ZKT_HIP(c, hipMemcpyAsync(pin + 1, tot2, 32, hipMemcpyDeviceToHost, c->stream));
        return ZKT_OK;
    }
    int grand_products_finish() {
        const size_t n = S.n;
        const F* pin = (const F*)S.pinned;
        int rc;
        if (fe_is_zero<R>(pin[0])) return set_err(c, ZKT_ERR_ZERO_DENOMINATOR, "zero denominator in the permutation grand product");
        if (fe_is_zero<R>(pin[1])) return set_err(c, ZKT_ERR_ZERO_DENOMINATOR, "zero denominator in the lookup grand product");
        const F inv12 = fe_inv_host<R>(fe_mul<R>(pin[0], pin[1]));
        const F inv1 = fe_mul<R>(inv12, pin[1]), inv2 = fe_mul<R>(inv12, pin[0]);
        wait_end();
        if (fused3) {
            if ((rc = grand_product_combine(c, S.sc[2], S.sc[3], S.sc[0], inv1.v, S.ev[7], n))) return rc;
            return grand_product_combine(c, pn2(), sd2(), S.sc[1], inv2.v, S.sc[0], n);
        }
        if ((rc = z_combine(c, S.sc[2], S.sc[3], inv1.v, S.ev[7], n))) return rc;
        return z_combine(c, pn2(), sd2(), inv2.v, S.sc[0], n);
    }

    int gather_windows() {
        const void* const wp[QC_WIN_POLYS] = {S.poly[0], S.poly[1], S.poly[2], S.poly[6], S.poly[7], S.poly[3]};
        if (int rc = quotient_gather_windows(c, wp, S.n - 6, S.d_win)) return rc;
        ZKT_HIP(c, hipMemcpyAsync(S.pinned_win, S.d_win, QC_WIN_POLYS * QC_WIN * 32, hipMemcpyDeviceToHost, c->stream));
        ZKT_HIP(c, hipEventRecord(S.ev_win, c->stream));
        return ZKT_OK;
    }

    int public_inputs(const zkt_prove_inputs& in) {
        const size_t n = S.n;
        int rc;
        for (size_t i = 0; i < in.n_pi; ++i)
            if (in.pi_pos[i] >= n) return set_err(c, ZKT_ERR_INVALID_ARGUMENT, "public input position out of range");
        pi_direct = in.n_pi <= (size_t)QUOTIENT_PI_DIRECT_MAX && S.G <= 4;
        if (pi_direct) {
            uint32_t* tab = (uint32_t*)S.pinned_pi;
            pi_rows<R>(in.pi_pos, in.pi_vals, in.n_pi, classes ? 4 : (size_t)S.G, tab);
            if (in.n_pi)
                ZKT_HIP(c, hipMemcpyAsync(S.pi_tab, tab, in.n_pi * 40, hipMemcpyHostToDevice, c->stream));
            return ZKT_OK;
        }
        ZKT_HIP(c, hipMemsetAsync(S.ev[7], 0, n * 32, c->stream));
        for (size_t i = 0; i < in.n_pi; ++i)
            ZKT_HIP(c, hipMemcpyAsync((char*)S.ev[7] + in.pi_pos[i] * 32, in.pi_vals + 4 * i, 32, hipMemcpyHostToDevice, c->stream));
        if ((rc = evals_to_blinded_poly(S.ev[7], S.poly[8], 0, 0, 8))) return rc;
        return to_coset(W_PI);
    }

    int round_3(const zkt_prove_inputs& in) {
        const size_t n = S.n;
        int rc;
        if ((rc = grand_products_begin())) return rc;
        mark("enqueue grand products");
        if ((rc = check_status())) return rc;
        mark("wait grand products");
        if ((rc = grand_products_finish())) return rc;
        const PolyJob jobs[2] = {{S.ev[7], S.poly[6], 11, 3, 6}, {S.sc[0], S.poly[7], 14, 3, 7}};
        if ((rc = evals_to_blinded_polys(jobs, 2))) return rc;
        if (classes && (rc = gather_windows())) return rc;
        void* const z1p[1] = {S.poly[6]};
        const size_t z1l[1] = {n + 3};
        static const int slots[2] = {0, 1};
        if ((rc = commit_begin_many(z1p, z1l, slots, 1))) return rc;
        if ((rc = commit_evals_begin(S.sc[0], S.poly[7], 14, 3, 7, 1))) return rc;
        if ((rc = commit_flush())) return rc;
        if ((rc = to_coset_many({W_Z1, W_Z2}))) return rc;
        if ((rc = public_inputs(in))) return rc;
        return commit_collect(slots, nullptr, 2, cm + 6);
    }


    int quotient_on_classes(QuotientArgs q, bool* closed) {
        const size_t n = S.n;
        const int log_n = S.log_n;
        int rc;
        q.G = 4;
        q.next_off = 1;
        q.n4 = n;
        const bool grid = c->fused(8);
        for (int j = 0; j < (grid ? 1 : 3); ++j) {
            const size_t off = (size_t)j * n * 32;
            quotient_vectors(q, S.ccoset, S.wcos, off);
            q.cls = (uint32_t)j;
            q.ncls = grid ? 3 : 0;
            q.cls_stride = n;
            q.z1_next = q.z1; q.z2_next = q.z2; q.t_next = q.t; q.h1_next = q.h1;
            q.out = (char*)S.qev + off;
            if ((rc = quotient_pointwise(c, q))) return rc;
        }
        if (grid) {
            const int codes[3] = {ntt_class_code(log_n + 2, 0), ntt_class_code(log_n + 2, 1), ntt_class_code(log_n + 2, 2)};
            const void* in = S.qev;
            void* out = S.qev;
            if ((rc = ntt_run_classes(c, log_n, 1, codes, 1, &in, &n, &out, n, n))) return rc;
        } else {
            for (int j = 0; j < 3; ++j) {
                void* e = (char*)S.qev + (size_t)j * n * 32;
                if ((rc = ntt_run(c, log_n, 1, ntt_class_code(log_n + 2, j), e, n, e))) return rc;
            }
        }
        ZKT_HIP(c, hipEventSynchronize(S.ev_win));
        const uint32_t* pw = (const uint32_t*)S.pinned_win;
        QuotientWindows W{};
        W.a = pw; W.b = pw + QCW * 8; W.c = pw + 2 * QCW * 8; W.z1 = pw + 3 * QCW * 8; W.z2 = pw + 4 * QCW * 8;
        W.t = pw + 5 * QCW * 8;
        W.sigma1 = &S.key_win[0][0][0]; W.sigma2 = &S.key_win[1][0][0]; W.sigma3 = &S.key_win[2][0][0];
        W.q_lookup = &S.key_win[3][0][0];
        F u[6];
        quotient_top_coefficients<R>(log_n, W, ch.alpha, ch.beta, ch.delta, u);
        for (int e = 0; e < 6; ++e) put(S.last_u[e], u[e]);
        S.last_u_valid = true;
        *closed = c->fused(16);
        if (*closed)
            return quotient_classes_close(c, S.qev, n, &S.qc_vinv[0][0], &S.last_u[0][0], &S.qc_g3[0][0], S.poly[9], S.poly[10], S.poly[11]);
        return quotient_classes_combine(c, S.qev, n, &S.qc_vinv[0][0], &S.last_u[0][0], &S.qc_g3[0][0]);
    }

    int quotient_sharded(QuotientArgs q) {
        const size_t n = S.n;
        int rc;
        q.G = (uint32_t)S.G;
        q.cls = (uint32_t)S.cls;
        q.next_off = S.G <= 4 ? 4u / (uint32_t)S.G : (uint32_t)((S.cls + 4) >> 3);
        q.z1_next = S.G == 8 ? S.wnext[0] : q.z1;
        q.z2_next = S.G == 8 ? S.wnext[1] : q.z2;
        q.t_next = S.G == 8 ? S.wnext[2] : q.t;
        q.h1_next = S.G == 8 ? S.wnext[3] : q.h1;
        const size_t pieces = ZKT_QUOTIENT_CHUNKS;
        if (!(comm_async_available(c) && S.comm_stream && S.m % pieces == 0 && S.m / pieces >= 1024)) {
            q.out = (char*)S.qgather + (size_t)S.cls * S.m * 32;
            if ((rc = quotient_pointwise(c, q))) return rc;
            if ((rc = comm_all_gather_dev(c, q.out, S.qgather, S.m * 32))) return rc;
            return quotient_interleave(c, S.qgather, S.qev, 4 * n, (uint32_t)S.G);
        }
        const size_t mp = S.m / pieces;
        for (size_t j = 0; j < pieces; ++j) {
            char* recv = (char*)S.qgather + j * (size_t)S.G * mp * 32;
            char* mine = recv + (size_t)S.cls * mp * 32;
            q.first = j * mp;
            q.count = mp;
            q.out = mine - q.first * 32;
            if ((rc = quotient_pointwise(c, q))) return rc;
            ZKT_HIP(c, hipEventRecord(S.ev_piece[j], c->stream));
            ZKT_HIP(c, hipStreamWaitEvent(S.comm_stream, S.ev_piece[j], 0));
            if ((rc = comm_all_gather_async(c, mine, recv, mp * 32, S.comm_stream))) return rc;
        }
        ZKT_HIP(c, hipEventRecord(S.ev_gathered, S.comm_stream));
        ZKT_HIP(c, hipStreamWaitEvent(c->stream, S.ev_gathered, 0));
        return quotient_interleave(c, S.qgather, S.qev, 4 * n, (uint32_t)S.G, (uint32_t)pieces);
    }

// ... 782 lines not shown
void zkt_transcript_challenge_scalar(zkt_transcript* t, const char* label, int fr_bits, uint8_t out_le32[32]) {
    t->impl->challenge_scalar(label, (size_t)fr_bits, out_le32);
}
int zkt_transcript_challenge_bytes(zkt_transcript* t, const char* label, uint8_t* out, size_t len) {
    if (!t->merlin) return ZKT_ERR_INVALID_ARGUMENT;
    t->merlin->challenge_bytes(label, out, len);
    return ZKT_OK;
}
int zkt_transcript_append_message(zkt_transcript* t, const char* label, const uint8_t* msg, size_t len) {
    if (!t->merlin) return ZKT_ERR_INVALID_ARGUMENT;
    t->merlin->append_message(label, msg, len);
    return ZKT_OK;
}

int zkt_circuit_load(zkt_ctx* c, int log_n, const uint64_t* const* pk_polys, const size_t* pk_lens) {
    if (!c || !pk_polys || !pk_lens) return set_err(c, ZKT_ERR_INVALID_ARGUMENT, "null pointer");
    (void)hipSetDevice(c->device);
    if (c->curve == ZKT_CURVE_BN254) return circuit_load_t<Bn254Curve>(c, log_n, pk_polys, pk_lens);
    return circuit_load_t<Bls381Curve>(c, log_n, pk_polys, pk_lens);
}

static int check_sharded_key(zkt_ctx* c) {
    if (!c->sharded()) return ZKT_OK;
    size_t off = 0, cnt = 0, total = 0, lo = 0, hi = 0;
    zkt::msm_slice(c, &off, &cnt, &total);
    (void)zkt_shard_range(total, c->comm.vt.rank, c->comm.vt.world, &lo, &hi);
    if (off != lo || off + cnt != hi)
        return set_err(c, ZKT_ERR_INVALID_ARGUMENT,
                       "sharded proof: this rank must load powers zkt_shard_range(total, rank, world) with zkt_srs_load_slice");
    if (c->circuit && c->circuit->G != c->comm.vt.world)
        return set_err(c, ZKT_ERR_NOT_LOADED, "the circuit was loaded for another communicator");
    return ZKT_OK;
}

static int prove_impl(zkt_ctx* c, const zkt_prove_inputs* in, HostTranscript& tr, uint8_t* out, size_t cap, size_t* len) {
    if (!c->circuit) return set_err(c, ZKT_ERR_NOT_LOADED, "no circuit loaded (zkt_circuit_load)");
    if (!c->msm) return set_err(c, ZKT_ERR_NOT_LOADED, "no SRS loaded (zkt_srs_load)");
    if (int rc0 = check_sharded_key(c)) return rc0;
    (void)hipSetDevice(c->device);
    if (!c->lagrange_off)
        if (int rc1 = lagrange_ensure(c, c->circuit->log_n)) return rc1;
    std::vector<uint8_t> proof;
    const int rc = c->curve == ZKT_CURVE_BN254 ? run_prover<Bn254Curve>(c, *in, tr, proof) : run_prover<Bls381Curve>(c, *in, tr, proof);
    if (rc) {
        c->circuit->has_next = false;
        c->circuit->prefetch_stage = 0;
        return rc;
    }
    if (len) *len = proof.size();
    if (proof.size() > cap) return set_err(c, ZKT_ERR_INVALID_ARGUMENT, "proof buffer too small");
    memcpy(out, proof.data(), proof.size());
    return ZKT_OK;
}

int zkt_ctx_set_lagrange(zkt_ctx* c, int on) {
    if (!c) return ZKT_ERR_INVALID_ARGUMENT;
    c->lagrange_off = !on;
    ++c->msm_epoch;
    return ZKT_OK;
}

int zkt_ctx_set_wire_elimination(zkt_ctx* c, int mode) {
    if (!c) return ZKT_ERR_INVALID_ARGUMENT;
    if (mode < 0 || mode > 2) return set_err(c, ZKT_ERR_INVALID_ARGUMENT, "mode: 0 off, 1 automatic, 2 whenever a table can be built");
    c->wire_elim_mode = mode;
    ++c->msm_epoch;
    return ZKT_OK;
}

int zkt_ctx_set_quotient_route(zkt_ctx* c, int mode) {
    if (!c) return ZKT_ERR_INVALID_ARGUMENT;
    if (mode < 0 || mode > 2) return set_err(c, ZKT_ERR_INVALID_ARGUMENT, "mode: 0 automatic, 1 three classes, 2 the whole coset");
    c->quotient_route = mode;
    return ZKT_OK;
}

int zkt_ctx_set_fused_passes(zkt_ctx* c, int mode) {
    if (!c) return ZKT_ERR_INVALID_ARGUMENT;
    if (mode < 0 || mode > 2) return set_err(c, ZKT_ERR_INVALID_ARGUMENT, "mode: 0 automatic, 1 fused, 2 one launch per step");
    c->fused_passes = mode;
    return ZKT_OK;
}

int zkt_debug_quotient_top(zkt_ctx* c, uint64_t* out_u, int* out_on_classes) {
    if (!c || !out_u) return set_err(c, ZKT_ERR_INVALID_ARGUMENT, "null pointer");
    if (!c->circuit) return set_err(c, ZKT_ERR_NOT_LOADED, "no circuit loaded (zkt_circuit_load)");
    const CircuitState& S = *c->circuit;
    if (out_on_classes) *out_on_classes = S.use_classes ? 1 : 0;
    memcpy(out_u, S.last_u, sizeof(S.last_u));
    return ZKT_OK;
}

int zkt_debug_quotient_coeffs(zkt_ctx* c, uint64_t* out, size_t count) {
    if (!c || !out) return set_err(c, ZKT_ERR_INVALID_ARGUMENT, "null pointer");
    if (!c->circuit) return set_err(c, ZKT_ERR_NOT_LOADED, "no circuit loaded (zkt_circuit_load)");
    const CircuitState& S = *c->circuit;
    if (count > 4 * S.n) return set_err(c, ZKT_ERR_INVALID_ARGUMENT, "the quotient vector holds 4n elements");
    (void)hipSetDevice(c->device);
    ZKT_HIP(c, hipStreamSynchronize(c->stream));
    ZKT_HIP(c, hipMemcpy(out, S.qev, count * 32, hipMemcpyDeviceToHost));
    return ZKT_OK;
}

extern "C++" template <class R>
static void debug_quotient_classes_host_t(int log_n, const uint64_t* windows, const uint64_t* challenges, uint64_t* out_u,
                                          uint64_t* out_consts) {
    typedef Fe<R> F;
    const QuotientClassConsts<R> q = quotient_class_consts<R>(log_n);
    for (int k = 0; k < 4; ++k) memcpy(out_consts + 4 * k, q.gamma[k].v, 32);
    for (int k = 0; k < 9; ++k) memcpy(out_consts + 4 * (4 + k), q.vinv[k].v, 32);
    for (int k = 0; k < 3; ++k) memcpy(out_consts + 4 * (13 + k), q.g3[k].v, 32);
    const uint32_t* w = (const uint32_t*)windows;
    QuotientWindows W{};
    const uint32_t** slot[10] = {&W.a, &W.b, &W.c, &W.z1, &W.z2, &W.t, &W.sigma1, &W.sigma2, &W.sigma3, &W.q_lookup};
    for (int k = 0; k < 10; ++k) *slot[k] = w + (size_t)k * QCW * 8;
    F alpha, beta, delta, u[6];
    memcpy(alpha.v, challenges, 32);
    memcpy(beta.v, challenges + 4, 32);
    memcpy(delta.v, challenges + 8, 32);
    quotient_top_coefficients<R>(log_n, W, alpha, beta, delta, u);
    for (int e = 0; e < 6; ++e) memcpy(out_u + 4 * e, u[e].v, 32);
}

int zkt_debug_quotient_classes_host(int curve, int log_n, const uint64_t* windows, const uint64_t* challenges, uint64_t* out_u,
                                    uint64_t* out_consts) {
    if (!windows || !challenges || !out_u || !out_consts) return ZKT_ERR_INVALID_ARGUMENT;
    if (curve == ZKT_CURVE_BN254) {
        if (log_n < 3 || log_n + 2 > Bn254Fr::TWO_ADICITY) return ZKT_ERR_INVALID_DOMAIN_SIZE;
        debug_quotient_classes_host_t<Bn254Fr>(log_n, windows, challenges, out_u, out_consts);
    } else if (curve == ZKT_CURVE_BLS12_381) {
        if (log_n < 3 || log_n + 2 > Bls381Fr::TWO_ADICITY) return ZKT_ERR_INVALID_DOMAIN_SIZE;
        debug_quotient_classes_host_t<Bls381Fr>(log_n, windows, challenges, out_u, out_consts);
    } else {
        return ZKT_ERR_INVALID_ARGUMENT;
    }
    return ZKT_OK;
}

int zkt_lagrange_info(zkt_ctx* c, int* log_n, size_t* bases) {
    if (!c) return ZKT_ERR_INVALID_ARGUMENT;
    const bool ready = c->circuit && lagrange_ready(c, c->circuit->log_n) && !c->lagrange_off;
    if (log_n) *log_n = ready ? c->circuit->log_n : -1;
    if (bases) *bases = ready ? lagrange_bases(c) : 0;
    return ZKT_OK;
}

int zkt_commit_evals_dev(zkt_ctx* c, const void* d_evals, const uint64_t* blinders, int k, int path, uint64_t* out_xy,
                         int* out_is_infinity) {
    if (!c || !d_evals || !out_xy || (k > 0 && !blinders)) return set_err(c, ZKT_ERR_INVALID_ARGUMENT, "null pointer");
    if (k < 0 || k > 3) return set_err(c, ZKT_ERR_INVALID_ARGUMENT, "0 .. 3 blinders");
    if (!c->circuit) return set_err(c, ZKT_ERR_NOT_LOADED, "no circuit loaded (the domain comes from it)");
    if (!c->msm) return set_err(c, ZKT_ERR_NOT_LOADED, "no SRS loaded (zkt_srs_load)");
    if (c->sharded()) return set_err(c, ZKT_ERR_INVALID_ARGUMENT, "not available on a sharded key");
    (void)hipSetDevice(c->device);
    CircuitState& S = *c->circuit;
    const size_t n = S.n;
    int rc;
    if (path == 1) {
        if ((rc = lagrange_ensure(c, S.log_n))) return rc;
        if (!lagrange_ready(c, S.log_n)) return set_err(c, ZKT_ERR_NOT_LOADED, "the key is too short for the Lagrange-basis table");
    } else if (path != 0) {
        return set_err(c, ZKT_ERR_INVALID_ARGUMENT, "path: 0 coefficients, 1 Lagrange basis");
    }
    c->circuit->prefetch_stage = 0;
    uint32_t* d_len = S.status + 8 + 12;
    void* d_bl = (char*)S.lag_scalars + (n + 8) * 32;
    void* poly = S.poly[12];
    ZKT_HIP(c, hipMemsetAsync(d_len, 0, 4, c->stream));
    if (k) ZKT_HIP(c, hipMemcpyAsync(d_bl, blinders, (size_t)k * 32, hipMemcpyHostToDevice, c->stream));
    if ((rc = ntt_run(c, S.log_n, 1, 0, d_evals, n, poly))) return rc;
    if (c->fused(4)) {
        const TrimBlindSpec tb{poly, d_bl, d_len, k};
        if ((rc = poly_trim_blind(c, &tb, 1, n, 8))) return rc;
    } else {
        if ((rc = poly_trim_len(c, poly, n, d_len, (char*)poly + n * 32, 8))) return rc;
        if (k && (rc = poly_add_blinders(c, poly, d_len, d_bl, k, n + 8))) return rc;
    }
    if (path == 0) return msm_g1_dev(c, poly, n + (size_t)k, 0, 1, out_xy, out_is_infinity);
    if ((rc = lagrange_scalars(c, d_evals, n, d_len, d_bl, k, S.roots, S.lag_scalars))) return rc;
    if ((rc = msm_begin(c, S.lag_scalars, n + (size_t)k, 0, 1, 0, 1))) return rc;
    uint64_t xy[12] = {};
    if ((rc = msm_end(c, 0, xy))) return rc;
    const size_t words = c->curve == ZKT_CURVE_BN254 ? 8 : 12;
    memcpy(out_xy, xy, words * 8);
    if (out_is_infinity) {
        bool any = false;
        for (size_t i = 0; i < words; ++i) any = any || xy[i] != 0;
        *out_is_infinity = any ? 0 : 1;
    }
    return ZKT_OK;
}

int zkt_circuit_setup(zkt_ctx* c, int log_n, const uint64_t* const* evals, const size_t* eval_lens, int evals_on_device,
                      uint64_t* out_commitments, int* out_is_infinity) {
    if (!c || !evals || !eval_lens || !out_commitments) return set_err(c, ZKT_ERR_INVALID_ARGUMENT, "null pointer");
    if (!c->msm) return set_err(c, ZKT_ERR_NOT_LOADED, "no SRS loaded (zkt_srs_load)");
    (void)hipSetDevice(c->device);
    if (log_n < 3 || log_n > 26) return set_err(c, ZKT_ERR_INVALID_DOMAIN_SIZE, "circuit bound out of range");
    if (int rc0 = check_sharded_key(c)) return rc0;
    const unsigned mask = evals_on_device ? (1u << PK_COUNT) - 1u : 0u;
    if (c->curve == ZKT_CURVE_BN254)
        return circuit_setup_t<Bn254Curve>(c, log_n, evals, eval_lens, mask, out_commitments, out_is_infinity);
    return circuit_setup_t<Bls381Curve>(c, log_n, evals, eval_lens, mask, out_commitments, out_is_infinity);
}

int zkt_circuit_setup_wiring(zkt_ctx* c, int log_n, const uint64_t* const* evals, const size_t* eval_lens, int evals_on_device,
                             const uint32_t* w_l, const uint32_t* w_r, const uint32_t* w_o, size_t n_rows, size_t n_vars,
                             int wiring_on_device, uint64_t* out_commitments, int* out_is_infinity) {
    if (!c || !evals || !eval_lens || !out_commitments) return set_err(c, ZKT_ERR_INVALID_ARGUMENT, "null pointer");
    if (!c->msm) return set_err(c, ZKT_ERR_NOT_LOADED, "no SRS loaded (zkt_srs_load)");
    (void)hipSetDevice(c->device);
    const int max_log_n = (c->curve == ZKT_CURVE_BN254 ? Bn254Fr::TWO_ADICITY : Bls381Fr::TWO_ADICITY) - 2;
    if (log_n < 3 || log_n > 25 || log_n > max_log_n)
        return set_err(c, ZKT_ERR_INVALID_DOMAIN_SIZE, "circuit bound out of range");
    if (int rc0 = check_sharded_key(c)) return rc0;
    if (int rf = refuse_if_forked(c, "loading a circuit")) return rf;
    circuit_release(c);
    const size_t n = (size_t)1 << log_n;
    if (n_rows > n) return set_err(c, ZKT_ERR_INVALID_ARGUMENT, "more wiring rows than the domain size");
    for (int k = PK_S1; k <= PK_S3; ++k)
        if (evals[k] || eval_lens[k])
            return set_err(c, ZKT_ERR_INVALID_ARGUMENT, "zkt_circuit_setup_wiring makes sigma1..3 itself: entries 5, 6, 7 must be NULL / 0");
    if (n_rows && (!w_l || !w_r || !w_o)) return set_err(c, ZKT_ERR_INVALID_ARGUMENT, "null wiring pointer");
    void* held[6] = {};
    auto release = [&]() {
        (void)hipStreamSynchronize(c->stream);
        for (void* p : held) dev_free(c, p);
    };
    int rc = ZKT_OK;
    for (int k = 0; k < 3 && !rc; ++k) rc = dev_alloc(c, &held[k], n * 32);
    const uint32_t* w[3] = {w_l, w_r, w_o};
    if (!wiring_on_device && n_rows) {
        for (int k = 0; k < 3 && !rc; ++k) {
            rc = dev_alloc(c, &held[3 + k], n_rows * 4);
            if (!rc && hipMemcpyAsync(held[3 + k], w[k], n_rows * 4, hipMemcpyHostToDevice, c->stream) != hipSuccess)
                rc = set_err(c, ZKT_ERR_HIP, "uploading the wiring failed");
            w[k] = (const uint32_t*)held[3 + k];
        }
    }
    if (!rc) rc = sigma_build(c, log_n, w[0], w[1], w[2], n_rows, n_vars, held);
    if (!rc) {
        const uint64_t* ev[PK_COUNT];
        size_t lens[PK_COUNT];
        for (int k = 0; k < PK_COUNT; ++k) { ev[k] = evals[k]; lens[k] = eval_lens[k]; }
        unsigned mask = evals_on_device ? (1u << PK_COUNT) - 1u : 0u;
        for (int k = 0; k < 3; ++k) {
            ev[PK_S1 + k] = (const uint64_t*)held[k];
            lens[PK_S1 + k] = n;
            mask |= 1u << (PK_S1 + k);
        }
        rc = c->curve == ZKT_CURVE_BN254 ? circuit_setup_t<Bn254Curve>(c, log_n, ev, lens, mask, out_commitments, out_is_infinity)
                                         : circuit_setup_t<Bls381Curve>(c, log_n, ev, lens, mask, out_commitments, out_is_infinity);
    }
    release();
    return rc;
}

int zkt_circuit_check_witness(zkt_ctx* c, const zkt_prove_inputs* in, int flags, zkt_witness_report* out) {
    if (!c) return ZKT_ERR_INVALID_ARGUMENT;
    if (!in || !out) return set_err(c, ZKT_ERR_INVALID_ARGUMENT, "null pointer");
    if (!c->circuit) return set_err(c, ZKT_ERR_NOT_LOADED, "no circuit loaded (zkt_circuit_load)");
    if (flags & ~ZKT_CHECK_WIRING) return set_err(c, ZKT_ERR_INVALID_ARGUMENT, "unknown flag bits");
    const CircuitState& S = *c->circuit;
    const size_t n = S.n;
    if (in->n_rows > n) return set_err(c, ZKT_ERR_INVALID_ARGUMENT, "more rows than the circuit bound");
// ... 261 lines not shown
```

Measured before the change: 70.62 proofs/s.

## Add sparse short-list MSM path for Lagrange commitments with mostly-zero evaluations

Adds a path that compacts the nonzero Lagrange-basis scalars into a short index/scalar list, then groups them into buckets with a single-kernel grouping step instead of the full n-length grouping pass. It targets commitments such as lookup/permutation-related vectors whose evaluations are mostly zero, so grouping and accumulation touch only the nonzero entries. If the count exceeds the cap (n/8, at most 8192), the host detects this after the fact through mapped memory, marks that commitment slot as given up, and redoes the full MSM. This costs an extra recompute and synchronization on overflow.

```diff
diff --git a/include/zkt_plonk.h b/include/zkt_plonk.h
--- a/include/zkt_plonk.h
+++ b/include/zkt_plonk.h
@@ -104,6 +104,8 @@
 int zkt_lagrange_info(zkt_ctx* ctx, int* log_n, size_t* bases);
 int zkt_commit_evals_dev(zkt_ctx* ctx, const void* d_evals, const uint64_t* blinders, int k, int path, uint64_t* out_xy_mont,
                          int* out_is_infinity);
+int zkt_ctx_set_short_msm(zkt_ctx* ctx, int mode);
+int zkt_debug_short_msm(zkt_ctx* ctx, uint64_t* out_taken, uint64_t* out_fell_back);
 
 enum {
     ZKT_TRANSCRIPT_MERLIN = 0,
diff --git a/shim/src/ffi.rs b/shim/src/ffi.rs
--- a/shim/src/ffi.rs
+++ b/shim/src/ffi.rs
@@ -110,6 +110,7 @@
     pub fn zkt_ctx_set_wire_elimination(ctx: *mut ZktCtx, mode: c_int) -> c_int;
     pub fn zkt_ctx_set_quotient_route(ctx: *mut ZktCtx, mode: c_int) -> c_int;
     pub fn zkt_ctx_set_fused_passes(ctx: *mut ZktCtx, mode: c_int) -> c_int;
+    pub fn zkt_ctx_set_short_msm(ctx: *mut ZktCtx, mode: c_int) -> c_int;
     pub fn zkt_lagrange_info(ctx: *mut ZktCtx, log_n: *mut c_int, bases: *mut usize) -> c_int;
     pub fn zkt_circuit_load(ctx: *mut ZktCtx, log_n: c_int, pk_polys: *const *const u64, pk_lens: *const usize) -> c_int;
     pub fn zkt_circuit_load_file(ctx: *mut ZktCtx, pk_path: *const c_char, log_n: c_int) -> c_int;
diff --git a/zkt-plonk_amd/_lib.py b/zkt-plonk_amd/_lib.py
--- a/zkt-plonk_amd/_lib.py
+++ b/zkt-plonk_amd/_lib.py
@@ -1539,6 +1539,16 @@
         self._L.zkt_ctx_set_fused_passes.argtypes = [ctypes.c_void_p, ctypes.c_int]
         self.check(self._L.zkt_ctx_set_fused_passes(self._h, int(mode)))
 
+    def set_short_msm(self, mode: int = 1):
+        self._L.zkt_ctx_set_short_msm.argtypes = [ctypes.c_void_p, ctypes.c_int]
+        self.check(self._L.zkt_ctx_set_short_msm(self._h, int(mode)))
+
+    def debug_short_msm(self):
+        taken, back = ctypes.c_uint64(0), ctypes.c_uint64(0)
+        self._L.zkt_debug_short_msm.argtypes = [ctypes.c_void_p, ctypes.POINTER(ctypes.c_uint64), ctypes.POINTER(ctypes.c_uint64)]
+        self.check(self._L.zkt_debug_short_msm(self._h, ctypes.byref(taken), ctypes.byref(back)))
+        return int(taken.value), int(back.value)
+
     def debug_quotient_top(self):
         u = np.zeros((6, 4), dtype=np.uint64)
         on = ctypes.c_int(0)
diff --git a/zkt-plonk_amd/csrc/capi.hip b/zkt-plonk_amd/csrc/capi.hip
--- a/zkt-plonk_amd/csrc/capi.hip
+++ b/zkt-plonk_amd/csrc/capi.hip
@@ -234,6 +234,7 @@
     c->batch_off = exp_env("ZKT_MSM_NO_BATCH") != nullptr;
     c->aux_off = exp_env("ZKT_NO_AUX") != nullptr;
     if (const char* parts = exp_env("ZKT_FUSED_PARTS")) c->fused_parts = atoi(parts) & 63;
+    if (const char* parts = exp_env("ZKT_SHORT_MSM_PARTS")) c->short_parts = atoi(parts) & 1;
     c->curve = curve_id;
     c->device = device_id;
     if (hipStreamCreateWithFlags(&c->stream, hipStreamNonBlocking) != hipSuccess) {
@@ -259,6 +260,8 @@
     c->quotient_route = parent->quotient_route;
     c->fused_passes = parent->fused_passes;
     c->fused_parts = parent->fused_parts;
+    c->short_msm = parent->short_msm;
+    c->short_parts = parent->short_parts;
     c->batch_off = parent->batch_off;
     c->aux_off = parent->aux_off;
     c->ntt_plans = parent->ntt_plans;
diff --git a/zkt-plonk_amd/csrc/ctx.hpp b/zkt-plonk_amd/csrc/ctx.hpp
--- a/zkt-plonk_amd/csrc/ctx.hpp
+++ b/zkt-plonk_amd/csrc/ctx.hpp
@@ -76,6 +76,8 @@
     int fused_passes = 0;
     int fused_parts = 63;
     bool fused(int part) const { return fused_passes != 2 && (fused_parts & part); }
+    int short_msm = 1;
+    int short_parts = 1;
     std::shared_ptr<zkt::CircuitState> circuit;
     std::vector<std::pair<void*, size_t>> owned;
 };
diff --git a/zkt-plonk_amd/csrc/msm.hip b/zkt-plonk_amd/csrc/msm.hip
--- a/zkt-plonk_amd/csrc/msm.hip
+++ b/zkt-plonk_amd/csrc/msm.hip
@@ -593,6 +593,128 @@
     }
     __syncthreads();
     for (uint32_t j = threadIdx.x; j < cnt; j += MSM_L2S_THREADS) vals[delta[skey[j]] + j] = sval[j];
+}
+
+constexpr int MSM_SHORT_WGS = 64;
+constexpr int MSM_SHORT_PER = 4;
+constexpr int MSM_SHORT_KEYS = 1024 * MSM_SHORT_PER;
+template <class C>
+__global__ __launch_bounds__(1024) void k_msm_short_group(const uint32_t* list_idx, const Fe<typename C::Fr>* list_sc, const uint32_t* count,
+                                                          uint32_t* count_next, uint32_t cap, int mont, MsmWindows win, uint32_t B,
+                                                          uint32_t keys_per, uint32_t acc_threads, uint32_t lanes_fold, uint32_t* vals,
+                                                          uint32_t* chunk_bucket, uint32_t* entries_out, MsmBatch bt) {
+    using R = typename C::Fr;
+    extern __shared__ uint32_t lds[];
+    uint32_t* hist = lds;
+    uint32_t* cursor = lds + keys_per;
+    __shared__ uint32_t wsum[16];
+    __shared__ uint32_t s_below, s_total, nbig;
+    __shared__ uint32_t big[256][3];
+    const uint32_t raw = *count;
+    const uint32_t M = raw <= cap ? raw : 0u;
+    const uint32_t lo = blockIdx.x * keys_per;
+    const uint32_t hi = (lo + keys_per < B + 2) ? lo + keys_per : B + 2;
+    const size_t count_t = bt.tcount[0], base_off = bt.base_off[0];
+    uint32_t* offsets = bt.offsets[0];
+    for (uint32_t r = threadIdx.x; r < keys_per; r += 1024) hist[r] = 0;
+    if (threadIdx.x == 0) {
+        s_below = 0;
+        s_total = 0;
+        nbig = 0;
+    }
+    __syncthreads();
+    uint32_t below = 0, total = 0;
+    Fe<R> s0 = fe_zero<R>();
+    uint32_t idx0 = 0;
+    if (threadIdx.x < M) {
+        s0 = fe_load<R>(list_sc + threadIdx.x);
+        idx0 = list_idx[threadIdx.x];
+        if (!mont) s0 = fe_to_mont<R>(s0);
+    }
+    for (uint32_t e = threadIdx.x; e < M; e += 1024) {
+        Fe<R> s = s0;
+        if (e >= 1024) {
+            s = fe_load<R>(list_sc + e);
+            if (!mont) s = fe_to_mont<R>(s);
+        }
+        msm_for_each_digit<R>(s, win, [&](int, uint32_t d, uint32_t) {
+            if (!d) return;
+            ++total;
+            if (d < lo) ++below;
+            else if (d < hi) atomicAdd(&hist[d - lo], 1u);
+        });
+    }
+#pragma unroll
+    for (int d = 32; d >= 1; d >>= 1) {
+        below += __shfl_down(below, d);
+        total += __shfl_down(total, d);
+    }
+    if ((threadIdx.x & 63u) == 0) {
+        atomicAdd(&s_below, below);
+        atomicAdd(&s_total, total);
+    }
+    __syncthreads();
+    const uint32_t pairs = s_total;
+    uint32_t clo = 1;
+    const uint32_t twice = lanes_fold ? (pairs / B) / 11u : 2u * (pairs / B);
+    while (clo < (uint32_t)MSM_CHUNK_MIN && (clo + 1) * (clo + 1) <= twice) ++clo;
+    const uint32_t even = (uint32_t)(((uint64_t)pairs + acc_threads - 1) / acc_threads);
+    const uint32_t chunk = even > clo ? even : clo;
+    uint32_t run[MSM_SHORT_PER], first[MSM_SHORT_PER];
+    uint32_t mine = 0;
+#pragma unroll
+    for (int k = 0; k < MSM_SHORT_PER; ++k) {
+        const uint32_t col = threadIdx.x * MSM_SHORT_PER + k;
+        run[k] = col < keys_per ? hist[col] : 0u;
+        mine += run[k];
+    }
+    first[0] = s_below + block_excl_scan_1024(mine, wsum, nullptr);
+#pragma unroll
+    for (int k = 1; k < MSM_SHORT_PER; ++k) first[k] = first[k - 1] + run[k - 1];
+#pragma unroll
+    for (int k = 0; k < MSM_SHORT_PER; ++k) {
+        const uint32_t col = threadIdx.x * MSM_SHORT_PER + k;
+        const uint32_t key = lo + col;
+        if (col >= keys_per || key >= hi) continue;
+        offsets[key] = first[k];
+        cursor[col] = first[k];
+        if (key >= 1 && key <= B && run[k]) {
+            const uint32_t tb = (first[k] + chunk - 1) / chunk;
+            const uint32_t te = (uint32_t)(((uint64_t)first[k] + run[k] + chunk - 1) / chunk);
+            uint32_t at = 256;
+            if (te - tb > 8) at = atomicAdd(&nbig, 1u);
+            if (at < 256) {
+                big[at][0] = key; big[at][1] = tb; big[at][2] = te;
+            } else {
+                for (uint32_t t = tb; t < te; ++t) chunk_bucket[t] = key;
+            }
+        }
+    }
+    __syncthreads();
+    const uint32_t nb = nbig < 256u ? nbig : 256u;
+    for (uint32_t e = 0; e < nb; ++e)
+        for (uint32_t t = big[e][1] + threadIdx.x; t < big[e][2]; t += 1024) chunk_bucket[t] = big[e][0];
+    for (uint32_t e = threadIdx.x; e < M; e += 1024) {
+        Fe<R> s = s0;
+        uint32_t idx = idx0;
+        if (e >= 1024) {
+            s = fe_load<R>(list_sc + e);
+            if (!mont) s = fe_to_mont<R>(s);
+            idx = list_idx[e];
+        }
+        msm_for_each_digit<R>(s, win, [&](int w, uint32_t d, uint32_t neg) {
+            if (!d || d < lo || d >= hi) return;
+            const uint32_t at = atomicAdd(&cursor[d - lo], 1u);
+            vals[at] = (uint32_t)((size_t)w * count_t + base_off + idx) | (neg << 31);
+        });
+    }
+    if (blockIdx.x == 0 && threadIdx.x == 0) {
+        bt.params[0][0] = chunk;
+        bt.params[0][1] = pairs;
+        *bt.heavy[0] = 0;
+        *count_next = 0;
+        *entries_out = raw;
+    }
 }
 
 template <class C>
@@ -1090,7 +1212,7 @@
     for (DevBuf& b : st.wb_scalars) dev_free(c, b.p);
     dev_free(c, st.wb_dig);
     void* ptrs[] = {st.vals2, st.pairs, st.bin_offs, st.bin_aux, st.bin_start, st.tile_start, st.cnt2, st.pos2, st.chunk_bucket,
-                    st.tile_desc};
+                    st.tile_desc, st.short_idx, st.short_scalars, st.short_count};
     for (void* p : ptrs) dev_free(c, p);
     for (int i = 0; i < MsmState::SLOTS; ++i) {
         dev_free(c, st.heavy[i]); dev_free(c, st.offsets[i]); dev_free(c, st.pieces[i]); dev_free(c, st.params[i]);
@@ -1294,9 +1416,9 @@
 
 template <class C>
 static int msm_enqueue_batch(zkt_ctx* c, int k, const void* const* d_scalars, const size_t* ns, const size_t* base_offs, int mont,
-                             const int* slots, const int* tbls) {
+                             const int* slots, const int* tbls, const MsmShortList* sh = nullptr) {
     MsmState& st = *c->msm;
-    if (k < 1 || k > MSM_BATCH) return set_err(c, ZKT_ERR_INVALID_ARGUMENT, "msm batch size");
+    if (k < 1 || k > MSM_BATCH || (sh && k != 1)) return set_err(c, ZKT_ERR_INVALID_ARGUMENT, "msm batch size");
     ++c->msm_epoch;
     for (int j = 0; j < k; ++j)
         for (int w = 0; w < st.n_tail_wait; ++w)
@@ -1327,8 +1449,18 @@
     ProfScope prof_all(c, all_lag ? "msm_lag_main" : "msm_main", nullptr, (uint64_t)k);
     const MsmWork wk{st.bin_offs, st.bin_aux, st.bin_start, st.tile_start, st.tile_desc, st.cnt2, st.pos2, st.pairs, st.vals2,
                      st.chunk_bucket};
-    if (int rc = msm_launch_grouping<C, false>(c, st.plan, wk, bt, mont, n_max, (unsigned)k, st.acc_threads, st.defer_tails))
+    if (sh) {
+        using R = typename C::Fr;
+        const uint32_t keys_per = (st.plan.keys + 2 + MSM_SHORT_WGS - 1) / MSM_SHORT_WGS;
+        hipLaunchKernelGGL(k_msm_short_group<C>, dim3(MSM_SHORT_WGS), dim3(1024), (size_t)keys_per * 8, c->stream, sh->idx,
+                           (const Fe<R>*)sh->scalars, sh->count, st.short_count + ((st.short_seq + 1) & 1u), sh->cap, mont, st.plan.win,
+                           st.plan.keys, keys_per, (uint32_t)st.acc_threads, st.defer_tails ? 1u : 0u, wk.vals, wk.chunk_bucket,
+                           st.short_entries_dev + slots[0], bt);
+        ZKT_HIP(c, hipGetLastError());
+        ++st.short_seq;
+    } else if (int rc = msm_launch_grouping<C, false>(c, st.plan, wk, bt, mont, n_max, (unsigned)k, st.acc_threads, st.defer_tails)) {
         return rc;
+    }
     for (int j = 0; j < k; ++j) {
         MsmBatch one = bt;
         one.offsets[0] = bt.offsets[j];
@@ -1338,7 +1470,8 @@
         {
             ProfScope prof_acc(c, tbls[j] ? "msm_lag_accumulate" : "msm_accumulate");
             if (int rc = msm_launch_accumulate<C>(c, st.plan, st.vals2 + (size_t)j * st.strides.s_vals,
-                                                  st.chunk_bucket + (size_t)j * st.strides.s_chunk, one, ns[j], st.acc_threads, st.acc_lds))
+                                                  st.chunk_bucket + (size_t)j * st.strides.s_chunk, one,
+                                                  sh ? std::min(ns[j], (size_t)sh->cap) : ns[j], st.acc_threads, st.acc_lds))
                 return rc;
         }
         ZKT_HIP(c, hipEventRecord(st.ev_main[slots[j]], c->stream));
@@ -1435,6 +1568,50 @@
     if (c->curve == ZKT_CURVE_BN254) return msm_enqueue<Bn254Curve>(c, d_scalars, n, base_off, mont, slot, tbl);
     return msm_enqueue<Bls381Curve>(c, d_scalars, n, base_off, mont, slot, tbl);
 }
+bool msm_short_fits(const zkt_ctx* c) {
+    return c->msm && ((size_t)c->msm->plan.keys + 2 + MSM_SHORT_WGS - 1) / MSM_SHORT_WGS <= (size_t)MSM_SHORT_KEYS;
+}
+static uint32_t msm_short_cap(size_t n) {
+    size_t cap = std::max<size_t>(16, n / 8);
+    if (const char* e = exp_env("ZKT_SHORT_MSM_CAP")) cap = (size_t)std::max(1, atoi(e));
+    return (uint32_t)std::min(std::min<size_t>(cap, MSM_SHORT_CAP), n);
+}
+int msm_short_list(zkt_ctx* c, size_t n, MsmShortList* out) {
+    if (!msm_short_fits(c)) return set_err(c, ZKT_ERR_INVALID_ARGUMENT, "no short MSM path under this key");
+    MsmState& st = *c->msm;
+    if (!st.short_count) {
+        int rc;
+        if ((rc = dev_alloc(c, (void**)&st.short_idx, (size_t)MSM_SHORT_CAP * 4))) return rc;
+        if ((rc = dev_alloc(c, &st.short_scalars, (size_t)MSM_SHORT_CAP * 32))) return rc;
+        ZKT_HIP(c, hipHostMalloc((void**)&st.short_entries, MsmState::SLOTS * 4, hipHostMallocMapped));
+        memset(st.short_entries, 0, MsmState::SLOTS * 4);
+        ZKT_HIP(c, hipHostGetDevicePointer((void**)&st.short_entries_dev, st.short_entries, 0));
+        if ((rc = dev_alloc(c, (void**)&st.short_count, 8))) return rc;
+        ZKT_HIP(c, hipMemsetAsync(st.short_count, 0, 8, c->stream));
+        st.short_seq = 0;
+    }
+    out->idx = st.short_idx;
+    out->scalars = st.short_scalars;
+    out->count = st.short_count + (st.short_seq & 1u);
+    out->cap = msm_short_cap(n);
+    return ZKT_OK;
+}
+int msm_begin_short(zkt_ctx* c, const MsmShortList& list, size_t n, int mont, int slot, int tbl) {
+    if (!msm_short_fits(c) || !c->msm->short_count || list.count != c->msm->short_count + (c->msm->short_seq & 1u))
+        return set_err(c, ZKT_ERR_INVALID_ARGUMENT, "short MSM: not the list of msm_short_list");
+    if (slot < 0 || slot >= MsmState::SLOTS) return set_err(c, ZKT_ERR_INVALID_ARGUMENT, "bad MSM slot");
+    if (tbl != 1 || !c->msm->tbl_table(tbl)) return set_err(c, ZKT_ERR_NOT_LOADED, "no Lagrange-basis table built");
+    if (n == 0 || n > c->msm->tbl_count(tbl) || list.cap > n || list.cap > MSM_SHORT_CAP)
+        return set_err(c, ZKT_ERR_TOO_MANY_COEFFICIENTS, "TooManyCoefficients: polynomial longer than the committer key");
+    const void* none = nullptr;
+    const size_t off = 0;
+    if (c->curve == ZKT_CURVE_BN254) return msm_enqueue_batch<Bn254Curve>(c, 1, &none, &n, &off, mont, &slot, &tbl, &list);
+    return msm_enqueue_batch<Bls381Curve>(c, 1, &none, &n, &off, mont, &slot, &tbl, &list);
+}
+uint32_t msm_short_entries(const zkt_ctx* c, int slot) {
+    return c->msm && c->msm->short_entries ? c->msm->short_entries[slot] : 0u;
+}
+
 int msm_begin_batch(zkt_ctx* c, int k, const void* const* d_scalars, const size_t* ns, int mont, const int* slots, const int* tbls) {
     if (!c->msm) return set_err(c, ZKT_ERR_NOT_LOADED, "no SRS loaded (zkt_srs_load)");
     if (k < 1 || k > MSM_BATCH) return set_err(c, ZKT_ERR_INVALID_ARGUMENT, "msm batch size");
diff --git a/zkt-plonk_amd/csrc/msm.hpp b/zkt-plonk_amd/csrc/msm.hpp
--- a/zkt-plonk_amd/csrc/msm.hpp
+++ b/zkt-plonk_amd/csrc/msm.hpp
@@ -126,6 +126,13 @@
     bool defer_tails = false;
     int tail_wait[SLOTS] = {};
     int n_tail_wait = 0;
+    uint32_t* short_idx = nullptr;
+    void* short_scalars = nullptr;
+    uint32_t* short_count = nullptr;
+    uint32_t short_seq = 0;
+    uint32_t short_cap_alloc = 0;
+    uint32_t* short_entries = nullptr;
+    uint32_t* short_entries_dev = nullptr;
     ~MsmState() {
         for (int i = 0; i < SLOTS; ++i) {
             if (host_result[i]) (void)hipHostFree(host_result[i]);
@@ -134,6 +141,7 @@
         }
         if (side) (void)hipStreamDestroy(side);
         if (wb_pin) (void)hipHostFree(wb_pin);
+        if (short_entries) (void)hipHostFree(short_entries);
     }
 };
 
@@ -174,6 +182,17 @@
 int msm_flush_tails(zkt_ctx* c);
 bool msm_defers_tails(const zkt_ctx* c);
 bool msm_batches_grouping(const zkt_ctx* c);
+constexpr uint32_t MSM_SHORT_CAP = 8192;
+struct MsmShortList {
+    uint32_t* idx;
+    void* scalars;
+    uint32_t* count;
+    uint32_t cap;
+};
+bool msm_short_fits(const zkt_ctx* c);
+int msm_short_list(zkt_ctx* c, size_t n, MsmShortList* out);
+int msm_begin_short(zkt_ctx* c, const MsmShortList& list, size_t n, int mont, int slot, int tbl);
+uint32_t msm_short_entries(const zkt_ctx* c, int slot);
 
 int lagrange_ensure(zkt_ctx* c, int log_n);
 bool lagrange_ready(const zkt_ctx* c, int log_n);
diff --git a/zkt-plonk_amd/csrc/poly.hip b/zkt-plonk_amd/csrc/poly.hip
--- a/zkt-plonk_amd/csrc/poly.hip
+++ b/zkt-plonk_amd/csrc/poly.hip
@@ -451,6 +451,64 @@
         }
     }
     fe_store<P>(D + i, fe_mul<P>(fe_sub<P>(e0, e1), ninv));
+}
+
+constexpr int LAG_COMPACT_PER = 4;
+template <class P>
+__global__ __launch_bounds__(256) void k_lagrange_scalars_compact(const Fe<P>* __restrict__ ev, size_t n, const uint32_t* __restrict__ len,
+                                                                  const Fe<P>* __restrict__ bl, int k, const Fe<P>* __restrict__ roots,
+                                                                  Fe<P> ninv, uint32_t cap, uint32_t* count, uint32_t* __restrict__ list_idx,
+                                                                  Fe<P>* __restrict__ list_sc) {
+    const size_t first = (size_t)blockIdx.x * (256 * LAG_COMPACT_PER) + threadIdx.x;
+    const size_t L = k ? (size_t)*len : n;
+    Fe<P> a0[LAG_COMPACT_PER], a1[LAG_COMPACT_PER];
+#pragma unroll
+    for (int r = 0; r < LAG_COMPACT_PER; ++r) {
+        const size_t i = first + 256u * r;
+        a0[r] = (i < n) ? fe_load<P>(ev + i) : fe_zero<P>();
+        a1[r] = (i + 1 < n) ? fe_load<P>(ev + i + 1) : fe_zero<P>();
+    }
+#pragma unroll
+    for (int r = 0; r < LAG_COMPACT_PER; ++r) {
+        const size_t i = first + 256u * r;
+        Fe<P> d = fe_zero<P>();
+        if (i >= n && i < n + (size_t)k) {
+            const size_t t = i - n;
+            for (int j = 0; j < k; ++j)
+                if (L + j == n + t) d = fe_add<P>(d, fe_load<P>(bl + j));
+        } else if (i < n) {
+            Fe<P> e0 = a0[r], e1 = a1[r];
+            bool same = L == n;
+#pragma unroll
+            for (int w = 0; w < P::N; ++w) same = same && e0.v[w] == e1.v[w];
+            if (!same) {
+                if (L != n) {
+                    for (int j = 0; j < k; ++j) {
+                        const size_t q = (L + j) & (n - 1);
+                        if (q == (size_t)j) continue;
+                        const Fe<P> b = fe_load<P>(bl + j);
+                        e0 = fe_add<P>(e0, fe_mul<P>(b, fe_sub<P>(fe_load<P>(roots + ((i * q) & (n - 1))), fe_load<P>(roots + ((i * j) & (n - 1))))));
+                        if (i + 1 < n)
+                            e1 = fe_add<P>(e1, fe_mul<P>(b, fe_sub<P>(fe_load<P>(roots + (((i + 1) * q) & (n - 1))),
+                                                                       fe_load<P>(roots + (((i + 1) * j) & (n - 1))))));
+                    }
+                }
+                d = fe_mul<P>(fe_sub<P>(e0, e1), ninv);
+            }
+        }
+        const bool nz = !fe_is_zero<P>(d);
+        const unsigned long long mask = __ballot(nz);
+        if (!mask) continue;
+        const uint32_t lane = threadIdx.x & 63u;
+        const int leader = __ffsll((long long)mask) - 1;
+        uint32_t at = 0;
+        if ((int)lane == leader) at = atomicAdd(count, (uint32_t)__popcll(mask));
+        at = __shfl(at, leader) + (uint32_t)__popcll(mask & ((1ull << lane) - 1ull));
+        if (nz && at < cap) {
+            list_idx[at] = (uint32_t)i;
+            fe_store<P>(list_sc + at, d);
+        }
+    }
 }
 
 struct FxArg {
@@ -1079,6 +1137,21 @@
 int lagrange_scalars(zkt_ctx* c, const void* ev, size_t n, const uint32_t* d_len, const void* d_blinders, int k, const void* d_roots,
                      void* out) {
     ZKT_DISPATCH(c, lagrange_scalars_t, ev, n, d_len, d_blinders, k, d_roots, out);
+}
+template <class P> static int lagrange_scalars_compact_t(zkt_ctx* c, const void* ev, size_t n, const uint32_t* d_len, const void* d_bl, int k,
+                                                         const void* roots, uint32_t cap, uint32_t* d_count, uint32_t* list_idx, void* list_sc) {
+    Fe<P> nn = fe_zero<P>();
+    nn.v[0] = (uint32_t)(n & 0xffffffffu);
+    nn.v[1] = (uint32_t)((uint64_t)n >> 32);
+    const Fe<P> ninv = fe_inv_host<P>(fe_to_mont<P>(nn));
+    hipLaunchKernelGGL(k_lagrange_scalars_compact<P>, dim3((unsigned)((n + (size_t)k + 256 * LAG_COMPACT_PER - 1) / (256 * LAG_COMPACT_PER))), dim3(256), 0, c->stream, (const Fe<P>*)ev, n, d_len,
+                       (const Fe<P>*)d_bl, k, (const Fe<P>*)roots, ninv, cap, d_count, list_idx, (Fe<P>*)list_sc);
+    ZKT_HIP(c, hipGetLastError());
+    return ZKT_OK;
+}
+int lagrange_scalars_compact(zkt_ctx* c, const void* ev, size_t n, const uint32_t* d_len, const void* d_blinders, int k, const void* d_roots,
+                             uint32_t cap, uint32_t* d_count, uint32_t* list_idx, void* list_scalars) {
+    ZKT_DISPATCH(c, lagrange_scalars_compact_t, ev, n, d_len, d_blinders, k, d_roots, cap, d_count, list_idx, list_scalars);
 }
 
 template <class P> static FxArg hat_arg(const Fe<P>& s) {
diff --git a/zkt-plonk_amd/csrc/poly.hpp b/zkt-plonk_amd/csrc/poly.hpp
--- a/zkt-plonk_amd/csrc/poly.hpp
+++ b/zkt-plonk_amd/csrc/poly.hpp
@@ -62,6 +62,8 @@
 int poly_trim_blind(zkt_ctx* c, const TrimBlindSpec* jobs, int nb, size_t n, int zero_count);
 int lagrange_scalars(zkt_ctx* c, const void* ev, size_t n, const uint32_t* d_len, const void* d_blinders, int k, const void* d_roots,
                      void* out);
+int lagrange_scalars_compact(zkt_ctx* c, const void* ev, size_t n, const uint32_t* d_len, const void* d_blinders, int k, const void* d_roots,
+                             uint32_t cap, uint32_t* d_count, uint32_t* list_idx, void* list_scalars);
 int poly_eval_many(zkt_ctx* c, const EvalArgs& a, void* d_partials, void* d_results, void* d_powers);
 int poly_eval_open_tables(zkt_ctx* c, const EvalArgs& a, const uint32_t z0[8], const uint32_t z0_inv[8], const uint32_t z1[8],
                           const uint32_t z1_inv[8], size_t len, void* d_partials, void* d_results, void* d_powers);
diff --git a/zkt-plonk_amd/csrc/prover.hip b/zkt-plonk_amd/csrc/prover.hip
--- a/zkt-plonk_amd/csrc/prover.hip
+++ b/zkt-plonk_amd/csrc/prover.hip
@@ -59,6 +59,18 @@
     void* qev = nullptr;
     void* lag_scalars = nullptr;
     void* lag_scalars_q[3] = {};
+    struct ShortJob {
+        bool on = false;
+        const void* ev = nullptr;
+        const void* blinders = nullptr;
+        const uint32_t* len = nullptr;
+        int k = 0, len_slot = 0;
+        uint32_t cap = 0;
+    };
+    ShortJob short_job[11];
+    bool short_gave_up[16] = {};
+    uint64_t short_srs_generation = 0;
+    uint64_t short_taken = 0, short_fell_back = 0;
     void* small = nullptr;
     uint32_t* status = nullptr;
     uint32_t* lk_u32 = nullptr;
@@ -174,6 +186,43 @@
     return q;
 }
 
+static bool short_msm_wanted(zkt_ctx* c, CircuitState& S, int len_slot, bool queued) {
+    if (c->short_msm == 0 || !(c->short_parts & 1) || c->sharded() || !msm_short_fits(c)) return false;
+    if (queued && c->short_msm != 2) return false;
+    if (S.short_srs_generation != c->srs_generation) {
+        for (bool& g : S.short_gave_up) g = false;
+        S.short_srs_generation = c->srs_generation;
+    }
+    return !S.short_gave_up[len_slot];
+}
+static int short_msm_begin(zkt_ctx* c, CircuitState& S, const void* ev, const void* blinders, const uint32_t* d_len, int k, int len_slot,
+                           int slot) {
+    MsmShortList l{};
+    int rc;
+    if ((rc = msm_short_list(c, S.n + (size_t)k, &l))) return rc;
+    if ((rc = lagrange_scalars_compact(c, ev, S.n, d_len, blinders, k, S.roots, l.cap, l.count, l.idx, l.scalars))) return rc;
+    if ((rc = msm_begin_short(c, l, S.n + (size_t)k, 1, slot, 1))) return rc;
+    CircuitState::ShortJob& j = S.short_job[slot];
+    j.on = true; j.ev = ev; j.blinders = blinders; j.len = d_len; j.k = k; j.len_slot = len_slot; j.cap = l.cap;
+    return ZKT_OK;
+}
+static int short_msm_check(zkt_ctx* c, CircuitState& S, int slot, bool* redo) {
+    *redo = false;
+    const CircuitState::ShortJob j = S.short_job[slot];
+    S.short_job[slot].on = false;
+    if (!j.on) return ZKT_OK;
+    const uint32_t entries = msm_short_entries(c, slot);
+    ++S.short_taken;
+    if (exp_env("ZKT_HOST_TRACE"))
+        fprintf(stderr, "[zkt host] short msm: commitment %d has %u entries (capacity %u)\n", j.len_slot, entries, j.cap);
+    if (entries <= j.cap) return ZKT_OK;
+    S.short_gave_up[j.len_slot] = true;
+    ++S.short_fell_back;
+    *redo = true;
+    if (int rc = lagrange_scalars(c, j.ev, S.n, j.len, j.blinders, j.k, S.roots, S.lag_scalars)) return rc;
+    return msm_begin(c, S.lag_scalars, S.n + (size_t)j.k, 0, 1, slot, 1);
+}
+
 constexpr int WIRE_ELIM_MIN_LOG_N = 17;
 constexpr int QUOTIENT_CLASSES_MIN_LOG_N = 18;
 
@@ -280,8 +329,11 @@
     }
     int commit_evals_begin(const void* ev, const void* d_poly, int blinder_off, int k, int len_slot, int slot) {
         const bool q = queueing();
+        S.short_job[slot].on = false;
         if (!lagrange_ready(c, S.log_n) || c->lagrange_off)
             return q ? commit_push(d_poly, S.n + (size_t)k, slot, 0) : commit_begin(d_poly, S.n + (size_t)k, slot);
+        if (short_msm_wanted(c, S, len_slot, q))
+            return short_msm_begin(c, S, ev, (const char*)S.small + (size_t)blinder_off * 32, S.status + 8 + len_slot, k, len_slot, slot);
         if (q && n_lag_queued == 3)
             if (int rc0 = commit_flush()) return rc0;
         void* d = q ? S.lag_scalars_q[n_lag_queued] : S.lag_scalars;
@@ -313,6 +365,21 @@
             if (skip && skip[j]) continue;
             memcpy(out[j].x.v, xy + 12 * j, Q::N * 4);
             memcpy(out[j].y.v, xy + 12 * j + Q::N / 2, Q::N * 4);
+        }
+        return ZKT_OK;
+    }
+
+    int short_recollect(const int* slots, const bool* skip, int k, Affine<Q>* out) {
+        for (int j = 0; j < k; ++j) {
+            if (skip && skip[j]) {
+                S.short_job[slots[j]].on = false;
+                continue;
+            }
+            bool redo = false;
+            int rc = short_msm_check(c, S, slots[j], &redo);
+            if (rc) return rc;
+            if (!redo) continue;
+            if ((rc = msm_flush_tails(c)) || (rc = commit_collect(slots + j, nullptr, 1, out + j))) return rc;
         }
         return ZKT_OK;
     }
@@ -724,6 +791,7 @@
         const bool skip[6] = {false, false, false, same_table, false, false};
         int rc;
         if ((rc = commit_collect(slots, skip, 6, cm))) return rc;
+        if ((rc = short_recollect(slots + 3, skip + 3, 3, cm + 3))) return rc;
         if ((rc = collect_wires(cm))) return rc;
         mark("wait commits of rounds 1+2");
         if (!same_table) {
@@ -834,7 +902,8 @@
         if ((rc = commit_flush())) return rc;
         if ((rc = to_coset_many({W_Z1, W_Z2}))) return rc;
         if ((rc = public_inputs(in))) return rc;
-        return commit_collect(slots, nullptr, 2, cm + 6);
+        if ((rc = commit_collect(slots, nullptr, 2, cm + 6))) return rc;
+        return short_recollect(slots + 1, nullptr, 1, cm + 7);
     }
 
 
@@ -1783,6 +1852,22 @@
     return ZKT_OK;
 }
 
+int zkt_ctx_set_short_msm(zkt_ctx* c, int mode) {
+    if (!c) return ZKT_ERR_INVALID_ARGUMENT;
+    if (mode < 0 || mode > 2) return set_err(c, ZKT_ERR_INVALID_ARGUMENT, "mode: 0 the full scalar vector, 1 automatic, 2 the list at every size");
+    c->short_msm = mode;
+    ++c->msm_epoch;
+    return ZKT_OK;
+}
+
+int zkt_debug_short_msm(zkt_ctx* c, uint64_t* out_taken, uint64_t* out_fell_back) {
+    if (!c) return ZKT_ERR_INVALID_ARGUMENT;
+    if (!c->circuit) return set_err(c, ZKT_ERR_NOT_LOADED, "no circuit loaded (zkt_circuit_load)");
+    if (out_taken) *out_taken = c->circuit->short_taken;
+    if (out_fell_back) *out_fell_back = c->circuit->short_fell_back;
+    return ZKT_OK;
+}
+
 int zkt_debug_quotient_top(zkt_ctx* c, uint64_t* out_u, int* out_on_classes) {
     if (!c || !out_u) return set_err(c, ZKT_ERR_INVALID_ARGUMENT, "null pointer");
     if (!c->circuit) return set_err(c, ZKT_ERR_NOT_LOADED, "no circuit loaded (zkt_circuit_load)");
@@ -1878,10 +1963,18 @@
         if (k && (rc = poly_add_blinders(c, poly, d_len, d_bl, k, n + 8))) return rc;
     }
     if (path == 0) return msm_g1_dev(c, poly, n + (size_t)k, 0, 1, out_xy, out_is_infinity);
-    if ((rc = lagrange_scalars(c, d_evals, n, d_len, d_bl, k, S.roots, S.lag_scalars))) return rc;
-    if ((rc = msm_begin(c, S.lag_scalars, n + (size_t)k, 0, 1, 0, 1))) return rc;
     uint64_t xy[12] = {};
-    if ((rc = msm_end(c, 0, xy))) return rc;
+    S.short_job[0].on = false;
+    if (short_msm_wanted(c, S, 12, false)) {
+        bool redo = false;
+        if ((rc = short_msm_begin(c, S, d_evals, d_bl, d_len, k, 12, 0)) || (rc = msm_end(c, 0, xy)) || (rc = short_msm_check(c, S, 0, &redo)))
+            return rc;
+        if (redo && (rc = msm_end(c, 0, xy))) return rc;
+    } else {
+        if ((rc = lagrange_scalars(c, d_evals, n, d_len, d_bl, k, S.roots, S.lag_scalars))) return rc;
+        if ((rc = msm_begin(c, S.lag_scalars, n + (size_t)k, 0, 1, 0, 1))) return rc;
+        if ((rc = msm_end(c, 0, xy))) return rc;
+    }
     const size_t words = c->curve == ZKT_CURVE_BN254 ? 8 : 12;
     memcpy(out_xy, xy, words * 8);
     if (out_is_infinity) {
```

Measured after the change: 71.33 proofs/s (median of 6 runs). Within noise of the previous version (+1.0%).
